# ayushpradhan-dev/robust-speech-analysis-framework

Measured on AMD Instinct MI355X. Metric: audio-seconds processed/sec (extract+CNN-LSTM fwd), higher is better.
Workload: dtype f32

## Files before the change

robust_speech_analysis_framework_amd/csrc/mshds_pitch.hip:

```cpp
#include <algorithm>
#include <map>
#include <mutex>
#include <vector>

#include "mshds_common.h"
#include "mshds_pitch_layout.h"

namespace rsaf {
namespace mshds {

struct PitchParams {
    double dt, min_pitch, ceiling, voicing_thr, octave_cost, dt_window;
    int cheb_all_full;
    int cheb_clipped;
    int nsamp_window, half_window, nsamp_period, half_period, min_lag, max_lag, brent_ixmax, max_cand;
    int refine_depth, is_cc;
    int nfft;
    double voicing_thr2;
    int debug_stop;
};

struct FrameOut {
    double intensity;
    double ncand;
    double freq[MAXC];
    double strength[MAXC];
};

typedef double double4_t __attribute__((ext_vector_type(4)));
__device__ __forceinline__ double cheb_eval(const double* __restrict__ c, double frac) {
    const double t = 2.0 * frac - 1.0, t2 = 2.0 * t;
    double b1 = 0.0, b2 = 0.0;
#pragma unroll
    for (int j = NCH - 1; j >= 1; --j) { const double b0 = fma(t2, b1, c[j] - b2); b2 = b1; b1 = b0; }
    return fma(t, b1, c[0] - b2);
}

__device__ void improve_max_cheb(const double* __restrict__ Pc, int x0, bool live, double& xm, double& ym) {
    const double ix1 = (double)x0 + 1.0;
    double c0[NCH], c1[NCH];
#pragma unroll
    for (int j = 0; j < NCH; ++j) { c0[j] = Pc[j]; c1[j] = Pc[NCH + j]; }
    auto f = [&](double v1) {
        double fl = floor(v1);
        double cell = fl - (ix1 - 1.0);
        cell = cell < 0.0 ? 0.0 : (cell > 1.0 ? 1.0 : cell);
        const double frac = v1 - (ix1 - 1.0 + cell);
        const bool hi = cell > 0.5;
        const double t = 2.0 * frac - 1.0, t2 = 2.0 * t;
        double b1 = 0.0, b2 = 0.0;
#pragma unroll
        for (int j = NCH - 1; j >= 1; --j) { const double b0 = fma(t2, b1, (hi ? c1[j] : c0[j]) - b2); b2 = b1; b1 = b0; }
        return -fma(t, b1, (hi ? c1[0] : c0[0]) - b2);
    };
    brent_maximise(f, ix1, live, xm, ym);
}

struct RefineArgs {
    const double* r; int RN, RC, depth, nz_lo, nz_hi, ncand;
    const int* place; double* cf; double* cs;
};
template <int G, bool RECUR>
__device__ void refine_candidates(const RefineArgs& A, int tid, int nthreads) {
    const int lane = tid & 63, lg = lane & (G - 1), gidx = (tid >> 6) * (64 / G) + lane / G;
    __syncthreads();
    for (int kb = 1; kb < A.ncand; kb += nthreads / G) {
        const int k = kb + gidx;
        const bool live = k < A.ncand;
        double xm, ym;
        improve_max_group<G, RECUR>(A.r, A.RN, (double)(A.place[live ? k : 1] + A.RC), A.depth, A.nz_lo, A.nz_hi, lg,
                                    live, xm, ym);
        if (ym > 1.0) ym = 1.0 / ym;
        if (live && lg == 0) { A.cf[k] = 1.0 / DXS / (xm - A.RC); A.cs[k] = ym; }
    }
}


__device__ __forceinline__ double2_t cmul(double2_t a, double2_t b) {
    return double2_t{a.x * b.x - a.y * b.y, a.x * b.y + a.y * b.x};
}
__device__ __forceinline__ double2_t tw_at(const double2_t* __restrict__ tw, int t, int M) {
    const bool neg = t >= M;
    const double2_t w = tw[neg ? t - M : t];
    return neg ? double2_t{-w.x, -w.y} : w;
}

template <int LOG2M>
struct FftPlan {
    static constexpr int M = 1 << LOG2M, N = 2 * M;
    static constexpr int N4 = LOG2M / 2;
    static constexpr bool HAS2 = (LOG2M & 1) != 0;
    static constexpr int T4 = M / 4, T2 = M / 2;
    static constexpr int BPT4 = T4 > 256 ? T4 / 256 : 1, BPT2 = T2 > 256 ? T2 / 256 : 1;
    static constexpr bool PRE = LOG2M <= 11;
    static constexpr int NTW4 = PRE && N4 > 1 ? (N4 - 1) * BPT4 * 3 : 1, NTW2 = PRE && HAS2 ? BPT2 : 1;
};

template <int LOG2M>
struct FftTw {
    double2_t w4[FftPlan<LOG2M>::NTW4];
    double2_t w2[FftPlan<LOG2M>::NTW2];
};

template <int LOG2M>
__device__ __forceinline__ void fft_load_twiddles(FftTw<LOG2M>& R, const double2_t* __restrict__ tw, int tid) {
    using PL = FftPlan<LOG2M>;
    if (!PL::PRE) return;
#pragma unroll
    for (int st = 1; st < PL::N4; ++st) {
        const int Ns = 1 << (2 * st), step = PL::N / (Ns * 4);
#pragma unroll
        for (int bq = 0; bq < PL::BPT4; ++bq) {
            const int j = tid + 256 * bq, t1 = (j & (Ns - 1)) * step;
#pragma unroll
            for (int r = 1; r <= 3; ++r) R.w4[((st - 1) * PL::BPT4 + bq) * 3 + r - 1] = tw_at(tw, (r * t1) & (PL::N - 1), PL::M);
        }
    }
    if (PL::HAS2) {
        const int Ns = 1 << (2 * PL::N4), step = PL::N / (Ns * 2);
#pragma unroll
        for (int bq = 0; bq < PL::BPT2; ++bq) R.w2[bq] = tw_at(tw, ((tid + 256 * bq) & (Ns - 1)) * step, PL::M);
    }
}

__device__ __forceinline__ int fsw(int e) { return e ^ ((e >> 3) & 3); }

template <int LOG2M>
__device__ __forceinline__ double2_t* fft_stockham(double2_t* a, double2_t* b, const FftTw<LOG2M>& R,
                                                   const double2_t* __restrict__ tw, int tid) {
    using PL = FftPlan<LOG2M>;
    constexpr int M = PL::M, N = PL::N, T4 = PL::T4, T2 = PL::T2;
    double2_t* src = a;
    double2_t* dst = b;
#pragma unroll
    for (int st = 0; st < PL::N4; ++st) {
        const int Ns = 1 << (2 * st), step = N / (Ns * 4);
#pragma unroll
        for (int bq = 0; bq < PL::BPT4; ++bq) {
            const int j = tid + 256 * bq;
            if (T4 >= 256 || j < T4) {
                const int k = j & (Ns - 1);
                const bool rs = st == 1;
                double2_t v0 = src[rs ? fsw(j) : j], v1 = src[rs ? fsw(j + T4) : j + T4], v2 = src[rs ? fsw(j + 2 * T4) : j + 2 * T4],
                          v3 = src[rs ? fsw(j + 3 * T4) : j + 3 * T4];
                if (st > 0) {
                    if (PL::PRE) {
                        const int o = ((st - 1) * PL::BPT4 + bq) * 3;
                        v1 = cmul(v1, R.w4[o]);
                        v2 = cmul(v2, R.w4[o + 1]);
                        v3 = cmul(v3, R.w4[o + 2]);
                    } else {
                        const int t1 = k * step;
                        v1 = cmul(v1, tw_at(tw, t1, M));
                        v2 = cmul(v2, tw_at(tw, 2 * t1, M));
                        v3 = cmul(v3, tw_at(tw, 3 * t1, M));
                    }
                }
                const double2_t a0 = v0 + v2, a1 = v0 - v2, a2 = v1 + v3;
                const double2_t d = v1 - v3;
                const double2_t a3 = double2_t{d.y, -d.x};
                const int j0 = ((j - k) << 2) + k;
                const bool ws = st == 0 && PL::N4 >= 2;
                dst[ws ? fsw(j0) : j0] = a0 + a2;
                dst[ws ? fsw(j0 + Ns) : j0 + Ns] = a1 + a3;
                dst[ws ? fsw(j0 + 2 * Ns) : j0 + 2 * Ns] = a0 - a2;
                dst[ws ? fsw(j0 + 3 * Ns) : j0 + 3 * Ns] = a1 - a3;
            }
        }
        __syncthreads();
        double2_t* t_ = src; src = dst; dst = t_;
    }
    if (PL::HAS2) {
        const int Ns = 1 << (2 * PL::N4), step = N / (Ns * 2);
#pragma unroll
        for (int bq = 0; bq < PL::BPT2; ++bq) {
            const int j = tid + 256 * bq;
            if (T2 >= 256 || j < T2) {
                const int k = j & (Ns - 1);
                const double2_t v0 = src[j];
                const double2_t v1 = cmul(src[j + T2], PL::PRE ? R.w2[bq] : tw_at(tw, k * step, M));
                const int j0 = ((j - k) << 1) + k;
                dst[j0] = v0 + v1;
                dst[j0 + Ns] = v0 - v1;
            }
        }
        __syncthreads();
        double2_t* t_ = src; src = dst; dst = t_;
    }
    return src;
}


template <int LOG2N>
__global__ __launch_bounds__(256) void pitch_cc_kernel(const float* __restrict__ wav, const ClipInfo* __restrict__ ci,
                                                       const double* __restrict__ gpeak, const PitchParams P,
                                                       const double2_t* __restrict__ tw1, const double2_t* __restrict__ tw2,
                                                       double* __restrict__ rbuf, int rstride, int max_frames) {
    extern __shared__ __attribute__((aligned(16))) char smem_raw[];
    const ClipInfo c = ci[blockIdx.y];
    if ((int)blockIdx.x * CC_FRAMES_PER_WG >= c.n_frames) return;
    const int tid = threadIdx.x, lane = tid & 63, wv = tid >> 6;
    constexpr int N = 1 << LOG2N, M = N >> 1;
    const int nw = P.nsamp_window, L = P.max_lag;
    const int seg_len = nw + L + 1;
    FftTw<LOG2N> twa;
    FftTw<LOG2N - 1> twb;
    fft_load_twiddles<LOG2N>(twa, tw1, tid);
    fft_load_twiddles<LOG2N - 1>(twb, tw2, tid);
    constexpr int NPK = (M / 2) / 256 + 1;
    double2_t twp[NPK];
#pragma unroll
    for (int i = 0; i < NPK; ++i) twp[i] = tw2[tid + 256 * i <= M / 2 ? tid + 256 * i : 0];
    const CcLds lds(N, L);
    double2_t* za = lds.za<double2_t>(smem_raw);
    double2_t* zb = lds.zb<double2_t, N>(smem_raw);
    double* s_sy = lds.sy(smem_raw);
    double* s_red = lds.scratch(smem_raw) + CcLds::RED;
    double* s_val = lds.scratch(smem_raw) + CcLds::VAL;
    double* s_scan = lds.scratch(smem_raw) + CcLds::SCAN;
    const float* x = wav + c.sample_off;
    const int n = c.n_samples;
    const double gp = gpeak[blockIdx.y];
    for (int f = blockIdx.x * CC_FRAMES_PER_WG; f < (int)(blockIdx.x + 1) * CC_FRAMES_PER_WG && f < c.n_frames; ++f) {
    double* rb = rbuf + ((int64_t)blockIdx.y * max_frames + f) * rstride;
    const double t = c.t1 + f * P.dt;
    const int64_t left = low_index(t, c.x1), right = left + 1;
    {
        int64_t s0 = right - P.nsamp_period, s1 = left + P.nsamp_period;
        s0 = s0 < 0 ? 0 : (s0 > n - 1 ? n - 1 : s0);
        s1 = s1 < 0 ? 0 : (s1 > n - 1 ? n - 1 : s1);
        double s = 0.0;
        for (int64_t i = s0 + tid; i <= s1; i += 256) s += (double)x[i];
        s = group_sum<64>(s);
        if (lane == 0) s_red[wv] = s;
    }
    __syncthreads();
    const double local_mean = (s_red[0] + s_red[1] + s_red[2] + s_red[3]) / (2.0 * P.nsamp_period);
    int loc_max_lag;
    {
        const double start_time = t - 0.5 * (1.0 / P.min_pitch + P.dt_window);
        int64_t start = low_index(start_time, c.x1);
        if (start < 0) start = 0;
        int64_t span = L + nw;
        if (span > n - start) span = n - start;
        loc_max_lag = (int)(span - nw);
        int pa = P.half_window - P.half_period, pb = P.half_window + P.half_period;
        pa = pa < 0 ? 0 : pa;
        pb = pb > nw ? nw : pb;
        double m = 0.0, sx = 0.0;
        const float* xs = x + start;
        const int avail = (int)((n - start) < (int64_t)seg_len ? (n - start) : (int64_t)seg_len);
#pragma unroll 4
        for (int j = tid; j < N; j += 256) {
            const double v = j < avail ? ((double)xs[j] - local_mean) : 0.0;
            za[j] = double2_t{j < nw ? v : 0.0, v};
            if (j >= pa && j < pb) m = fmax(m, fabs(v));
            if (j < nw) sx += v * v;
        }
        m = wave_max_dpp(m);
        sx = group_sum<64>(sx);
        if (lane == 0) { s_val[wv] = m; s_red[4 + wv] = sx; }
    }
    __syncthreads();
    const double local_peak = fmax(fmax(s_val[0], s_val[1]), fmax(s_val[2], s_val[3]));
    const double intensity = gp > 0.0 ? (local_peak > gp ? 1.0 : local_peak / gp) : 0.0;
    const double sumx2 = (s_red[4] + s_red[5]) + (s_red[6] + s_red[7]);
    {
        constexpr int NQ = 4;
        double inc[NQ];
#pragma unroll
        for (int q = 0; q < NQ; ++q) {
            const int i = tid + 256 * q;
            double d = 0.0;
            if (i < L) { const double u = za[i + nw].y, w0 = za[i].y; d = u * u - w0 * w0; }
            double sc = d;
#pragma unroll
            for (int o = 1; o < 64; o <<= 1) { const double t2 = __shfl_up(sc, o, 64); if (lane >= o) sc += t2; }
            inc[q] = sc;
            if (lane == 63) s_scan[4 * q + wv] = sc;
        }
        __syncthreads();
        if (tid == 0) s_sy[0] = sumx2;
#pragma unroll
        for (int q = 0; q < NQ; ++q) {
            const int i = tid + 256 * q;
            if (i < L) {
                double off = 0.0;
                for (int z = 0; z < 4 * q + wv; ++z) off += s_scan[z];
                s_sy[i + 1] = sumx2 + (off + inc[q]);
            }
        }
    }
    if (P.debug_stop == 1) continue;

    double2_t* Z = fft_stockham<LOG2N>(za, zb, twa, tw1, tid);
    double2_t* Y = Z == za ? zb : za;
    auto spec = [&](int k) {
        const double2_t zk = Z[k], zn = Z[(N - k) & (N - 1)];
        const double2_t A = double2_t{0.5 * (zk.x + zn.x), 0.5 * (zk.y - zn.y)};
        const double2_t Bm = double2_t{0.5 * (zk.y + zn.y), -0.5 * (zk.x - zn.x)};
        return double2_t{A.x * Bm.x + A.y * Bm.y, A.x * Bm.y - A.y * Bm.x};
    };
#pragma unroll
    for (int i = 0; i < NPK; ++i) {
        const int k = tid + 256 * i;
        if (k > M / 2) continue;
        const double2_t ck = spec(k), cm = spec(M - k);
        const double2_t w = twp[i];
        {
            const double2_t su = double2_t{ck.x + cm.x, ck.y - cm.y}, di = double2_t{ck.x - cm.x, ck.y + cm.y};
            const double2_t yy = double2_t{su.x - (w.x * di.y - w.y * di.x), su.y + (w.x * di.x + w.y * di.y)};
            Y[k] = double2_t{yy.x, -yy.y};
        }
        if (k != 0 && k != M - k) {
            const double2_t su = double2_t{cm.x + ck.x, cm.y - ck.y}, di = double2_t{cm.x - ck.x, cm.y + ck.y};
            const double2_t yy = double2_t{su.x + (w.x * di.y + w.y * di.x), su.y - (w.x * di.x - w.y * di.y)};
            Y[M - k] = double2_t{yy.x, -yy.y};
        }
    }
    __syncthreads();
    const double* r = reinterpret_cast<const double*>(fft_stockham<LOG2N - 1>(Y, Y == za ? zb : za, twb, tw2, tid));
    if (P.debug_stop == 2) continue;
    if (tid == 0) { rb[0] = 1.0; rb[L + 1] = intensity; }
    const double inv_n = 1.0 / (double)N;
    for (int l = 1 + tid; l <= L; l += 256) {
        const double v = ((l & 1) ? -r[l] : r[l]) * inv_n;
        const double den = sumx2 * s_sy[l];
        rb[l] = (l <= loc_max_lag && den > 0.0) ? v / sqrt(den) : 0.0;
    }
    __syncthreads();
    }
}


__device__ __forceinline__ wfft::cplx ld_tw(const double2_t* __restrict__ tw, int i) {
    const double2_t w = tw[i];
    return wfft::cplx{w.x, w.y};
}
__device__ __forceinline__ double fast_rsqrt(double d) {
    double y = __builtin_amdgcn_rsq(d);
    y = y * (1.5 - 0.5 * d * y * y);
    y = y * (1.5 - 0.5 * d * y * y);
    return y;
}
__device__ __forceinline__ double wave_scan_incl(double v, int lane) {
    v += dpp_f64<0x111>(v);
    v += dpp_f64<0x112>(v);
    v += dpp_f64<0x114>(v);
    v += dpp_f64<0x118>(v);
    const double t0 = readlane_f64(v, 15), t1 = readlane_f64(v, 31), t2 = readlane_f64(v, 47);
    const int row = lane >> 4;
    return v + (row == 0 ? 0.0 : (row == 1 ? t0 : (row == 2 ? t0 + t1 : (t0 + t1) + t2)));
}

template <int R>
__global__ __launch_bounds__(64, R == 32 ? 2 : (R == 16 ? 3 : 4)) void pitch_ac_wave_kernel(const float* __restrict__ wav, const ClipInfo* __restrict__ ci,
                                                           const double* __restrict__ gpeak, const double* __restrict__ win,
                                                           const double* __restrict__ wr, const PitchParams P,
                                                           const double2_t* __restrict__ tw, double* __restrict__ rbuf,
                                                           int rstride, int max_frames) {
    using namespace wfft;
    extern __shared__ __attribute__((aligned(16))) char smem_raw[];
    double* lds = reinterpret_cast<double*>(smem_raw);
    const ClipInfo c = ci[blockIdx.y];
    const int f0 = blockIdx.x * WF_FRAMES;
    if (f0 >= c.n_frames) return;
    const int lane_ = threadIdx.x;
    constexpr int S = 64 * R, N = 2 * S, L2 = 64 / R;
    const int nw = P.nsamp_window, L = P.brent_ixmax;
    const float* x = wav + c.sample_off;
    const int n = c.n_samples;
    const double gp = gpeak[blockIdx.y];
    LdsMem mem{lds};
    const int f1 = f0 + WF_FRAMES < c.n_frames ? f0 + WF_FRAMES : c.n_frames;
    int pa = P.half_window - P.half_period, pb = P.half_window + P.half_period;
    pa = pa < 0 ? 0 : pa;
    pb = pb > nw ? nw : pb;
#pragma unroll 1
    for (int f = f0; f < f1; ++f) {
        int lane = lane_;
        asm volatile("" : "+v"(lane));
        cplx w_s = ld_tw(tw, 2 * lane), w_b = ld_tw(tw, (lane % L2) * (N / 64));
        double* rb = rbuf + ((int64_t)blockIdx.y * max_frames + f) * rstride;
        const double t = c.t1 + f * P.dt;
        const int left = (int)low_index(t, c.x1), right = left + 1;
        const int start = right - P.half_window;
        const bool inside = start >= 0 && start + nw <= n;
        cplx v[R];
#pragma unroll
        for (int m = 0; m < R; ++m) {
            const int j = 128 * m + 2 * lane;
            int i0 = start + j, i1 = i0 + 1;
            i0 = i0 < 0 ? 0 : (i0 > n - 1 ? n - 1 : i0);
            i1 = i1 < 0 ? 0 : (i1 > n - 1 ? n - 1 : i1);
            v[m] = cplx{(double)x[i0], (double)x[i1]};
        }
        double local_mean;
        {
            int s0 = right - P.nsamp_period, s1 = left + P.nsamp_period;
            s0 = s0 < 0 ? 0 : (s0 > n - 1 ? n - 1 : s0);
            s1 = s1 < 0 ? 0 : (s1 > n - 1 ? n - 1 : s1);
            double sm = 0.0;
            if (inside && s0 >= start && s1 < start + nw) {
                const int a0 = s0 - start, a1 = s1 - start;
#pragma unroll
                for (int m = 0; m < R; ++m) {
                    const int jb = 128 * m, j = jb + 2 * lane;
                    if (jb + 127 >= a0 && jb <= a1) {
                        if (j >= a0 && j <= a1) sm += v[m].x;
                        if (j + 1 >= a0 && j + 1 <= a1) sm += v[m].y;
                    }
                }
            } else {
                for (int i = s0 + lane; i <= s1; i += 256) {
                    const float q0 = x[i], q1 = i + 64 <= s1 ? x[i + 64] : 0.f, q2 = i + 128 <= s1 ? x[i + 128] : 0.f,
                                q3 = i + 192 <= s1 ? x[i + 192] : 0.f;
                    sm += ((double)q0 + (double)q1) + ((double)q2 + (double)q3);
                }
            }
            local_mean = group_sum<64>(sm) / (2.0 * P.nsamp_period);
        }
        constexpr int WCH = R == 32 ? 8 : 4;
        double pk = 0.0;
#pragma unroll
        for (int mc = 0; mc < R; mc += WCH) {
            double2_t w2[WCH];
#pragma unroll
            for (int u = 0; u < WCH; ++u) {
                const int j = 128 * (mc + u) + 2 * lane;
                w2[u] = *reinterpret_cast<const double2_t*>(win + (j < nw ? j : nw - 2));
            }
#pragma unroll
            for (int u = 0; u < WCH; ++u) {
                const int m = mc + u, jb = 128 * m, j = jb + 2 * lane;
                const bool on = j < nw;
                const double e0 = on ? (v[m].x - local_mean) * w2[u].x : 0.0, e1 = on ? (v[m].y - local_mean) * w2[u].y : 0.0;
                if (jb + 127 >= pa && jb < pb) {
                    if (j >= pa && j < pb) pk = fmax(pk, fabs(e0));
                    if (j + 1 >= pa && j + 1 < pb) pk = fmax(pk, fabs(e1));
                }
                v[m] = cplx{e0, e1};
            }
            asm volatile("" ::: "memory");
        }
        const double local_peak = wave_max_dpp(pk);
        const double intensity = gp > 0.0 ? (local_peak > gp ? 1.0 : local_peak / gp) : 0.0;
        if (P.debug_stop == 1) continue;
        wave_fft<R>(v, lds, lane, w_s, w_b);
        {
            ac_spec_store<R>(v, mem, lane);
            wave_sync();
            const cplx y_half = ac_spec_pairs<R>(v, mem, lane, ld_tw(tw, lane));
            wave_sync();
            ac_spec_load<R>(v, mem, lane, y_half);
            wave_sync();
        }
        asm volatile("" : "+v"(lane));
        w_s = ld_tw(tw, 2 * lane);
        w_b = ld_tw(tw, (lane % L2) * (N / 64));
        wave_fft<R>(v, lds, lane, w_s, w_b);
        if (P.debug_stop == 2) continue;
        const double r0 = readlane_f64(v[0].x, 0);
        if (lane == 0) { rb[0] = 1.0; rb[L + 1] = intensity; }
        double wa[8], wb[8];
#pragma unroll
        for (int m = 0; m < 8; ++m) {
            const int l0 = 2 * (lane + 64 * m);
            wa[m] = wr[l0 < L ? l0 : L];
            wb[m] = wr[l0 + 1 < L ? l0 + 1 : L];
        }
#pragma unroll
        for (int m = 0; m < 8; ++m) {
            const int l0 = 2 * (lane + 64 * m);
            if (128 * m > L) break;
            if (l0 >= 1 && l0 <= L) rb[l0] = r0 > 0.0 ? v[m].x * fast_rcp(r0 * wa[m]) : 0.0;
            if (l0 + 1 <= L) rb[l0 + 1] = r0 > 0.0 ? -v[m].y * fast_rcp(r0 * wb[m]) : 0.0;
        }
    }
}

template <int R>
__global__ __launch_bounds__(64, R == 32 ? 2 : 3) void pitch_cc_wave_kernel(const float* __restrict__ wav, const ClipInfo* __restrict__ ci,
                                                           const double* __restrict__ gpeak, const PitchParams P,
                                                           const double2_t* __restrict__ tw, double* __restrict__ rbuf,
                                                           int rstride, int max_frames) {
    using namespace wfft;
    extern __shared__ __attribute__((aligned(16))) char smem_raw[];
    const int nw = P.nsamp_window, L = P.max_lag;
    const CcWaveLds lay(Plan<R>::LDS_DOUBLES, L);
    double* lds = lay.fft(smem_raw);
    double* s_sy = lay.sy(smem_raw);
    const ClipInfo c = ci[blockIdx.y];
    const int f0 = blockIdx.x * WF_FRAMES;
    if (f0 >= c.n_frames) return;
    const int lane_ = threadIdx.x;
    constexpr int S = 64 * R, H = R / 2, L2 = 64 / R, L2H = 64 / H;
    const int seg_len = nw + L + 1;
    const float* x = wav + c.sample_off;
    const int n = c.n_samples;
    const double gp = gpeak[blockIdx.y];
    LdsMem mem{lds};
    const int f1 = f0 + WF_FRAMES < c.n_frames ? f0 + WF_FRAMES : c.n_frames;
    int pa = P.half_window - P.half_period, pb = P.half_window + P.half_period;
    pa = pa < 0 ? 0 : pa;
    pb = pb > nw ? nw : pb;
#pragma unroll 1
    for (int f = f0; f < f1; ++f) {
        int lane = lane_;
        asm volatile("" : "+v"(lane));
        double* rb = rbuf + ((int64_t)blockIdx.y * max_frames + f) * rstride;
        const double t = c.t1 + f * P.dt;
        const int left = (int)low_index(t, c.x1), right = left + 1;
        const double start_time = t - 0.5 * (1.0 / P.min_pitch + P.dt_window);
        int64_t start64 = low_index(start_time, c.x1);
        if (start64 < 0) start64 = 0;
        const int start = (int)start64;
        int span = L + nw;
        if (span > n - start) span = n - start;
        const int loc_max_lag = span - nw;
        const int avail = n - start < seg_len ? n - start : seg_len;
        cplx v[R];
#pragma unroll
        for (int m = 0; m < R; ++m) {
            int gi = start + lane + 64 * m;
            gi = gi > n - 1 ? n - 1 : gi;
            v[m] = cplx{0.0, (double)x[gi]};
        }
        float tail[16];
#pragma unroll
        for (int q = 0; q < 16; ++q) {
            int gi = start + lane + 64 * q + nw;
            gi = gi > n - 1 ? n - 1 : gi;
            tail[q] = x[gi];
        }
        double local_mean;
        {
            int s0 = right - P.nsamp_period, s1 = left + P.nsamp_period;
            s0 = s0 < 0 ? 0 : (s0 > n - 1 ? n - 1 : s0);
            s1 = s1 < 0 ? 0 : (s1 > n - 1 ? n - 1 : s1);
            double sm = 0.0;
            if (s0 >= start && s1 < start + avail) {
                const int a0 = s0 - start, a1 = s1 - start;
#pragma unroll
                for (int m = 0; m < R; ++m) {
                    const int jb = 64 * m, j = jb + lane;
                    if (jb + 63 >= a0 && jb <= a1 && j >= a0 && j <= a1) sm += v[m].y;
                }
            } else {
                for (int i = s0 + lane; i <= s1; i += 256) {
                    const float q0 = x[i], q1 = i + 64 <= s1 ? x[i + 64] : 0.f, q2 = i + 128 <= s1 ? x[i + 128] : 0.f,
                                q3 = i + 192 <= s1 ? x[i + 192] : 0.f;
                    sm += ((double)q0 + (double)q1) + ((double)q2 + (double)q3);
                }
            }
            local_mean = group_sum<64>(sm) / (2.0 * P.nsamp_period);
        }
        double pk = 0.0, sx = 0.0;
#pragma unroll
        for (int m = 0; m < R; ++m) {
            const int jb = 64 * m, j = jb + lane;
            double e = 0.0, a = 0.0;
            if (j < avail) e = v[m].y - local_mean;
            if (j < nw) a = e;
            if (jb + 63 >= pa && jb < pb && j >= pa && j < pb) pk = fmax(pk, fabs(e));
            sx = fma(a, a, sx);
            v[m] = cplx{a, e};
        }
        const double local_peak = wave_max_dpp(pk);
        const double intensity = gp > 0.0 ? (local_peak > gp ? 1.0 : local_peak / gp) : 0.0;
        const double sumx2 = group_sum<64>(sx);
        {
            double carry = 0.0;
            if (lane == 0) s_sy[0] = sumx2;
#pragma unroll
            for (int q = 0; q < 16; ++q) {
                if (64 * q >= L) break;
                const int i = lane + 64 * q;
                double d = 0.0;
                if (i < L) {
                    const double u = i + nw < avail ? (double)tail[q] - local_mean : 0.0, w0 = v[q].y;
                    d = u * u - w0 * w0;
                }
                const double sc = wave_scan_incl(d, lane);
                if (i < L) s_sy[i + 1] = sumx2 + (carry + sc);
                carry += readlane_f64(sc, 63);
            }
        }
        if (P.debug_stop == 1) continue;
        const cplx w_s1 = ld_tw(tw, lane);
        wave_fft<R>(v, lds, lane, w_s1, ld_tw(tw, (lane % L2) * R));
        cplx y[H];
        cc_spec_store<R>(v, mem, lane);
        wave_sync();
        const cplx y_half = cc_spec_pairs<R>(v, y, mem, lane, w_s1);
        wave_sync();
        cc_spec_load<R>(y, mem, lane, y_half);
        wave_sync();
        wave_fft<H>(y, lds, lane, ld_tw(tw, 2 * lane), ld_tw(tw, (lane % L2H) * R));
        if (P.debug_stop == 2) continue;
        if (lane == 0) { rb[0] = 1.0; rb[L + 1] = intensity; }
        const double inv_n = 1.0 / (double)S;
        constexpr int MO = H < 8 ? H : 8;
        double ya[MO], yb[MO];
#pragma unroll
        for (int m = 0; m < MO; ++m) {
            const int l0 = 2 * (lane + 64 * m);
            ya[m] = s_sy[l0 < L ? l0 : L];
            yb[m] = s_sy[l0 + 1 < L ? l0 + 1 : L];
        }
#pragma unroll
        for (int m = 0; m < MO; ++m) {
            const int l0 = 2 * (lane + 64 * m);
            if (128 * m > L) break;
            if (l0 >= 1 && l0 <= L) {
                const double den = sumx2 * ya[m];
                rb[l0] = (l0 <= loc_max_lag && den > 0.0) ? (y[m].x * inv_n) * fast_rsqrt(den) : 0.0;
            }
            if (l0 + 1 <= L) {
                const double den = sumx2 * yb[m];
                rb[l0 + 1] = (l0 + 1 <= loc_max_lag && den > 0.0) ? (-y[m].y * inv_n) * fast_rsqrt(den) : 0.0;
            }
        }
        wave_sync();
    }
}

constexpr int CT = 64;
struct DeferArgs {
    FrameHdr* hdr;
    double* pc_a;
    double* pc_b;
    int grouped;
};
struct CandCtx {
    const PitchParams& P;
    const DeferArgs& DA;
    const double* cheb;
    int lane;
    int L, RC, RN;
    int nz_lo, nz_hi;
    double* r;
    double *s_mfreq, *s_mstr, *s_mloc;
    int* s_maxlag;
    int* s_cnt;
    double* s_part;
};

__device__ __forceinline__ void cand_load_row(const CandCtx& X, const double* __restrict__ rb, int r_lo, int r_hi) {
    const int tid = X.lane, RC = X.RC, L = X.L;
    double* r = X.r;
    for (int j0 = RC + r_lo + tid; j0 <= RC + r_hi; j0 += 10 * CT) {
        double v[10];
#pragma unroll
        for (int u = 0; u < 10; ++u) {
            const int j = j0 + u * CT;
            const int l = j >= RC ? j - RC : RC - j;
            v[u] = rb[l <= L ? l : L];
        }
#pragma unroll
        for (int u = 0; u < 10; ++u) {
            const int j = j0 + u * CT;
            const int l = j >= RC ? j - RC : RC - j;
            if (j <= RC + r_hi) r[j] = l <= L ? v[u] : 0.0;
        }
    }
}

__device__ __forceinline__ void cand_collect_maxima(const CandCtx& X, double thr_low) {
    const PitchParams& P = X.P;
    const int lane = X.lane, RC = X.RC;
    const double* r = X.r;
    int* s_maxlag = X.s_maxlag;
    int* s_cnt = X.s_cnt;
    const int lag_lo = P.min_lag > 2 ? P.min_lag : 2;
    int lag_hi = P.max_lag - 1;
    if (lag_hi > P.brent_ixmax - 1) lag_hi = P.brent_ixmax - 1;
    int count = 0;
    for (int base = lag_lo; base <= lag_hi; base += 64) {
        const int l = base + lane;
        bool ok = false;
        if (l <= lag_hi) {
            const double v = r[RC + l];
            ok = (v > 0.5 * thr_low) && (v > r[RC + l - 1]) && (v >= r[RC + l + 1]);
        }
        const unsigned long long m = __ballot(ok);
        const int pos = count + __popcll(m & ((1ull << lane) - 1ull));
        if (ok && pos < MAX_MAXIMA) s_maxlag[pos] = l;
        count += __popcll(m);
    }
    if (lane == 0) s_cnt[CandLds::CNT_NMAX] = count < MAX_MAXIMA ? count : MAX_MAXIMA;
}

__device__ __forceinline__ void cand_first_estimates(const CandCtx& X, int nmax) {
    const PitchParams& P = X.P;
    const int lane = X.lane, RC = X.RC, RN = X.RN, nz_lo = X.nz_lo, nz_hi = X.nz_hi;
    const double* r = X.r;
    const int* s_maxlag = X.s_maxlag;
    double *s_mfreq = X.s_mfreq, *s_mstr = X.s_mstr, *s_mloc = X.s_mloc;
    const int l16 = lane & 15, gidx = lane >> 4;
    for (int mb = 0; mb < nmax; mb += CT / 16) {
        const int m = mb + gidx;
        const bool live = m < nmax;
        const int l = s_maxlag[live ? m : 0];
        const double y0 = r[RC + l - 1], y1 = r[RC + l], y2 = r[RC + l + 1];
        const double dr = 0.5 * (y2 - y0), d2r = 2.0 * y1 - y0 - y2;
        const double fm = 1.0 / DXS / (l + dr / d2r);
        double st = sinc_group<16, false>(r, RN, RC + 1.0 / DXS / fm, 30, nz_lo, nz_hi, l16);
        if (st > 1.0) st = 1.0 / st;
        if (live && l16 == 0) { s_mfreq[m] = fm; s_mstr[m] = st; s_mloc[m] = st - P.octave_cost * log2(P.min_pitch / fm); }
    }
}

struct CandMaxima { double mloc0, mloc1, mr0, mr1; };
__device__ __forceinline__ void cand_build_list(const CandCtx& X, const CandMaxima& M, double vthr, double* cf, double* cs,
                                                double* cloc, int* place_lag, int* ncand_out) {
    const PitchParams& P = X.P;
    const int lane = X.lane;
    const double mloc0 = M.mloc0, mloc1 = M.mloc1, mr0 = M.mr0, mr1 = M.mr1;
    const double *s_mfreq = X.s_mfreq, *s_mstr = X.s_mstr;
    const int* s_maxlag = X.s_maxlag;
    unsigned long long todo0 = __ballot(mr0 > 0.5 * vthr), todo1 = __ballot(mr1 > 0.5 * vthr);
    double my_loc = 0.0;
    int my_m = -1, nc = 1;
    double weakest = 2.0;
    int wplace = 0;
    bool known = false;
    for (int half = 0; half < 2; ++half) {
        unsigned long long todo = half ? todo1 : todo0;
        while (todo) {
            const int bit = __ffsll((long long)todo) - 1;
            todo &= todo - 1;
            const int m = 64 * half + bit;
            const double loc_m = readlane_f64(half ? mloc1 : mloc0, bit);
            int place;
            if (nc < P.max_cand) {
                place = nc++;
            } else {
                if (!known) {
                    const double v = (lane >= 1 && lane < P.max_cand) ? my_loc : INFINITY;
                    double mn = v;
#pragma unroll
                    for (int o = 32; o >= 1; o >>= 1) mn = fmin(mn, __shfl_xor(mn, o, 64));
                    if (mn < 2.0) { weakest = mn; wplace = __ffsll((long long)__ballot(v == mn)) - 1; }
                    else { weakest = 2.0; wplace = 0; }
                    known = true;
                }
                place = loc_m <= weakest ? 0 : wplace;
            }
            if (place) {
                if (lane == place) { my_loc = loc_m; my_m = m; }
                known = false;
            }
        }
    }
    if (lane < MAXC) {
        const bool on = lane >= 1 && lane < nc && my_m >= 0;
        cf[lane] = on ? s_mfreq[my_m] : 0.0;
        cs[lane] = on ? s_mstr[my_m] : 0.0;
        cloc[lane] = on ? my_loc : 0.0;
        place_lag[lane] = on ? s_maxlag[my_m] : 0;
    }
    if (lane == 0) *ncand_out = nc;
}

__device__ __forceinline__ int cand_row_min(int v) {
    v = min(v, __builtin_amdgcn_update_dpp(0, v, 0xB1, 0xf, 0xf, false));
    v = min(v, __builtin_amdgcn_update_dpp(0, v, 0x4E, 0xf, 0xf, false));
    v = min(v, __builtin_amdgcn_update_dpp(0, v, 0x141, 0xf, 0xf, false));
    v = min(v, __builtin_amdgcn_update_dpp(0, v, 0x140, 0xf, 0xf, false));
    return __builtin_amdgcn_readlane(v, 0);
}

struct CandClip {
    bool use_cheb;
    int n_clip_cols;
    bool cand_lane;
    int my_b0;
};
__device__ __forceinline__ CandClip cand_clip_analysis(const CandCtx& X, int nc, const int* place_lag) {
    const PitchParams& P = X.P;
    const double* cheb = X.cheb;
    const int lane = X.lane, RC = X.RC, RN = X.RN;
    bool use_cheb = cheb != nullptr;
    int n_clip_cols = 0;
    const bool cand_lane = lane >= 1 && lane < nc;
    const int my_b0 = (cand_lane ? place_lag[lane] : 0) + RC - 1;
    if (use_cheb && !P.cheb_all_full) {
        int dc0 = P.refine_depth, dc1 = P.refine_depth;
        dc0 = dc0 < my_b0 + 1 ? dc0 : my_b0 + 1;
        dc0 = dc0 < RN - my_b0 - 1 ? dc0 : RN - my_b0 - 1;
        dc1 = dc1 < my_b0 + 2 ? dc1 : my_b0 + 2;
        dc1 = dc1 < RN - my_b0 - 2 ? dc1 : RN - my_b0 - 2;
        n_clip_cols = __popcll(__ballot(cand_lane && dc0 < P.refine_depth)) + __popcll(__ballot(cand_lane && dc1 < P.refine_depth));
        const int dmin = cand_row_min(cand_lane ? min(dc0, dc1) : P.refine_depth);
        if (n_clip_cols > 0 && (!P.cheb_clipped || dmin < 3)) use_cheb = false;
    }
    return CandClip{use_cheb, n_clip_cols, cand_lane, my_b0};
}

__device__ __forceinline__ void cand_coef_4x4x4(const CandCtx& X, int nc, const int* place_lag, const CandClip& C) {
    const double* cheb = X.cheb;
    const int lane = X.lane, RC = X.RC, nz_lo = X.nz_lo, nz_hi = X.nz_hi;
    const double* r = X.r;
    const bool cand_lane = C.cand_lane;
    const int my_b0 = C.my_b0;
    double* s_P = X.s_part;
    const int d = X.P.refine_depth;
    const int kq = lane >> 4, nn = lane & 15;
    const int ncol = 2 * (nc - 1);
    const int bmin = cand_row_min(cand_lane ? my_b0 : 0x7fffffff), bmax = -cand_row_min(cand_lane ? -my_b0 : 0x7fffffff);
    const int groups = (ncol + 3) >> 2;
    int rb4[3];
    bool cf4[3];
#pragma unroll
    for (int g = 0; g < 3; ++g) {
        const int n = 4 * g + (lane & 3), k = 1 + (n >> 1);
        rb4[g] = place_lag[k < nc ? k : 1] + RC - 1 + (n & 1);
        cf4[g] = n < ncol;
    }
    int o_lo = nz_lo - (bmax + 1), o_hi = nz_hi - bmin;
    o_lo = o_lo < -(d - 1) ? -(d - 1) : o_lo;
    o_hi = o_hi > d ? d : o_hi;
    double a4[3] = {0.0, 0.0, 0.0};
    const double* ctab = cheb + (int64_t)(d - 1) * NCH + nn;
    int o = o_lo;
    for (; o + 31 <= o_hi; o += 32) {
        double cw[8];
#pragma unroll
        for (int u = 0; u < 8; ++u) cw[u] = ctab[(int64_t)(o + 4 * u + kq) * NCH];
#pragma unroll
        for (int u = 0; u < 8; ++u) {
            const int oo = o + 4 * u + kq;
            a4[0] = __builtin_amdgcn_mfma_f64_4x4x4f64(cw[u], cf4[0] ? r[rb4[0] + oo] : 0.0, a4[0], 0, 0, 0);
            if (groups > 1) a4[1] = __builtin_amdgcn_mfma_f64_4x4x4f64(cw[u], cf4[1] ? r[rb4[1] + oo] : 0.0, a4[1], 0, 0, 0);
            if (groups > 2) a4[2] = __builtin_amdgcn_mfma_f64_4x4x4f64(cw[u], cf4[2] ? r[rb4[2] + oo] : 0.0, a4[2], 0, 0, 0);
        }
    }
    for (; o <= o_hi; o += 4) {
        const int oo = o + kq, oc = oo <= o_hi ? oo : o_hi;
        const double cw = oo <= o_hi ? ctab[(int64_t)oc * NCH] : 0.0;
        a4[0] = __builtin_amdgcn_mfma_f64_4x4x4f64(cw, cf4[0] ? r[rb4[0] + oc] : 0.0, a4[0], 0, 0, 0);
        if (groups > 1) a4[1] = __builtin_amdgcn_mfma_f64_4x4x4f64(cw, cf4[1] ? r[rb4[1] + oc] : 0.0, a4[1], 0, 0, 0);
        if (groups > 2) a4[2] = __builtin_amdgcn_mfma_f64_4x4x4f64(cw, cf4[2] ? r[rb4[2] + oc] : 0.0, a4[2], 0, 0, 0);
    }
    const int coef = (nn & 12) + kq;
#pragma unroll
    for (int g = 0; g < 3; ++g) {
        const int n = 4 * g + (lane & 3), k = 1 + (n >> 1);
        if (g < groups && n < ncol) s_P[(k * 2 + (n & 1)) * NCH + coef] = a4[g];
    }
}

__device__ __forceinline__ void cand_coef_16x16x4(const CandCtx& X, int nc, const int* place_lag, const CandClip& C) {
    const double* cheb = X.cheb;
    const int lane = X.lane, RC = X.RC, RN = X.RN, nz_lo = X.nz_lo, nz_hi = X.nz_hi;
    const double* r = X.r;
    const bool cand_lane = C.cand_lane;
    const int my_b0 = C.my_b0, n_clip_cols = C.n_clip_cols;
    double* s_P = X.s_part;
    const int d = X.P.refine_depth;
    const int kq = lane >> 4, nn = lane & 15;
    const int ncol = 2 * (nc - 1), tiles = (ncol + 15) >> 4;
    const int bmin = cand_row_min(cand_lane ? my_b0 : 0x7fffffff), bmax = -cand_row_min(cand_lane ? -my_b0 : 0x7fffffff);
    int rbase[2];
    bool colfull[2];
#pragma unroll
    for (int T = 0; T < 2; ++T) {
        const int n = 16 * T + nn, k = 1 + (n >> 1);
        rbase[T] = place_lag[k < nc ? k : 1] + RC - 1 + (n & 1);
        colfull[T] = n_clip_cols == 0 || (rbase[T] + 1 >= d && RN - rbase[T] - 1 >= d);
    }
    int o_lo = nz_lo - (bmax + 1), o_hi = nz_hi - bmin;
    o_lo = o_lo < -(d - 1) ? -(d - 1) : o_lo;
    o_hi = o_hi > d ? d : o_hi;
    double4_t acc0 = {0.0, 0.0, 0.0, 0.0}, acc1 = acc0;
    const double* ctab = cheb + (int64_t)(d - 1) * NCH + nn;
    int o = o_lo;
    for (; o + 31 <= o_hi; o += 32) {
        double cw[8];
#pragma unroll
        for (int u = 0; u < 8; ++u) cw[u] = ctab[(int64_t)(o + 4 * u + kq) * NCH];
#pragma unroll
        for (int u = 0; u < 8; ++u) {
            const int oo = o + 4 * u + kq;
            acc0 = __builtin_amdgcn_mfma_f64_16x16x4f64(cw[u], colfull[0] ? r[rbase[0] + oo] : 0.0, acc0, 0, 0, 0);
            if (tiles > 1) acc1 = __builtin_amdgcn_mfma_f64_16x16x4f64(cw[u], colfull[1] ? r[rbase[1] + oo] : 0.0, acc1, 0, 0, 0);
        }
    }
    for (; o <= o_hi; o += 4) {
        const int oo = o + kq, oc = oo <= o_hi ? oo : o_hi;
        const double cw = oo <= o_hi ? ctab[(int64_t)oc * NCH] : 0.0;
        acc0 = __builtin_amdgcn_mfma_f64_16x16x4f64(cw, colfull[0] ? r[rbase[0] + oc] : 0.0, acc0, 0, 0, 0);
        if (tiles > 1) acc1 = __builtin_amdgcn_mfma_f64_16x16x4f64(cw, colfull[1] ? r[rbase[1] + oc] : 0.0, acc1, 0, 0, 0);
    }
#pragma unroll
    for (int T = 0; T < 2; ++T) {
        const int n = 16 * T + nn, k = 1 + (n >> 1);
        if (T < tiles && k < nc) {
#pragma unroll
            for (int v = 0; v < 4; ++v) s_P[(k * 2 + (n & 1)) * NCH + kq + 4 * v] = T == 0 ? acc0[v] : acc1[v];
        }
    }
}

__device__ __forceinline__ void cand_coef_clipped_cells(const CandCtx& X, int nc, const int* place_lag) {
    const double* cheb = X.cheb;
    const int lane = X.lane, RC = X.RC, RN = X.RN;
    const double* r = X.r;
    double* s_P = X.s_part;
    const int d = X.P.refine_depth;
    const int ncol = 2 * (nc - 1);
    __builtin_amdgcn_fence(__ATOMIC_RELEASE, "workgroup");
    __builtin_amdgcn_wave_barrier();
    __builtin_amdgcn_fence(__ATOMIC_ACQUIRE, "workgroup");
    const double* clip_tabs = cheb + (int64_t)2 * d * NCH;
    const int jj = lane & 15, ph = lane >> 4;
    for (int col = 0; col < ncol; ++col) {
        const int k = 1 + (col >> 1), b = place_lag[k] + RC - 1 + (col & 1);
        int dc = d;
        dc = dc < b + 1 ? dc : b + 1;
        dc = dc < RN - b - 1 ? dc : RN - b - 1;
        if (dc >= d) continue;
        const double* tab = clip_tabs + (int64_t)NCH * dc * (dc - 1) + jj;
        double acc = 0.0;
        int o = -(dc - 1) + ph;
        for (; o + 12 <= dc; o += 16) {
            double tw4[4];
#pragma unroll
            for (int u = 0; u < 4; ++u) tw4[u] = tab[(int64_t)(o + 4 * u + dc - 1) * NCH];
#pragma unroll
            for (int u = 0; u < 4; ++u) acc = fma(tw4[u], r[b + o + 4 * u], acc);
        }
        for (; o <= dc; o += 4) acc = fma(tab[(int64_t)(o + dc - 1) * NCH], r[b + o], acc);
        acc += __shfl_xor(acc, 16, 64);
        acc += __shfl_xor(acc, 32, 64);
        if (ph == 0) s_P[(k * 2 + (col & 1)) * NCH + jj] = acc;
    }
}

__device__ __forceinline__ bool cand_hand_over_or_brent(const CandCtx& X, int nc, const int* place_lag, double* cf, double* cs,
                                                        double* pc_out) {
    const DeferArgs& DA = X.DA;
    const int tid = X.lane, RC = X.RC;
    const double* s_P = X.s_part;
    if (DA.hdr) {
        for (int i = 2 * NCH + tid; i < nc * 2 * NCH; i += CT) pc_out[i] = s_P[i];
        __syncthreads();
        return true;
    }
    if (tid < 64) {
        const int k = 1 + tid;
        const bool live = k < nc;
        double xm, ym;
        improve_max_cheb(s_P + (live ? k : 1) * 2 * NCH, place_lag[live ? k : 1] + RC, live, xm, ym);
        if (ym > 1.0) ym = 1.0 / ym;
        if (live) { cf[k] = 1.0 / DXS / (xm - RC); cs[k] = ym; }
    }
    __syncthreads();
    return false;
}

__device__ __forceinline__ void cand_refine_direct(const CandCtx& X, int nc, const int* place_lag, double* cf, double* cs) {
const PitchParams& P = X.P;
const int tid = X.lane, L = X.L, RC = X.RC, RN = X.RN, nz_lo = X.nz_lo, nz_hi = X.nz_hi;
const double* r = X.r;
    const int nref = nc - 1;
    const int span = P.refine_depth < 2 * L ? P.refine_depth : 2 * L;
    RefineArgs A{r, RN, RC, P.refine_depth, nz_lo, nz_hi, nc, place_lag, cf, cs};
    if (nref <= 4) { if (span >= 6 * 64) refine_candidates<64, true>(A, tid, CT); else refine_candidates<64, false>(A, tid, CT); }
    else if (nref <= 8) { if (span >= 6 * 32) refine_candidates<32, true>(A, tid, CT); else refine_candidates<32, false>(A, tid, CT); }
    else { if (span >= 6 * 16) refine_candidates<16, true>(A, tid, CT); else refine_candidates<16, false>(A, tid, CT); }
    __syncthreads();
}

__device__ __forceinline__ bool cand_refine_list(const CandCtx& X, int nc, const int* place_lag, double* cf, double* cs,
                                                 double* pc_out) {
    if (X.DA.hdr && X.DA.grouped) return true;
    const CandClip C = cand_clip_analysis(X, nc, place_lag);
    if (C.use_cheb) {
        const int ncol = 2 * (nc - 1);
        if (nc > 1 && ncol <= 12 && C.n_clip_cols == 0) {
            cand_coef_4x4x4(X, nc, place_lag, C);
        } else if (nc > 1) {
            cand_coef_16x16x4(X, nc, place_lag, C);
            if (C.n_clip_cols > 0) cand_coef_clipped_cells(X, nc, place_lag);
        }
        __syncthreads();
        if (X.P.debug_stop == 6) return true;
        return cand_hand_over_or_brent(X, nc, place_lag, cf, cs, pc_out);
    }
    cand_refine_direct(X, nc, place_lag, cf, cs);
    return false;
}

__device__ __forceinline__ void cand_write_hdr(FrameHdr* hdr, int tid, int flags, int n_a, const int* pl_a, int n_b,
                                               const int* pl_b, int hit) {
    if (tid < MAXC) {
        hdr->lag_a[tid] = (uint16_t)pl_a[tid];
        if (pl_b) {
            hdr->lag_b[tid] = (uint16_t)pl_b[tid];
            hdr->a_slot_of_b[tid] = (uint8_t)hit;
        }
    }
    if (tid == 0) { hdr->flags = flags; hdr->n_a = n_a; hdr->n_b = n_b; }
}

__device__ __forceinline__ void cand_write_frame_out(FrameOut* o, int tid, double intensity, double gp, int ncand,
                                                     const double* cf, const double* cs) {
    if (tid == 0) {
        o->intensity = intensity;
        o->ncand = gp > 0.0 ? (double)ncand : 1.0;
    }
    if (tid < MAXC) {
        const bool on = tid < ncand && gp > 0.0;
        o->freq[tid] = on ? cf[tid] : 0.0;
        o->strength[tid] = on ? cs[tid] : 0.0;
    }
}

__global__ __launch_bounds__(64) void pitch_cand_kernel(const ClipInfo* __restrict__ ci, const double* __restrict__ gpeak,
                                                        const PitchParams P, const double* __restrict__ rbuf, int rstride,
                                                        int max_frames, FrameOut* __restrict__ out,
                                                        FrameOut* __restrict__ out2, const double* __restrict__ cheb,
                                                        const DeferArgs DA) {
    extern __shared__ __attribute__((aligned(16))) char smem_raw[];
    const ClipInfo c = ci[blockIdx.y];
    const int f = blockIdx.x;
    if (f >= c.n_frames) return;
    const int tid = threadIdx.x, lane = tid & 63;
    const int L = P.is_cc ? P.max_lag : P.brent_ixmax;
    const int RC = P.brent_ixmax;
    const int RN = 2 * P.brent_ixmax + 1;
    int r_lo, r_hi;
    pitch_r_range(RC, L, P.min_lag, P.max_lag, (DA.hdr && DA.grouped) ? 30 : P.refine_depth, &r_lo, &r_hi);
    const CandLds lds(r_lo, r_hi);
    double* r_store = lds.r_store(smem_raw);
    double* r = r_store - (RC + r_lo);
    double* lists = lds.lists(smem_raw);
    int* ilists = reinterpret_cast<int*>(lists);
    double* s_mfreq = lists + CandLds::MFREQ;
    double* s_mstr = lists + CandLds::MSTR;
    double* s_mloc = lists + CandLds::MLOC;
    double* s_cf = lists + CandLds::CF;
    double* s_cs = lists + CandLds::CS;
    double* s_cloc = lists + CandLds::CLOC;
    int* s_maxlag = ilists + CandLds::MAXLAG;
    int* s_place = ilists + CandLds::PLACE;
    int* s_place2 = ilists + CandLds::PLACE2;
    int* s_cnt = ilists + CandLds::CNT;
    double* s_cf2 = lists + CandLds::CF2;
    double* s_cs2 = lists + CandLds::CS2;
    double* s_cloc2 = lists + CandLds::CLOC2;
    double* s_part = lists + CandLds::PART;
    const CandCtx X{P, DA, cheb, lane, L, RC, RN, RC - L, RC + L, r, s_mfreq, s_mstr, s_mloc, s_maxlag, s_cnt, s_part};

    FrameOut* o = out + c.frame_off + f;
#define RSAF_PITCH_DBG_STOP(k)                                                                       \
    if (P.debug_stop == (k)) {                                                                       \
        if (tid == 0) { o->intensity = 0.0; o->ncand = 1.0; }                                        \
        if (tid < MAXC) { o->freq[tid] = 0.0; o->strength[tid] = 0.0; }                              \
        return;                                                                                      \
    }
    RSAF_PITCH_DBG_STOP(1)
    RSAF_PITCH_DBG_STOP(2)
    const double* rb = rbuf + ((int64_t)blockIdx.y * max_frames + f) * rstride;
    const double intensity = rb[L + 1];
    const double gp = gpeak[blockIdx.y];
    cand_load_row(X, rb, r_lo, r_hi);
    if (tid == 0) s_cnt[CandLds::CNT_NMAX] = 0;
    __syncthreads();
    const bool dual = out2 != nullptr && P.voicing_thr2 >= 0.0;
    const double thr_low = dual && P.voicing_thr2 < P.voicing_thr ? P.voicing_thr2 : P.voicing_thr;
    cand_collect_maxima(X, thr_low);
    __syncthreads();
    RSAF_PITCH_DBG_STOP(3)
    const int nmax = s_cnt[CandLds::CNT_NMAX];
    cand_first_estimates(X, nmax);
    __syncthreads();
    RSAF_PITCH_DBG_STOP(4)
    const CandMaxima M{lane < nmax ? s_mloc[lane] : 0.0, lane + 64 < nmax ? s_mloc[lane + 64] : 0.0,
                       lane < nmax ? r[RC + s_maxlag[lane]] : -1.0, lane + 64 < nmax ? r[RC + s_maxlag[lane + 64]] : -1.0};
    cand_build_list(X, M, P.voicing_thr, s_cf, s_cs, s_cloc, s_place, &s_cnt[CandLds::CNT_NCAND]);
    if (dual) cand_build_list(X, M, P.voicing_thr2, s_cf2, s_cs2, s_cloc2, s_place2, &s_cnt[CandLds::CNT_NCAND2]);
    __syncthreads();
    const int ncand = s_cnt[CandLds::CNT_NCAND];
    RSAF_PITCH_DBG_STOP(5)
    const int64_t wframe = (int64_t)blockIdx.y * max_frames + f;
    FrameHdr* hdr = DA.hdr ? DA.hdr + wframe : nullptr;
    int flags = 0;
    if (!dual) {
        if (cand_refine_list(X, ncand, s_place, s_cf, s_cs, DA.pc_a ? DA.pc_a + wframe * PC_DOUBLES : nullptr)) flags = HDR_A_DEFER;
        if (hdr) cand_write_hdr(hdr, tid, gp > 0.0 ? flags : 0, ncand, s_place, 0, nullptr, 0);
    } else {
        const int ncand2 = s_cnt[CandLds::CNT_NCAND2];
        const bool low_is_second = P.voicing_thr2 < P.voicing_thr;
        int* pl_a = low_is_second ? s_place2 : s_place;   double* cf_a = low_is_second ? s_cf2 : s_cf;   double* cs_a = low_is_second ? s_cs2 : s_cs;
        int* pl_b = low_is_second ? s_place : s_place2;   double* cf_b = low_is_second ? s_cf : s_cf2;   double* cs_b = low_is_second ? s_cs : s_cs2;
        const int nc_a = low_is_second ? ncand2 : ncand, nc_b = low_is_second ? ncand : ncand2;
        const bool def_a = cand_refine_list(X, nc_a, pl_a, cf_a, cs_a, DA.pc_a ? DA.pc_a + wframe * PC_DOUBLES : nullptr);
        if (def_a) flags |= HDR_A_DEFER;
        if (tid == 0) s_cnt[CandLds::CNT_MISSING] = 0;
        __syncthreads();
        int hit = 0;
        {
            const int pa_reg = tid < MAXC ? pl_a[tid] : 0;
            const int mine = (tid >= 1 && tid < nc_b) ? pl_b[tid] : -1;
            for (int z = 1; z < nc_a; ++z) if (__builtin_amdgcn_readlane(pa_reg, z) == mine) hit = z;
            if (tid >= 1 && tid < nc_b) {
                if (hit) { if (!def_a) { cf_b[tid] = cf_a[hit]; cs_b[tid] = cs_a[hit]; } } else atomicAdd(&s_cnt[CandLds::CNT_MISSING], 1);
            }
        }
        __syncthreads();
        if (s_cnt[CandLds::CNT_MISSING] > 0) {
            if (tid >= 1 && tid < nc_b) {
                for (int m = 0; m < nmax; ++m) if (s_maxlag[m] == pl_b[tid]) { cf_b[tid] = s_mfreq[m]; cs_b[tid] = s_mstr[m]; }
            }
            __syncthreads();
            if (cand_refine_list(X, nc_b, pl_b, cf_b, cs_b, DA.pc_b ? DA.pc_b + wframe * PC_DOUBLES : nullptr)) flags |= HDR_B_DEFER;
        } else if (def_a) {
            flags |= HDR_B_COPY;
        }
        if (hdr) cand_write_hdr(hdr, tid, gp > 0.0 ? flags : 0, nc_a, pl_a, nc_b, pl_b, hit);
        cand_write_frame_out(out2 + c.frame_off + f, tid, intensity, gp, ncand2, s_cf2, s_cs2);
    }
    cand_write_frame_out(o, tid, intensity, gp, ncand, s_cf, s_cs);
}
#undef RSAF_PITCH_DBG_STOP

__global__ __launch_bounds__(256) void pitch_cell_coef_kernel(const ClipInfo* __restrict__ ci, int n_clips, int max_frames,
                                                              const int* __restrict__ hdr, const double* __restrict__ rbuf,
                                                              int rstride, int L, int RC, const double* __restrict__ tabs,
                                                              int b_lo, int n_b, int ntap_pad, int chunk_frames, int n_chunks,
                                                              double* __restrict__ pc) {
    using namespace wfft;
    extern __shared__ __attribute__((aligned(16))) char smem_raw[];
    const CellLds lds(ntap_pad);
    double* tab = lds.tab(smem_raw);
    unsigned* qall = lds.queues(smem_raw);
    const int64_t wid = blockIdx.x;
    const int64_t q = wid >> 3;
    const int bi = (int)(q % n_b);
    const int64_t chunk = (q / n_b) * 8 + (wid & 7);
    if (chunk >= n_chunks) return;
    const int tid = threadIdx.x, lane = tid & 63, wv = tid >> 6;
    unsigned* qb = qall + wv * CELL_Q;
    const int b = b_lo + bi;
    const int lag0 = b - RC + 1, lag1 = b - RC;
    const int64_t total = (int64_t)n_clips * max_frames;
    const int per_wave = chunk_frames / 4;
    const int64_t g_begin = chunk * chunk_frames + (int64_t)wv * per_wave;
    const int64_t g_end = g_begin + per_wave < total ? g_begin + per_wave : total;
    const int nn = lane & 15, kq = lane >> 4;
    struct Rec { int nc; int lw[8]; };
    auto load_rec = [&](int64_t g) {
        Rec r;
        r.nc = 0;
#pragma unroll
        for (int i = 0; i < 8; ++i) r.lw[i] = 0;
        if (g < g_end) {
            const int clip = (int)(g / max_frames), fr = (int)(g - (int64_t)clip * max_frames);
            if (fr < ci[clip].n_frames) {
                const FrameHdr* h = FrameHdr::at(hdr, g);
                const int flags = h->flags, nc = h->n_a;
#pragma unroll
                for (int i = 0; i < 8; ++i) r.lw[i] = (int)h->lag_a_pair(i);
                r.nc = (flags & HDR_A_DEFER) ? nc : 0;
            }
        }
        return r;
    };
    Rec rec = load_rec(g_begin + lane);
    {
        const double2_t* src = reinterpret_cast<const double2_t*>(tabs + (int64_t)bi * ntap_pad * NCH);
        double2_t* dst = reinterpret_cast<double2_t*>(tab);
        const int n2 = ntap_pad * NCH / 2;
        for (int i0 = tid; i0 < n2; i0 += 8 * 256) {
            double2_t v[8];
#pragma unroll
            for (int u = 0; u < 8; ++u) v[u] = src[i0 + 256 * u < n2 ? i0 + 256 * u : n2 - 1];
#pragma unroll
            for (int u = 0; u < 8; ++u) if (i0 + 256 * u < n2) dst[i0 + 256 * u] = v[u];
        }
    }
    __syncthreads();
    int count = 0;
    auto run_tile = [&](int off, int n) {
        const unsigned e = qb[off + (nn < n ? nn : 0)];
        const int64_t g = e >> 5;
        const int k = (e >> 1) & 15, c = e & 1;
        const double* rb = rbuf + g * rstride;
        double4_t acc = {0.0, 0.0, 0.0, 0.0};
        double av[2][8], bv[2][8];
        auto fetch = [&](int t0, double (&a8)[8], double (&b8)[8]) {
#pragma unroll
            for (int u = 0; u < 8; ++u) {
                const int t = t0 + 4 * u + kq;
                const int tc = t < ntap_pad ? t : ntap_pad - 1;
                b8[u] = rb[tc <= L ? tc : L];
                a8[u] = t < ntap_pad ? tab[tc * NCH + nn] : 0.0;
            }
        };
        fetch(0, av[0], bv[0]);
        for (int t0 = 0; t0 < ntap_pad; t0 += 64) {
            if (t0 + 32 < ntap_pad) fetch(t0 + 32, av[1], bv[1]);
#pragma unroll
            for (int u = 0; u < 8; ++u) acc = __builtin_amdgcn_mfma_f64_16x16x4f64(av[0][u], bv[0][u], acc, 0, 0, 0);
            if (t0 + 32 >= ntap_pad) break;
            if (t0 + 64 < ntap_pad) fetch(t0 + 64, av[0], bv[0]);
#pragma unroll
            for (int u = 0; u < 8; ++u) acc = __builtin_amdgcn_mfma_f64_16x16x4f64(av[1][u], bv[1][u], acc, 0, 0, 0);
        }
        if (nn < n) {
            double* dst = pc + (g * MAXC + k) * (2 * NCH) + c * NCH;
#pragma unroll
            for (int v = 0; v < 4; ++v) dst[kq + 4 * v] = acc[v];
        }
    };
    for (int64_t g0 = g_begin; g0 < g_end; g0 += 64) {
        const int64_t g = g0 + lane;
        int m0 = 0, m1 = 0;
#pragma unroll
        for (int k = 1; k < MAXC; ++k) {
            const int lg = (rec.lw[k >> 1] >> (16 * (k & 1))) & 0xffff;
            if (k < rec.nc && lg == lag0) m0 = k;
            if (k < rec.nc && lg == lag1) m1 = k;
        }
        rec = load_rec(g + 64);
        const unsigned long long b0 = __ballot(m0 != 0), b1 = __ballot(m1 != 0);
        const unsigned long long below = (1ull << lane) - 1ull;
        if (m0) qb[count + __popcll(b0 & below)] = ((unsigned)g << 5) | ((unsigned)m0 << 1);
        count += __popcll(b0);
        if (m1) qb[count + __popcll(b1 & below)] = ((unsigned)g << 5) | ((unsigned)m1 << 1) | 1u;
        count += __popcll(b1);
        wave_sync();
        int done = 0;
        for (; count - done >= 16; done += 16) run_tile(done, 16);
        const int left = count - done;
        const unsigned rest = lane < left ? qb[done + lane] : 0u;
        wave_sync();
        if (lane < left) qb[lane] = rest;
        count = left;
        wave_sync();
    }
    if (count > 0) run_tile(0, count);
}

__global__ __launch_bounds__(64) void pitch_brent_kernel(const ClipInfo* __restrict__ ci, const int* __restrict__ hdr,
                                                         const double* __restrict__ pc_a, const double* __restrict__ pc_b,
                                                         int max_frames, int RC, FrameOut* __restrict__ out_a,
                                                         FrameOut* __restrict__ out_b) {
    const ClipInfo c = ci[blockIdx.y];
    const int f0 = blockIdx.x * BR_FRAMES;
    if (f0 >= c.n_frames) return;
    const int lane = threadIdx.x;
    const int64_t g0 = (int64_t)blockIdx.y * max_frames + f0;
    int cnt_a = 0, cnt_b = 0;
    if (lane < BR_FRAMES && f0 + lane < c.n_frames) {
        const FrameHdr* h = FrameHdr::at(hdr, g0 + lane);
        const int flags = h->flags;
        if (flags & HDR_A_DEFER) cnt_a = h->n_a > 1 ? h->n_a - 1 : 0;
        if (flags & HDR_B_DEFER) cnt_b = h->n_b > 1 ? h->n_b - 1 : 0;
    }
    const int tot = cnt_a + cnt_b;
    int incl = tot;
#pragma unroll
    for (int o = 1; o < BR_FRAMES; o <<= 1) { const int up = __shfl_up(incl, o, 64); if (lane >= o) incl += up; }
    const int excl = incl - tot;
    const int T = __builtin_amdgcn_readlane(incl, BR_FRAMES - 1);
    for (int q0 = 0; q0 < T; q0 += 64) {
        const int q = q0 + lane;
        const bool live = q < T;
        int j = 0;
#pragma unroll
        for (int jj = 1; jj < BR_FRAMES; ++jj) if (__builtin_amdgcn_readlane(excl, jj) <= q) j = jj;
        if (!live) j = 0;
        const int r = q - __shfl(excl, j, 64), na = __shfl(cnt_a, j, 64);
        const bool is_b = live && r >= na;
        const int slot = live ? (is_b ? r - na : r) + 1 : 1;
        const int64_t g = g0 + j;
        const FrameHdr* h = FrameHdr::at(hdr, g);
        const int lag = (is_b ? h->lag_b : h->lag_a)[slot];
        const double* Pc = (is_b ? pc_b : pc_a) + (g * MAXC + slot) * (2 * NCH);
        double xm, ym;
        improve_max_cheb(Pc, lag + RC, live, xm, ym);
        if (ym > 1.0) ym = 1.0 / ym;
        const double fq = 1.0 / DXS / (xm - RC);
        if (live) {
            FrameOut* o = (is_b ? out_b : out_a) + c.frame_off + f0 + j;
            o->freq[slot] = fq;
            o->strength[slot] = ym;
            if (!is_b && out_b != nullptr && (h->flags & HDR_B_COPY)) {
                const int nc_b = h->n_b;
                FrameOut* o2 = out_b + c.frame_off + f0 + j;
#pragma unroll
                for (int w = 0; w < 4; ++w) {
                    const unsigned hw = h->a_slot_of_b_quad(w);
#pragma unroll
                    for (int u = 0; u < 4; ++u) {
                        const int t = 4 * w + u;
                        if (t >= 1 && t < nc_b && (int)((hw >> (8 * u)) & 0xff) == slot) { o2->freq[t] = fq; o2->strength[t] = ym; }
                    }
                }
            }
        }
    }
}

constexpr int PATH_CH = 32;
constexpr int PATH_RING = 4 * PATH_CH;

__global__ __launch_bounds__(64) void path_kernel(const FrameOut* __restrict__ fr, const ClipInfo* __restrict__ ci,
                                                  double dt, double silence_thr, double voicing_thr, double octave_cost,
                                                  double octave_jump_cost, double vuv_cost, double ceiling,
                                                  unsigned char* __restrict__ psi, int* __restrict__ end_state) {
    __shared__ double s_delta[PATH_RING * MAXC], s_logf[PATH_RING * MAXC];
    __shared__ unsigned char s_flag[PATH_RING * MAXC];
    __shared__ double s_cur[2][MAXC];
    __shared__ __attribute__((aligned(16))) unsigned char s_psi[PATH_CH * MAXC];
    const ClipInfo c = ci[blockIdx.x];
    const int lane = threadIdx.x;
    const int nF = c.n_frames;
    if (nF <= 0) return;
    const FrameOut* F = fr + c.frame_off;
    unsigned char* P = psi + c.frame_off * MAXC;
    const double corr = 0.01 / dt;
    const double ojc = octave_jump_cost * corr, vuc = vuv_cost * corr;
    auto clampn = [](double nc) { const int v = (int)nc; return v < 0 ? 0 : (v > MAXC ? MAXC : v); };
    constexpr int PPLN = PATH_CH * MAXC / 64;
    constexpr int RING = PATH_RING;
    double lfq[PPLN], lst[PPLN], lnc[PPLN], lin[PPLN];
    auto fetch = [&](int f0) {
#pragma unroll
        for (int u = 0; u < PPLN; ++u) {
            const int pr = lane + 64 * u, fi = f0 + (pr >> 4), cd = pr & (MAXC - 1);
            const int f = fi < nF ? fi : nF - 1;
            lfq[u] = F[f].freq[cd]; lst[u] = F[f].strength[cd]; lnc[u] = F[f].ncand; lin[u] = F[f].intensity;
        }
    };
    auto derive_to = [&](int f0) {
        const int base = (f0 % RING) * MAXC;
#pragma unroll
        for (int u = 0; u < PPLN; ++u) {
            const int pr = lane + 64 * u, cd = pr & (MAXC - 1);
            const bool valid = cd < clampn(lnc[u]);
            const bool vl = !(lfq[u] > 0.0 && lfq[u] < ceiling);
            double unv = silence_thr <= 0.0 ? 0.0 : 2.0 - lin[u] / (silence_thr / (1.0 + voicing_thr));
            unv = voicing_thr + fmax(0.0, unv);
            s_delta[base + pr] = valid ? (vl ? unv : lst[u] - octave_cost * log2(ceiling / lfq[u])) : -1e300;
            s_logf[base + pr] = vl ? 0.0 : log2(lfq[u]);
            s_flag[base + pr] = (unsigned char)((vl ? 1 : 0) | (valid ? 2 : 0));
        }
    };
    auto lds_sync = [] {
        __builtin_amdgcn_fence(__ATOMIC_RELEASE, "wavefront");
        __builtin_amdgcn_wave_barrier();
        __builtin_amdgcn_fence(__ATOMIC_ACQUIRE, "wavefront");
    };
    const int j = lane >> 2, q = lane & 3;
    fetch(0);
    derive_to(0);
    fetch(PATH_CH);
    lds_sync();
    if (q == 0) { s_cur[0][j] = s_delta[j]; s_psi[j] = 0; }
    double cur = s_delta[j];
    for (int f0 = 0; f0 < nF; f0 += PATH_CH) {
        if (f0 + PATH_CH < nF) {
            derive_to(f0 + PATH_CH);
            fetch(f0 + 2 * PATH_CH);
        }
        lds_sync();
        const int fend = f0 + PATH_CH < nF ? f0 + PATH_CH : nF;
#pragma unroll 1
        for (int f = f0 > 0 ? f0 : 1; f < fend; ++f) {
            const int me = (f % RING) * MAXC + j, pb = ((f - 1) % RING) * MAXC;
            const double delta = s_delta[me], logf = s_logf[me];
            const int fl = s_flag[me], vl = fl & 1, valid = (fl >> 1) & 1;
            const double* pcur = s_cur[(f - 1) & 1];
            double best = -INFINITY;
            int place = 0;
#pragma unroll
            for (int u = 0; u < 4; ++u) {
                const int c1 = q + 4 * u;
                const double pc = pcur[c1], pl = s_logf[pb + c1];
                const int pf = s_flag[pb + c1], pv = pf & 1, pval = (pf >> 1) & 1;
                const double tc = (pv && vl) ? 0.0 : ((pv || vl) ? vuc : ojc * fabs(pl - logf));
                const double v = pval ? pc - tc + delta : -INFINITY;
                if (v > best) { best = v; place = c1; }
            }
            {
                double ov = dpp_f64<0xB1>(best);
                int op = __builtin_amdgcn_update_dpp(0, place, 0xB1, 0xf, 0xf, false);
                if (ov > best || (ov == best && op < place)) { best = ov; place = op; }
                ov = dpp_f64<0x4E>(best);
                op = __builtin_amdgcn_update_dpp(0, place, 0x4E, 0xf, 0xf, false);
                if (ov > best || (ov == best && op < place)) { best = ov; place = op; }
            }
            if (best == -INFINITY) place = 0;
            if (!valid) best = -1e300;
            cur = best;
            if (q == 0) { s_cur[f & 1][j] = best; s_psi[(f - f0) * MAXC + j] = (unsigned char)place; }
            lds_sync();
        }
        if (lane < fend - f0)
            reinterpret_cast<uint4*>(P + (int64_t)f0 * MAXC)[lane] = reinterpret_cast<const uint4*>(s_psi)[lane];
        lds_sync();
    }
    double bv = q == 0 ? cur : -INFINITY;
    int bi = j;
#pragma unroll
    for (int o = 32; o >= 1; o >>= 1) {
        const double ov = __shfl_xor(bv, o, 64);
        const int oi = __shfl_xor(bi, o, 64);
        if (ov > bv || (ov == bv && oi < bi)) { bv = ov; bi = oi; }
    }
    if (lane == 0) end_state[blockIdx.x] = bi;
}

constexpr int BT_CHUNK = 3072;
__global__ __launch_bounds__(256) void backtrack_kernel(const FrameOut* __restrict__ fr, const ClipInfo* __restrict__ ci,
                                                        const unsigned char* __restrict__ psi,
                                                        const int* __restrict__ end_state, double* __restrict__ sel_freq,
                                                        double* __restrict__ sel_strength) {
    __shared__ __attribute__((aligned(16))) unsigned char s_psi[BT_CHUNK * MAXC];
    __shared__ unsigned char s_state[BT_CHUNK];
    __shared__ unsigned char s_map[256 * MAXC];
    __shared__ unsigned char s_entry[256];
    __shared__ int s_carry;
    const ClipInfo c = ci[blockIdx.x];
    if (c.n_frames <= 0) return;
    const int tid = threadIdx.x;
    const FrameOut* F = fr + c.frame_off;
    const unsigned char* P = psi + c.frame_off * MAXC;
    if (tid == 0) s_carry = end_state[blockIdx.x];
    for (int hi = c.n_frames; hi > 0; hi -= BT_CHUNK) {
        const int lo = hi > BT_CHUNK ? hi - BT_CHUNK : 0, cnt = hi - lo;
        const uint4* src = reinterpret_cast<const uint4*>(P + (int64_t)lo * MAXC);
        uint4* dst = reinterpret_cast<uint4*>(s_psi);
        for (int i = tid; i < cnt; i += 256) dst[i] = src[i];
        __syncthreads();
        const int SL = (cnt + 255) / 256, nseg = (cnt + SL - 1) / SL;
        const int fb = tid * SL, ft = min(fb + SL, cnt) - 1;
        if (tid < nseg) {
            unsigned char x[MAXC];
#pragma unroll
            for (int e = 0; e < MAXC; ++e) x[e] = (unsigned char)e;
            for (int f = ft; f >= fb; --f) {
                if (lo + f > 0) {
#pragma unroll
                    for (int e = 0; e < MAXC; ++e) x[e] = s_psi[f * MAXC + x[e]];
                }
            }
#pragma unroll
            for (int e = 0; e < MAXC; ++e) s_map[tid * MAXC + e] = x[e];
        }
        __syncthreads();
        if (tid == 0) {
            int st = s_carry;
            for (int t = nseg - 1; t >= 0; --t) { s_entry[t] = (unsigned char)st; st = s_map[t * MAXC + st]; }
            s_carry = st;
        }
        __syncthreads();
        if (tid < nseg) {
            int st = s_entry[tid];
            for (int f = ft; f >= fb; --f) {
                s_state[f] = (unsigned char)st;
                if (lo + f > 0) st = s_psi[f * MAXC + st];
            }
        }
        __syncthreads();
        for (int i = tid; i < cnt; i += 256) {
            const int st = s_state[i];
            sel_freq[c.frame_off + lo + i] = F[lo + i].freq[st];
            sel_strength[c.frame_off + lo + i] = F[lo + i].strength[st];
        }
        __syncthreads();
    }
}

__global__ __launch_bounds__(64) void pitch_stats_kernel(const double* __restrict__ sel_freq, const ClipInfo* __restrict__ ci,
                                                         double ceiling, double* __restrict__ out) {
    const ClipInfo c = ci[blockIdx.x];
    const int lane = threadIdx.x;
    const double* f = sel_freq + c.frame_off;
    double n0 = 0, s0 = 0, nv = 0, sv = 0, sst = 0;
    for (int i = lane; i < c.n_frames; i += 64) {
        const double v = f[i];
        if (v != 0.0) { n0 += 1; s0 += v; }
        if (v > 0.0 && v < ceiling) { nv += 1; sv += v; sst += 12.0 * log2(v / 100.0); }
    }
    n0 = wave_sum_f64(n0); s0 = wave_sum_f64(s0); nv = wave_sum_f64(nv); sv = wave_sum_f64(sv); sst = wave_sum_f64(sst);
    const double m0 = n0 > 0 ? s0 / n0 : 0.0, mst = nv > 0 ? sst / nv : 0.0;
    double q0 = 0, qst = 0;
    for (int i = lane; i < c.n_frames; i += 64) {
        const double v = f[i];
        if (v != 0.0) q0 += (v - m0) * (v - m0);
        if (v > 0.0 && v < ceiling) { const double d = 12.0 * log2(v / 100.0) - mst; qst += d * d; }
    }
    q0 = wave_sum_f64(q0); qst = wave_sum_f64(qst);
    const double sd0 = n0 > 0 ? sqrt(q0 / n0) : 0.0;
    double nf = 0, sf = 0;
    for (int i = lane; i < c.n_frames; i += 64) {
        const double v = f[i];
        if (v != 0.0 && fabs((v - m0) / sd0) <= 2.0) { nf += 1; sf += v; }
    }
    nf = wave_sum_f64(nf); sf = wave_sum_f64(sf);
    if (lane == 0) {
        double* o = out + (int64_t)blockIdx.x * 8;
        const double qn = __longlong_as_double(0x7ff8000000000000LL);
        o[0] = n0; o[1] = m0; o[2] = sd0; o[3] = nf > 0 ? sf / nf : qn;
        o[4] = nv; o[5] = nv > 0 ? sv / nv : qn; o[6] = nv > 1 ? sqrt(qst / (nv - 1)) : qn; o[7] = nf;
    }
}

}
}

using namespace rsaf;
using namespace rsaf::mshds;


static int fft_twiddles(int N, const double** out) {
    static std::mutex mu;
    static std::map<std::pair<int, int>, double*> cache;
    int dev = 0;
    RSAF_CHECK_HIP(hipGetDevice(&dev));
    std::lock_guard<std::mutex> lock(mu);
    auto it = cache.find({dev, N});
    if (it == cache.end()) {
        std::vector<double> h((size_t)N);
        for (int k = 0; k < N / 2; ++k) {
            const double a = 2.0 * M_PI * (double)k / (double)N;
            h[2 * k] = cos(a);
            h[2 * k + 1] = -sin(a);
        }
        if (N >= 4) { h[2 * (N / 4)] = 0.0; h[2 * (N / 4) + 1] = -1.0; }
        double* d = nullptr;
        RSAF_CHECK_HIP(hipMalloc(&d, (size_t)N * sizeof(double)));
        RSAF_CHECK_HIP(hipMemcpy(d, h.data(), (size_t)N * sizeof(double), hipMemcpyHostToDevice));
        it = cache.emplace(std::make_pair(dev, N), d).first;
    }
    *out = it->second;
    return RSAF_OK;
}


enum PitchSlot {
    PS_DT, PS_MIN_PITCH, PS_CEILING, PS_VOICING_THR, PS_OCTAVE_COST, PS_SILENCE_THR, PS_OCTAVE_JUMP, PS_VUV,
    PS_NSAMP_WINDOW, PS_NSAMP_PERIOD, PS_MIN_LAG, PS_MAX_LAG, PS_BRENT_IXMAX, PS_MAX_CAND, PS_REFINE_DEPTH, PS_IS_CC,
    PS_DT_WINDOW,
    PS_TABLE_MODE,
};

static int pitch_row_lags(const double* h) { return (int)h[PS_IS_CC] ? (int)h[PS_MAX_LAG] : (int)h[PS_BRENT_IXMAX]; }

struct PitchCall {
    const float* wav;
    const ClipInfo* ci;
    int n_clips, max_frames;
    const double* gpeak;
    const double *window, *window_r, *sinc_cheb;
    double* workspace;
    int64_t workspace_bytes;
    hipStream_t stream;
};

struct PitchOutputs {
    FrameOut* frame_out;
    unsigned char* psi;
    int* end_state;
    double *sel_freq, *sel_strength, *stats;
    bool complete() const { return frame_out && psi && end_state && sel_freq && sel_strength && stats; }
};

struct PitchPlan {
    PitchParams P;
    double silence_thr, octave_jump, vuv;
    bool dual;
    int seg_len, Lr, rstride;
    int ncc, log2m, log2n;
    int wave_r;
    size_t lds_corr, lds_cand, lds_cell;
    int cell_b_lo, cell_n_b, cell_ntap_pad;
    bool defer;
    bool grouped;
    const double* cheb;
    int group;
    double corr_flops, corr_lds;
};

static int64_t cell_workgroups(const PitchPlan& pl, int64_t gframes, int* n_chunks_out) {
    const int64_t n_chunks = (gframes + CELL_CHUNK_FRAMES - 1) / CELL_CHUNK_FRAMES;
    if (n_chunks_out) *n_chunks_out = (int)n_chunks;
    return 8 * (int64_t)pl.cell_n_b * ((n_chunks + 7) / 8);
}

static int pitch_plan(const PitchCall& c, const double* h, const PitchOutputs& o1, const PitchOutputs& o2,
                      double voicing_thr2, PitchPlan* plan) {
    PitchPlan& pl = *plan;
    PitchParams& P = pl.P;
    const int n_clips = c.n_clips, max_frames = c.max_frames;
    RSAF_CHECK_ARG(n_clips >= 0 && n_clips <= 65535 && max_frames >= 0, "bad clip/frame count");
    if (n_clips == 0) return RSAF_OK;
    RSAF_CHECK_ARG(c.wav && c.ci && c.gpeak && h && o1.complete(), "NULL pointer");
    const bool dual = pl.dual = voicing_thr2 >= 0.0;
    RSAF_CHECK_ARG(!dual || o2.complete(), "NULL pointer (second threshold outputs)");
    P.dt = h[PS_DT]; P.min_pitch = h[PS_MIN_PITCH]; P.ceiling = h[PS_CEILING]; P.voicing_thr = h[PS_VOICING_THR];
    P.octave_cost = h[PS_OCTAVE_COST];
    pl.silence_thr = h[PS_SILENCE_THR]; pl.octave_jump = h[PS_OCTAVE_JUMP]; pl.vuv = h[PS_VUV];
    P.nsamp_window = (int)h[PS_NSAMP_WINDOW]; P.nsamp_period = (int)h[PS_NSAMP_PERIOD];
    P.min_lag = (int)h[PS_MIN_LAG]; P.max_lag = (int)h[PS_MAX_LAG]; P.brent_ixmax = (int)h[PS_BRENT_IXMAX];
    P.max_cand = (int)h[PS_MAX_CAND]; P.refine_depth = (int)h[PS_REFINE_DEPTH]; P.is_cc = (int)h[PS_IS_CC];
    P.dt_window = h[PS_DT_WINDOW];
    const int table_mode = (int)h[PS_TABLE_MODE];
    P.cheb_clipped = table_mode == 1 ? 1 : 0;
    P.voicing_thr2 = dual ? voicing_thr2 : -1.0;
    { const char* e = getenv("RSAF_PITCH_STOP"); P.debug_stop = e ? atoi(e) : 0; }
    P.half_window = P.nsamp_window / 2;
    P.half_period = P.nsamp_period / 2 + 1;
    RSAF_CHECK_ARG(P.max_cand >= 2 && P.max_cand <= MAXC - 1, "max_candidates must be in [2, 15]");
    RSAF_CHECK_ARG(P.nsamp_window >= 4 && P.brent_ixmax >= 2 && P.max_lag >= 2, "window too short");
    RSAF_CHECK_ARG(P.is_cc || (c.window && c.window_r), "AC needs the window tables");
    RSAF_CHECK_ARG((P.is_cc ? P.max_lag : P.brent_ixmax) <= 1023, "more than 1023 lags (pitch floor below ~16 Hz) is not supported");
    P.nfft = 1;
    while ((double)P.nfft < (double)P.nsamp_window * 1.5) P.nfft *= 2;
    if (P.nfft < 16) P.nfft = 16;
    RSAF_CHECK_ARG(P.is_cc || P.nsamp_window + P.brent_ixmax <= P.nfft, "brent_ixmax must not exceed half the analysis window");
    const int seg_len = pl.seg_len = P.is_cc ? P.nsamp_window + P.max_lag + 1 : P.nsamp_window;
    const int Lr = pl.Lr = pitch_row_lags(h);
    pl.rstride = Lr + 2;
    int ncc = 64;
    while (ncc < seg_len) ncc *= 2;
    RSAF_CHECK_ARG(!P.is_cc || ncc <= 4096, "cross-correlation window + lag range longer than 4 095 samples is not supported");
    RSAF_CHECK_ARG(P.is_cc || P.nfft <= 4096, "autocorrelation window longer than 2 730 samples is not supported");
    pl.lds_corr = P.is_cc ? CcLds(ncc, Lr).bytes() : 0;
    pl.defer = getenv("RSAF_PITCH_INKERNEL") == nullptr;
    pl.grouped = pl.defer && table_mode == 2 && !dual && P.is_cc && c.sinc_cheb != nullptr;
    int r_lo_h, r_hi_h;
    pitch_r_range(P.brent_ixmax, Lr, P.min_lag, P.max_lag, pl.grouped ? 30 : P.refine_depth, &r_lo_h, &r_hi_h);
    pl.lds_cand = CandLds(r_lo_h, r_hi_h).bytes();
    RSAF_CHECK_ARG(pl.lds_corr <= 150 * 1024 && pl.lds_cand <= 150 * 1024, "analysis window too long for LDS");
    const int64_t row_bytes_per_clip = (int64_t)max_frames * PitchWs::bytes_per_frame(pl.rstride);
    RSAF_CHECK_ARG(max_frames == 0 || (c.workspace && c.workspace_bytes >= row_bytes_per_clip),
                   "workspace too small (rsaf_mshds_pitch_workspace_bytes)");
    int group = max_frames == 0 ? n_clips : (int)std::min<int64_t>(n_clips, c.workspace_bytes / std::max<int64_t>(row_bytes_per_clip, 1));
    if (max_frames > 0) group = (int)std::min<int64_t>(group, ((int64_t)1 << 26) / max_frames > 0 ? ((int64_t)1 << 26) / max_frames : 1);
    pl.group = group;
    RSAF_CHECK_ARG(table_mode != 2 || (!dual && P.is_cc), "per-cell tables serve single-threshold cross-correlation analyses only");
    pl.log2m = 0;
    while ((2 << pl.log2m) < P.nfft) ++pl.log2m;
    pl.log2n = 0;
    while ((1 << pl.log2n) < ncc) ++pl.log2n;
    int wave_r = 0;
    if (!P.is_cc) wave_r = pl.log2m <= 9 ? 8 : 1 << (pl.log2m - 6);
    else if (pl.log2n <= 11) wave_r = pl.log2n <= 10 ? 16 : 32;
    if (wave_r && !P.is_cc) P.nfft = 128 * wave_r;
    if (wave_r && P.is_cc) ncc = 64 * wave_r;
    pl.wave_r = wave_r;
    pl.ncc = ncc;
    pl.cheb = table_mode == 2 ? nullptr : c.sinc_cheb;
    const int cell_lag_lo = P.min_lag > 2 ? P.min_lag : 2;
    const int cell_lag_hi = std::min(P.max_lag - 1, P.brent_ixmax - 1);
    const bool unclipped = P.brent_ixmax + cell_lag_lo - 1 >= P.refine_depth && cell_lag_hi + 2 + P.refine_depth <= P.brent_ixmax;
    P.cheb_all_full = unclipped ? 1 : 0;
    if (pl.cheb == nullptr) P.cheb_clipped = 0;
    if (!unclipped && !P.cheb_clipped) pl.cheb = nullptr;
    pl.cell_b_lo = P.brent_ixmax + cell_lag_lo - 1;
    pl.cell_n_b = cell_lag_hi - cell_lag_lo + 2;
    pl.cell_ntap_pad = (Lr + 1 + 3) & ~3;
    pl.lds_cell = CellLds(pl.cell_ntap_pad).bytes();
    if (pl.grouped) {
        RSAF_CHECK_ARG(pl.cell_n_b >= 1 && pl.lds_cell <= 150 * 1024, "per-cell tables: lag range too long for LDS");
        if (max_frames > 0 && P.debug_stop == 0)
            RSAF_CHECK_ARG(cell_workgroups(pl, (int64_t)group * max_frames, nullptr) <= 0x7fffffffLL,
                           "per-cell tables: too many workgroups");
    }
    const double Mfft = 0.5 * (double)P.nfft;
    const double ac_flops = 2.0 * 5.0 * Mfft * log2(Mfft) + 30.0 * Mfft;
    const double cc_flops = 5.0 * ncc * log2((double)ncc) + 2.5 * ncc * log2(0.5 * ncc) + 40.0 * 0.5 * ncc + 4.0 * seg_len;
    const double ac_lds = 160.0 * Mfft;
    const double cc_lds = wave_r ? 120.0 * ncc + 16.0 * Lr
                                 : 16.0 * ncc * (ceil(log2((double)ncc) / 2.0) + 2.0) * 2.0 + 16.0 * 0.5 * ncc * (ceil(log2(0.5 * ncc) / 2.0) + 1.0) * 2.0;
    pl.corr_flops = P.is_cc ? cc_flops : ac_flops;
    pl.corr_lds = P.is_cc ? cc_lds : ac_lds;
    return RSAF_OK;
}

static int pitch_prepare(const PitchPlan& pl, const double2_t** tw_out, const double2_t** tw2_out) {
    if (!pl.wave_r)
        RSAF_CHECK_HIP(hipFuncSetAttribute((const void*)pitch_cc_kernel<12>, hipFuncAttributeMaxDynamicSharedMemorySize, (int)pl.lds_corr));
    const double *tw = nullptr, *tw2 = nullptr;
    int rc = fft_twiddles(pl.P.is_cc ? 2 * pl.ncc : pl.P.nfft, &tw);
    if (rc == RSAF_OK && pl.P.is_cc) rc = fft_twiddles(pl.ncc, &tw2);
    if (rc != RSAF_OK) return rc;
    *tw_out = reinterpret_cast<const double2_t*>(tw);
    *tw2_out = reinterpret_cast<const double2_t*>(tw2);
    if (pl.lds_cand > 48 * 1024)
        RSAF_CHECK_HIP(hipFuncSetAttribute((const void*)pitch_cand_kernel, hipFuncAttributeMaxDynamicSharedMemorySize,
                                           (int)pl.lds_cand));
    if (pl.grouped && pl.lds_cell > 48 * 1024)
        RSAF_CHECK_HIP(hipFuncSetAttribute((const void*)pitch_cell_coef_kernel, hipFuncAttributeMaxDynamicSharedMemorySize,
                                           (int)pl.lds_cell));
    return RSAF_OK;
}

struct PitchGroup {
    const ClipInfo* ci;
    const double* gpeak;
    int nc;
    PitchWs ws;
};

static PitchGroup pitch_group(const PitchCall& c, const PitchPlan& pl, int c0) {
    const int nc = std::min(pl.group, c.n_clips - c0);
    return PitchGroup{c.ci + c0, c.gpeak + c0, nc, PitchWs(c.workspace, (int64_t)nc * c.max_frames, pl.rstride)};
}

template <int R>
static void launch_ac_wave(const PitchCall& c, const PitchPlan& pl, const PitchGroup& g, dim3 grid, const double2_t* tw) {
    hipLaunchKernelGGL(pitch_ac_wave_kernel<R>, grid, dim3(64), (size_t)wfft::Plan<R>::LDS_DOUBLES * sizeof(double), c.stream,
                       c.wav, g.ci, g.gpeak, c.window, c.window_r, pl.P, tw, g.ws.rows, pl.rstride, c.max_frames);
}

template <int R>
static void launch_cc_wave(const PitchCall& c, const PitchPlan& pl, const PitchGroup& g, dim3 grid, const double2_t* tw2) {
    hipLaunchKernelGGL(pitch_cc_wave_kernel<R>, grid, dim3(64), CcWaveLds(wfft::Plan<R>::LDS_DOUBLES, pl.Lr).bytes(), c.stream, c.wav, g.ci, g.gpeak, pl.P, tw2,
                       g.ws.rows, pl.rstride, c.max_frames);
}

static int launch_correlation(const PitchCall& c, const PitchPlan& pl, const PitchGroup& g, const double2_t* tw, const double2_t* tw2) {
    ProfScope prof(pl.P.is_cc ? "mshds_pitch_cc_fft" : "mshds_pitch_ac_fft", c.stream,
                   pl.corr_flops * (double)c.max_frames * (double)g.nc, pl.corr_lds * (double)c.max_frames * (double)g.nc);
    const dim3 wave_grid((c.max_frames + WF_FRAMES - 1) / WF_FRAMES, g.nc);
    if (!pl.wave_r)
        hipLaunchKernelGGL(pitch_cc_kernel<12>, dim3((c.max_frames + CC_FRAMES_PER_WG - 1) / CC_FRAMES_PER_WG, g.nc), dim3(256),
                           pl.lds_corr, c.stream, c.wav, g.ci, g.gpeak, pl.P, tw, tw2, g.ws.rows, pl.rstride, c.max_frames);
    else if (pl.P.is_cc)
        switch (pl.wave_r) {
            case 16: launch_cc_wave<16>(c, pl, g, wave_grid, tw2); break;
            case 32: launch_cc_wave<32>(c, pl, g, wave_grid, tw2); break;
        }
    else
        switch (pl.wave_r) {
            case 8: launch_ac_wave<8>(c, pl, g, wave_grid, tw); break;
            case 16: launch_ac_wave<16>(c, pl, g, wave_grid, tw); break;
            case 32: launch_ac_wave<32>(c, pl, g, wave_grid, tw); break;
        }
    RSAF_CHECK_HIP(hipGetLastError());
    return RSAF_OK;
}

static int launch_candidates(const PitchCall& c, const PitchPlan& pl, const PitchGroup& g, FrameOut* out, FrameOut* out2) {
    const double rows = (double)c.max_frames * (double)g.nc;
    const DeferArgs DA{pl.defer ? g.ws.hdr : nullptr, pl.defer ? g.ws.pc_a : nullptr, pl.defer ? g.ws.pc_b : nullptr, pl.grouped ? 1 : 0};
    ProfScope prof(pl.grouped ? "mshds_pitch_cand_lists" : pl.cheb ? "mshds_pitch_cand_cheb" : "mshds_pitch_cand_direct", c.stream,
                   pl.cheb ? rows * 2048.0 * 2.0 * ceil(2.0 * pl.P.refine_depth / 4.0) : 0.0,
                   rows * (double)(pl.Lr + 2) * 8.0);
    hipLaunchKernelGGL(pitch_cand_kernel, dim3(c.max_frames, g.nc), dim3(CT), pl.lds_cand, c.stream, g.ci, g.gpeak, pl.P,
                       (const double*)g.ws.rows, pl.rstride, c.max_frames, out, out2, pl.cheb, DA);
    RSAF_CHECK_HIP(hipGetLastError());
    return RSAF_OK;
}

static int launch_refinement(const PitchCall& c, const PitchPlan& pl, const PitchGroup& g, FrameOut* out, FrameOut* out2) {
    const double rows = (double)c.max_frames * (double)g.nc;
    if (pl.grouped) {
        int n_chunks;
        const int64_t n_wg = cell_workgroups(pl, (int64_t)g.nc * c.max_frames, &n_chunks);
        ProfScope prof("mshds_pitch_cand_cells", c.stream, rows * 28.0 * 2.0 * pl.cell_ntap_pad * NCH,
                       rows * 28.0 * (double)(pl.Lr + 1) * 8.0);
        hipLaunchKernelGGL(pitch_cell_coef_kernel, dim3((unsigned)n_wg), dim3(256), pl.lds_cell, c.stream, g.ci, g.nc, c.max_frames,
                           (const int*)g.ws.hdr, (const double*)g.ws.rows, pl.rstride, pl.Lr, pl.P.brent_ixmax, c.sinc_cheb,
                           pl.cell_b_lo, pl.cell_n_b, pl.cell_ntap_pad, CELL_CHUNK_FRAMES, n_chunks, g.ws.pc_a);
        RSAF_CHECK_HIP(hipGetLastError());
    }
    const bool low_is_second = pl.dual && pl.P.voicing_thr2 < pl.P.voicing_thr;
    FrameOut* oa = low_is_second ? out2 : out;
    FrameOut* ob = low_is_second ? out : out2;
    ProfScope prof("mshds_pitch_cand_brent", c.stream, 0.0, rows * 15.0 * 2.0 * NCH * 8.0);
    hipLaunchKernelGGL(pitch_brent_kernel, dim3((c.max_frames + BR_FRAMES - 1) / BR_FRAMES, g.nc), dim3(64), 0, c.stream, g.ci,
                       (const int*)g.ws.hdr, (const double*)g.ws.pc_a, (const double*)g.ws.pc_b, c.max_frames, pl.P.brent_ixmax, oa, ob);
    RSAF_CHECK_HIP(hipGetLastError());
    return RSAF_OK;
}

static int launch_paths(const PitchCall& c, const PitchPlan& pl, const PitchOutputs& o, double voicing_thr) {
    const PitchParams& P = pl.P;
    {
        ProfScope prof("mshds_pitch_path", c.stream, 0.0, 0.0);
        hipLaunchKernelGGL(path_kernel, dim3(c.n_clips), dim3(64), 0, c.stream, (const FrameOut*)o.frame_out, c.ci, P.dt,
                           pl.silence_thr, voicing_thr, P.octave_cost, pl.octave_jump, pl.vuv, P.ceiling, o.psi, o.end_state);
        RSAF_CHECK_HIP(hipGetLastError());
        hipLaunchKernelGGL(backtrack_kernel, dim3(c.n_clips), dim3(256), 0, c.stream, (const FrameOut*)o.frame_out, c.ci, o.psi,
                           o.end_state, o.sel_freq, o.sel_strength);
        RSAF_CHECK_HIP(hipGetLastError());
    }
    hipLaunchKernelGGL(pitch_stats_kernel, dim3(c.n_clips), dim3(64), 0, c.stream, o.sel_freq, c.ci, P.ceiling, o.stats);
    RSAF_CHECK_HIP(hipGetLastError());
    return RSAF_OK;
}

static int pitch_run(const PitchCall& c, const double* params_host, const PitchOutputs& o1, const PitchOutputs& o2,
                     double voicing_thr2) {
    PitchPlan pl;
    int rc = pitch_plan(c, params_host, o1, o2, voicing_thr2, &pl);
    if (rc != RSAF_OK || c.n_clips == 0) return rc;
    const double2_t *tw, *tw2;
    if ((rc = pitch_prepare(pl, &tw, &tw2)) != RSAF_OK) return rc;
    FrameOut* out2 = pl.dual ? o2.frame_out : nullptr;
    for (int c0 = 0; c.max_frames > 0 && c0 < c.n_clips; c0 += pl.group) {
        const PitchGroup g = pitch_group(c, pl, c0);
        if ((rc = launch_correlation(c, pl, g, tw, tw2)) != RSAF_OK) return rc;
        if ((rc = launch_candidates(c, pl, g, o1.frame_out, out2)) != RSAF_OK) return rc;
        if (pl.defer && pl.P.debug_stop == 0 && (rc = launch_refinement(c, pl, g, o1.frame_out, out2)) != RSAF_OK) return rc;
    }
    if ((rc = launch_paths(c, pl, o1, pl.P.voicing_thr)) != RSAF_OK) return rc;
    return pl.dual ? launch_paths(c, pl, o2, voicing_thr2) : RSAF_OK;
}

extern "C" {

int rsaf_mshds_frameout_doubles(void) { return (int)(sizeof(FrameOut) / sizeof(double)); }

int64_t rsaf_mshds_pitch_workspace_bytes_per_clip(int max_frames, const double* params_host ) {
    if (!params_host || max_frames < 0) return -1;
    return (int64_t)max_frames * PitchWs::bytes_per_frame(pitch_row_lags(params_host) + 2);
}

int rsaf_mshds_pitch(const float* wav, const void* clip_info, int n_clips, int max_frames, const double* gpeak,
                     const double* window, const double* window_r, const double* params_host ,
                     void* frame_out, unsigned char* psi, int* end_state, double* sel_freq, double* sel_strength, double* stats_out,
                     const double* sinc_cheb, void* workspace, int64_t workspace_bytes, rsaf_stream_t stream) {
    const PitchCall call{wav, (const ClipInfo*)clip_info, n_clips, max_frames, gpeak, window, window_r, sinc_cheb,
                         (double*)workspace, workspace_bytes, (hipStream_t)stream};
    return pitch_run(call, params_host, PitchOutputs{(FrameOut*)frame_out, psi, end_state, sel_freq, sel_strength, stats_out},
                     PitchOutputs{}, -1.0);
}

int rsaf_mshds_pitch_dual(const float* wav, const void* clip_info, int n_clips, int max_frames, const double* gpeak,
                          const double* window, const double* window_r, const double* params_host ,
                          void* frame_out, unsigned char* psi, int* end_state, double* sel_freq, double* sel_strength,
                          double* stats_out, double voicing_threshold2, void* frame_out2, unsigned char* psi2, int* end_state2,
                          double* sel_freq2, double* sel_strength2, double* stats_out2, const double* sinc_cheb,
                          void* workspace, int64_t workspace_bytes, rsaf_stream_t stream) {
    RSAF_CHECK_ARG(voicing_threshold2 >= 0.0, "second voicing threshold must be >= 0");
    const PitchCall call{wav, (const ClipInfo*)clip_info, n_clips, max_frames, gpeak, window, window_r, sinc_cheb,
                         (double*)workspace, workspace_bytes, (hipStream_t)stream};
    return pitch_run(call, params_host, PitchOutputs{(FrameOut*)frame_out, psi, end_state, sel_freq, sel_strength, stats_out},
                     PitchOutputs{(FrameOut*)frame_out2, psi2, end_state2, sel_freq2, sel_strength2, stats_out2},
                     voicing_threshold2);
}

}
```

robust_speech_analysis_framework_amd/csrc/mshds_pitch_layout.h:

```cpp
#pragma once
#include <cstddef>
#include <cstdint>

#if defined(__HIPCC__)
#define PL_HD __host__ __device__ __forceinline__
#else
#define PL_HD inline
#endif

namespace rsaf {
namespace mshds {

constexpr int MAXC = 16;
constexpr int MAX_MAXIMA = 96;
constexpr int NCH = 16;
constexpr int PC_DOUBLES = MAXC * 2 * NCH;
constexpr int CELL_Q = 192;
constexpr int WF_FRAMES = 8;
constexpr int CC_FRAMES_PER_WG = 16;
constexpr int BR_FRAMES = 16;
constexpr int CELL_CHUNK_FRAMES = 4096;

PL_HD void pitch_r_range(int rc, int L, int min_lag, int max_lag, int depth, int* lo, int* hi) {
    const int w = 2 * L + 2, span = w < rc ? w : rc;
    const int lag_lo = min_lag > 2 ? min_lag : 2;
    int lag_hi = max_lag - 1;
    if (lag_hi > rc - 1) lag_hi = rc - 1;
    const int d = depth > 30 ? depth : 30;
    int a = lag_lo - d - 3, b = lag_hi + d + 3;
    *lo = a < -span ? -span : a;
    *hi = b > span ? span : b;
}

constexpr int HDR_A_DEFER = 1, HDR_B_DEFER = 2, HDR_B_COPY = 4;
struct FrameHdr {
    int flags;
    int n_a, n_b;
    int unused0;
    uint16_t lag_a[MAXC];
    uint16_t lag_b[MAXC];
    uint8_t a_slot_of_b[MAXC];
    uint8_t unused1[32];
    PL_HD uint32_t lag_a_pair(int i) const { return reinterpret_cast<const uint32_t*>(lag_a)[i]; }
    PL_HD uint32_t a_slot_of_b_quad(int i) const { return reinterpret_cast<const uint32_t*>(a_slot_of_b)[i]; }
    static PL_HD const FrameHdr* at(const int* records, int64_t frame);
};
static_assert(sizeof(FrameHdr) == 128, "one 128-byte record per frame");
static_assert(offsetof(FrameHdr, flags) == 0 && offsetof(FrameHdr, n_a) == 4 && offsetof(FrameHdr, n_b) == 8, "FrameHdr");
static_assert(offsetof(FrameHdr, lag_a) == 16 && offsetof(FrameHdr, lag_b) == 48 && offsetof(FrameHdr, a_slot_of_b) == 80,
              "FrameHdr");
PL_HD const FrameHdr* FrameHdr::at(const int* records, int64_t frame) {
    return reinterpret_cast<const FrameHdr*>(records + frame * (int64_t)(sizeof(FrameHdr) / sizeof(int)));
}

struct CandLds {
    int r_doubles;
    static constexpr int MFREQ = 0, MSTR = MFREQ + MAX_MAXIMA, MLOC = MSTR + MAX_MAXIMA;
    static constexpr int CF = MLOC + MAX_MAXIMA, CS = CF + MAXC, CLOC = CS + MAXC;
    static constexpr int MAXLAG = 2 * (CLOC + MAXC);
    static constexpr int PLACE = MAXLAG + MAX_MAXIMA, PLACE2 = PLACE + MAXC;
    static constexpr int CNT = PLACE2 + MAXC;
    static constexpr int CNT_NMAX = 0, CNT_NCAND = 1, CNT_NCAND2 = 2, CNT_MISSING = 3, CNT_INTS = 4;
    static_assert((CNT + CNT_INTS) % 2 == 0, "the doubles behind the int arrays stay 8-byte aligned");
    static constexpr int CF2 = (CNT + CNT_INTS) / 2, CS2 = CF2 + MAXC, CLOC2 = CS2 + MAXC;
    static constexpr int PART = CLOC2 + MAXC;
    static constexpr int LIST_DOUBLES = PART + PC_DOUBLES;
    PL_HD CandLds(int r_lo, int r_hi) : r_doubles((r_hi - r_lo + 2) & ~1) {}
    PL_HD double* r_store(char* lds) const { return reinterpret_cast<double*>(lds); }
    PL_HD double* lists(char* lds) const { return r_store(lds) + r_doubles; }
    PL_HD size_t bytes() const { return (size_t)(r_doubles + LIST_DOUBLES) * sizeof(double); }
};

struct CcLds {
    int n_complex, sy_doubles;
    static constexpr int RED = 0;
    static constexpr int VAL = RED + 8;
    static constexpr int SCAN = VAL + 4;
    static constexpr int UNUSED = SCAN + 16;
    static constexpr int SCRATCH_DOUBLES = UNUSED + 4;
    PL_HD CcLds(int N, int L) : n_complex(N), sy_doubles((L + 2) & ~1) {}
    template <class C> PL_HD C* za(char* lds) const {
        static_assert(sizeof(C) == 2 * sizeof(double), "a complex double");
        return reinterpret_cast<C*>(lds);
    }
    template <class C> PL_HD C* zb(char* lds) const { return za<C>(lds) + n_complex; }
    template <class C, int N> PL_HD C* zb(char* lds) const { return za<C>(lds) + N; }
    PL_HD double* sy(char* lds) const { return reinterpret_cast<double*>(lds) + 4 * n_complex; }
    PL_HD double* scratch(char* lds) const { return sy(lds) + sy_doubles; }
    PL_HD size_t bytes() const { return (size_t)(4 * n_complex + sy_doubles + SCRATCH_DOUBLES) * sizeof(double); }
};

struct CcWaveLds {
    int fft_doubles, sy_doubles;
    PL_HD CcWaveLds(int plan_doubles, int L) : fft_doubles(plan_doubles), sy_doubles((L + 3) & ~1) {}
    PL_HD double* fft(char* lds) const { return reinterpret_cast<double*>(lds); }
    PL_HD double* sy(char* lds) const { return fft(lds) + fft_doubles; }
    PL_HD size_t bytes() const { return (size_t)(fft_doubles + sy_doubles) * sizeof(double); }
};

struct CellLds {
    int tab_doubles;
    PL_HD explicit CellLds(int ntap_pad) : tab_doubles(ntap_pad * NCH) {}
    PL_HD double* tab(char* lds) const { return reinterpret_cast<double*>(lds); }
    PL_HD unsigned* queues(char* lds) const { return reinterpret_cast<unsigned*>(tab(lds) + tab_doubles); }
    PL_HD size_t bytes() const { return (size_t)tab_doubles * sizeof(double) + 4 * CELL_Q * sizeof(unsigned); }
};

struct PitchWs {
    double* rows;
    double *pc_a, *pc_b;
    FrameHdr* hdr;
    static PL_HD int64_t bytes_per_frame(int rstride) {
        return (int64_t)rstride * (int64_t)sizeof(double) + 2 * (int64_t)PC_DOUBLES * (int64_t)sizeof(double) + (int64_t)sizeof(FrameHdr);
    }
    PL_HD PitchWs(double* workspace, int64_t frames, int rstride) {
        rows = workspace;
        pc_a = rows + frames * rstride;
        pc_b = pc_a + frames * PC_DOUBLES;
        hdr = reinterpret_cast<FrameHdr*>(pc_b + frames * PC_DOUBLES);
    }
};

}
}
```

robust_speech_analysis_framework_amd/mshds.py:

```python
from __future__ import annotations

import collections
import ctypes as C
import math
import os

import numpy as np

from . import _lib
from .wavio import read_wav_mono_device

FS = 16000.0
DX = 1.0 / FS
SAMPLE_RATE = 16000

FEATURE_NAMES = [
    "Speaking_Rate", "Articulation_Rate", "Phonation_Ratio", "Pause_Rate", "Mean_Pause_Duration",
    "mean_F0", "stdev_F0_Semitone", "mean_dB", "range_ratio_dB", "HNR_dB",
    "Spectral_Slope", "Spectral_Tilt", "Cepstral_Peak_Prominence",
    "mean_F1_Loc", "std_F1_Loc", "mean_B1_Loc", "std_B1_Loc",
    "mean_F2_Loc", "std_F2_Loc", "mean_B2_Loc", "std_B2_Loc",
    "Spectral_Gravity", "Spectral_Std_Dev", "Spectral_Skewness", "Spectral_Kurtosis",
]
BUILT_COLUMNS = [0, 1, 2, 3, 4, 5, 6, 7, 8, 9, 10, 11, 12, 13, 14, 15, 16, 17, 18, 19, 20, 21, 22, 23, 24]

CLIP_INFO = np.dtype([("sample_off", "<i8"), ("frame_off", "<i8"), ("t1", "<f8"),
                      ("n_samples", "<i4"), ("n_frames", "<i4"), ("x1", "<f8"), ("xmax", "<f8")])
assert CLIP_INFO.itemsize == 48
CPP_SEG_FIELDS = ("ix1", "m_in", "m_out", "res_off", "frame_off", "nf", "x1_seg", "x1o", "window", "t1", "nx", "nfft",
                  "work_off", "item_off", "lg")
CPP_SEG = {name: i for i, name in enumerate(CPP_SEG_FIELDS)}
CPP_HDR_FIELDS = ("n_seg", "fail", "total_frames", "total_resampled")
CPP_HDR = {name: i for i, name in enumerate(CPP_HDR_FIELDS)}
CPP_HDR_INTS = len(CPP_HDR_FIELDS)
CPP_NQ_MAX = 513
RESAMPLE_INFO = np.dtype([("sample_off", "<i8"), ("out_off", "<i8"), ("pos0", "<f8"), ("x1o", "<f8"),
                          ("n_in", "<i4"), ("n_out", "<i4"), ("table", "<i4"), ("pad", "<i4")])
assert RESAMPLE_INFO.itemsize == 48
LP_SIG = np.dtype([("in_off", "<i8"), ("out_off", "<i8"), ("work_off", "<i8"), ("n", "<i4"), ("lg", "<i4")])
assert LP_SIG.itemsize == 32
RS_DEPTH = 500
RS_RATE = 10000.0


def resample10k_tables(pos0: float, depth: int = RS_DEPTH):
    k = np.arange(depth)
    sgn = np.where(k % 2 == 0, 1.0, -1.0)
    rows, bs = [], []
    for r in range(5):
        pr = pos0 + 1.6 * r
        b = int(math.floor(pr))
        f = pr - b
        w = np.zeros(2 * depth + 1)
        if f == 0.0:
            w[depth] = 1.0
        else:
            for a0, span, first, step in ((math.pi * f, f + depth, depth, -1), (math.pi * (1.0 - f), depth + 1.0 - f, depth + 1, 1)):
                a = a0 + math.pi * k
                w[first + step * k] = 0.5 * math.sin(a0) * sgn / a * (1.0 + np.cos(a / span))
        rows.append(w)
        bs.append(b)
    return np.stack(rows), bs


def short_term_frames(n_samples: int, window_duration: float, time_step: float, x1: float = 0.5 * DX):
    duration = n_samples * DX
    if window_duration > duration:
        return 0, 0.0
    nf = int(math.floor((duration - window_duration) / time_step)) + 1
    mid = x1 - 0.5 * DX + 0.5 * duration
    t1 = mid - 0.5 * nf * time_step + 0.5 * time_step
    return nf, t1


class SoundDomain:

    def __init__(self, lengths, x1=None, xmax=None):
        self.x1 = [0.5 * DX] * len(lengths) if x1 is None else [float(v) for v in x1]
        self.xmax = [int(n) / FS for n in lengths] if xmax is None else [float(v) for v in xmax]
        assert len(self.x1) == len(lengths) and len(self.xmax) == len(lengths)

    def sub(self, ids):
        return SoundDomain(ids, [self.x1[i] for i in ids], [self.xmax[i] for i in ids])


def _clip_info(sample_offs, lengths, grid, dom=None):
    dom = dom if dom is not None else SoundDomain(lengths)
    ci = np.zeros(len(lengths), dtype=CLIP_INFO)
    off = 0
    for i, (so, n) in enumerate(zip(sample_offs, lengths)):
        nf, t1 = grid(int(n), dom.x1[i])
        ci[i] = (int(so), off, t1, int(n), nf, dom.x1[i], dom.xmax[i])
        off += nf
    return ci, off, int(ci["n_frames"].max()) if len(ci) else 0


def _dev(arr, device, blocking=False):
    import torch
    a = np.ascontiguousarray(arr)
    t = torch.from_numpy(a.view(np.uint8).reshape(-1)) if a.dtype.fields is not None else torch.from_numpy(a)
    if blocking or torch.device(device).type != "cuda" or t.numel() == 0:
        return t.to(device)
    return t.pin_memory().to(device, non_blocking=True)


def sinc_cheb_table(depth: int, ncoef: int = 16):
    d = int(depth)
    n = np.arange(ncoef)
    nodes = np.cos(np.pi * (n + 0.5) / ncoef)
    frac = ((nodes + 1.0) / 2.0)[:, None]
    hs = 0.5 * np.sin(np.pi * frac)
    kk = np.arange(d)[None, :]
    sign = np.where(kk % 2 == 0, 1.0, -1.0)
    a_l = np.pi * (frac + kk)
    w_l = hs * sign / a_l * (1.0 + np.cos(a_l / (d + frac)))
    a_r = np.pi * (1.0 - frac + kk)
    w_r = hs * sign / a_r * (1.0 + np.cos(a_r / (d + 1.0 - frac)))
    w = np.concatenate([w_l[:, ::-1], w_r], axis=1)
    j = np.arange(ncoef)[:, None]
    t = np.cos(np.pi * j * (n[None, :] + 0.5) / ncoef)
    c = (2.0 / ncoef) * (t @ w)
    c[0] *= 0.5
    return np.ascontiguousarray(c.T)


CHEB_CLIP_MAX_DEPTH = 128


def sinc_cheb_tables(depth: int, with_clipped: bool):
    parts = [sinc_cheb_table(depth).reshape(-1)]
    if with_clipped:
        parts += [sinc_cheb_table(e).reshape(-1) for e in range(1, depth)]
    return np.concatenate(parts)


CELL_TABLES_MAX_LDS = 96 * 1024


def sinc_cell_tables(max_lag: int, brent_ixmax: int, min_lag: int, depth: int):
    L, RC = int(max_lag), int(brent_ixmax)
    RN = 2 * RC + 1
    lag_lo, lag_hi = max(int(min_lag), 2), min(L - 1, RC - 1)
    if lag_hi < lag_lo:
        return None
    b_lo, b_hi = RC + lag_lo - 1, RC + lag_hi
    ntap_pad = (L + 1 + 3) & ~3
    if ntap_pad * 16 * 8 + 4 * 192 * 4 > CELL_TABLES_MAX_LDS:
        return None
    out = np.zeros((b_hi - b_lo + 1, ntap_pad, 16))
    m = np.arange(L + 1)
    by_depth = {}
    for b in range(b_lo, b_hi + 1):
        dc = min(int(depth), b + 1, RN - b - 1)
        if dc < 3:
            return None
        if dc not in by_depth:
            by_depth[dc] = sinc_cheb_table(dc)
        tab = by_depth[dc]
        for sign in (1, -1):
            o = RC - b + sign * m
            ok = (o >= -(dc - 1)) & (o <= dc)
            if sign < 0:
                ok &= m > 0
            out[b - b_lo, m[ok]] += tab[o[ok] + dc - 1]
    return out


class _PitchGeom:

    def __init__(self, time_step, floor, ceiling, periods, is_cc):
        self.periods, self.is_cc, self.floor = periods, is_cc, float(floor)
        self.dt = time_step if time_step > 0 else periods / floor / 4.0
        self.ceiling = min(float(ceiling), 0.5 / DX)
        self.dt_window = periods / floor
        self.nsamp_period = int(math.floor(1.0 / DX / floor))
        nsw = int(math.floor(self.dt_window / DX))
        self.half_window = nsw // 2 - 1
        self.nsamp_window = self.half_window * 2
        self.min_lag = max(2, int(math.floor(1.0 / DX / self.ceiling)))
        self.max_lag = min(int(math.floor(self.nsamp_window / periods)) + 2, self.nsamp_window)
        self.brent_ixmax = int(math.floor(self.nsamp_window * (1.0 if is_cc else 0.5)))
        self.frame_window = (1.0 / floor + self.dt_window) if is_cc else self.dt_window

    def grid(self, n, x1=0.5 * DX):
        if self.half_window < 2:
            return 0, 0.0
        return short_term_frames(n, self.frame_window, self.dt, x1)

    def tables(self):
        if self.is_cc:
            return None, None
        n = self.nsamp_window
        i = np.arange(1, n + 1)
        win = 0.5 - 0.5 * np.cos(i * 2.0 * np.pi / (n + 1))
        nfft = 1
        while nfft < n * 1.5:
            nfft *= 2
        sp = np.fft.rfft(win, n=nfft)
        wr = np.fft.irfft(sp.real ** 2 + sp.imag ** 2, n=nfft)
        wr = wr / wr[0]
        return win, wr[:self.brent_ixmax + 1].copy()


def _gaussian_window(n: int):
    i = np.arange(1, n + 1)
    imid, edge = 0.5 * (n + 1), math.exp(-12.0)
    return (np.exp(-48.0 * (i - imid) ** 2 / (n + 1) ** 2) - edge) / (1.0 - edge)


_CppCaps = collections.namedtuple("_CppCaps", "max_seg cap_res cap_frames cap_work lg_max chunk")


def _cpp_caps(max_len: int, chunk_limit: int) -> _CppCaps:
    dur = max_len * DX
    max_seg = int(dur / 0.02) + 2
    cap_res = int(dur * 10000.0) + max_seg + 16
    cap_frames = int(dur / 0.002) + max_seg
    cap_work = int(max_len) + 2000 * max_seg
    lg_max = min(26, max(11, int(max_len + 2000 - 1).bit_length()))
    chunk = max(1, min(chunk_limit, int(3.0e9 // (cap_frames * CPP_NQ_MAX * 8))))
    return _CppCaps(max_seg, cap_res, cap_frames, cap_work, lg_max, chunk)


def lowpass_eligible(lengths):
    cap = int(_lib.load().rsaf_praat_lowpass_max_samples())
    return [int(n) <= cap for n in lengths]


class MshdsEngine:
    def __init__(self, device="cuda"):
        import torch
        _lib.load()
        _lib.require_gpu()
        self.device = torch.device(device)
        self._tables = {}
        self.fo_doubles = _lib.load().rsaf_mshds_frameout_doubles()
        self.n_streams = 3
        self._aux = None

    def _table(self, key, builder):
        if key not in self._tables:
            self._tables[key] = tuple(None if a is None else _dev(np.asarray(a, dtype=np.float64), self.device, blocking=True)
                                      for a in builder())
        return self._tables[key]

    def _pitch_outputs(self, tf, n):
        import torch
        dev = self.device
        return {"frame_out": torch.empty(tf * self.fo_doubles, dtype=torch.float64, device=dev),
                "psi": torch.empty(tf * 16, dtype=torch.uint8, device=dev),
                "end_state": torch.empty(max(n, 1), dtype=torch.int32, device=dev),
                "sel_freq": torch.zeros(tf, dtype=torch.float64, device=dev),
                "sel_strength": torch.zeros(tf, dtype=torch.float64, device=dev),
                "stats": torch.empty((max(n, 1), 8), dtype=torch.float64, device=dev)}

    def pitch(self, wav, sample_offs, lengths, gpeak, *, time_step, floor, ceiling, max_candidates=15,
              silence_threshold=0.03, voicing_threshold=0.45, octave_cost=0.01, octave_jump_cost=0.35,
              voiced_unvoiced_cost=0.14, periods=3.0, is_cc=False, refine_depth=70, voicing_threshold2=None,
              stream=None, dom=None):
        import torch
        lib = _lib.load()
        g = _PitchGeom(time_step, floor, ceiling, periods, is_cc)
        ci, total, mx = _clip_info(sample_offs, lengths, g.grid, dom)
        n = len(lengths)
        dev = self.device
        ci_d = _dev(ci, dev)
        win, wr = self._table(("pitch", g.nsamp_window, is_cc), g.tables)
        tf = max(total, 1)
        first = self._pitch_outputs(tf, n)
        clipped_tables = bool(is_cc) and int(refine_depth) <= CHEB_CLIP_MAX_DEPTH
        table_mode = 1 if clipped_tables else 0
        cheb = None
        if is_cc and not clipped_tables and voicing_threshold2 is None and g.half_window >= 2:
            (cell,) = self._table(("sinc_cell", g.max_lag, g.brent_ixmax, g.min_lag, int(refine_depth)),
                                  lambda: (sinc_cell_tables(g.max_lag, g.brent_ixmax, g.min_lag, int(refine_depth)),))
            if cell is not None:
                table_mode, cheb = 2, cell
        params = (C.c_double * 18)(g.dt, g.floor, g.ceiling, voicing_threshold, octave_cost, silence_threshold,
                                   octave_jump_cost, voiced_unvoiced_cost, g.nsamp_window, g.nsamp_period, g.min_lag,
                                   g.max_lag, g.brent_ixmax, max_candidates, refine_depth, 1 if is_cc else 0,
                                   g.dt_window, table_mode)
        second = None
        if voicing_threshold2 is not None:
            second = {"geom": g, "ci": ci, "ci_dev": ci_d, "total_frames": total, "max_frames": mx, **self._pitch_outputs(tf, n)}
        wp = _lib.ptr(win) if win is not None else None
        wrp = _lib.ptr(wr) if wr is not None else None
        if cheb is None:
            (cheb,) = self._table(("sinc_cheb", int(refine_depth), clipped_tables),
                                  lambda: (sinc_cheb_tables(int(refine_depth), clipped_tables),))
        chp = _lib.ptr(cheb)
        per_clip = int(lib.rsaf_mshds_pitch_workspace_bytes_per_clip(mx, params)) if n else 0
        ws_bytes = max(per_clip * max(1, min(n, int(self.pitch_ws_cap_bytes // max(per_clip, 1)))), 8)
        ws = torch.empty(ws_bytes // 8, dtype=torch.float64, device=dev)
        def ptrs(o):
            return [_lib.ptr(o[k]) for k in first]
        if n and g.half_window >= 2:
            if second is None:
                _lib.check(lib.rsaf_mshds_pitch(
                    _lib.ptr(wav), _lib.ptr(ci_d), n, mx, _lib.ptr(gpeak), wp, wrp, params, *ptrs(first),
                    chp, _lib.ptr(ws), ws_bytes, _lib.stream_ptr(stream)), "rsaf_mshds_pitch")
            else:
                _lib.check(lib.rsaf_mshds_pitch_dual(
                    _lib.ptr(wav), _lib.ptr(ci_d), n, mx, _lib.ptr(gpeak), wp, wrp, params, *ptrs(first),
                    float(voicing_threshold2), *ptrs(second), chp, _lib.ptr(ws), ws_bytes, _lib.stream_ptr(stream)),
                    "rsaf_mshds_pitch_dual")
        else:
            for o in (first, second) if second is not None else (first,):
                o["stats"].fill_(float("nan"))
                o["stats"][:, 0] = 0
        if second is not None:
            second["stats"] = second["stats"][:n]
        return {"geom": g, "ci": ci, "ci_dev": ci_d, "sel_freq": first["sel_freq"], "sel_strength": first["sel_strength"],
                "stats": first["stats"][:n], "frame_out": first["frame_out"], "total_frames": total, "max_frames": mx,
                "second": second}

    def intensity(self, wav, sample_offs, lengths, minimum_pitch, time_step, subtract_mean=True, stream=None, dom=None):
        import torch
        lib = _lib.load()
        phys = 6.4 / minimum_pitch
        dt = time_step if time_step > 0 else 0.8 / minimum_pitch
        half_dur = 0.5 * phys
        half = int(math.floor(half_dur / DX))

        def build():
            i = np.arange(-half, half + 1)
            xx = i * DX / half_dur
            return (np.i0((2.0 * np.pi * np.pi + 0.5) * np.sqrt(np.maximum(0.0, 1.0 - xx * xx))),)
        (win,) = self._table(("intensity", half, minimum_pitch), build)
        ci, total, mx = _clip_info(sample_offs, lengths, lambda n, x1: short_term_frames(n, phys, dt, x1), dom)
        n = len(lengths)
        db = torch.empty(max(total, 1), dtype=torch.float64, device=self.device)
        stats = torch.empty((max(n, 1), 2), dtype=torch.float64, device=self.device)
        if n:
            _lib.check(lib.rsaf_mshds_intensity(_lib.ptr(wav), _lib.ptr(_dev(ci, self.device)), n, mx, _lib.ptr(win),
                                                half, dt, 1 if subtract_mean else 0, _lib.ptr(db), _lib.ptr(stats),
                                                _lib.stream_ptr(stream)), "rsaf_mshds_intensity")
        return {"db": db, "ci": ci, "ci_dev": _dev(ci, self.device), "stats": stats[:n], "dt": dt, "max_frames": mx}

    def speechrate(self, wav, sample_offs, lengths, gpeak, stream=None, dom=None):
        import torch
        lib = _lib.load()
        n = len(lengths)
        inten = self.intensity(wav, sample_offs, lengths, 50.0, 0.016, True, stream, dom)
        p = self.pitch(wav, sample_offs, lengths, gpeak, time_step=0.02, floor=30.0, ceiling=450.0,
                       max_candidates=4, silence_threshold=0.03, voicing_threshold=0.25, octave_cost=0.01,
                       octave_jump_cost=0.35, voiced_unvoiced_cost=0.25, stream=stream, dom=dom)
        out = torch.empty((max(n, 1), 5), dtype=torch.float64, device=self.device)
        if n:
            wsd = int(lib.rsaf_mshds_speechrate_workspace_doubles(inten["max_frames"]))
            ws = torch.empty(n * wsd, dtype=torch.float64, device=self.device)
            _lib.check(lib.rsaf_mshds_speechrate(_lib.ptr(inten["db"]), _lib.ptr(inten["ci_dev"]), n, inten["max_frames"],
                                                 inten["dt"], _lib.ptr(p["sel_freq"]), _lib.ptr(p["ci_dev"]),
                                                 p["geom"].dt, p["geom"].ceiling, _lib.ptr(ws), _lib.ptr(out),
                                                 _lib.stream_ptr(stream)), "rsaf_mshds_speechrate")
        return out[:n]

    def spectral_moments(self, wav, sample_offs, lengths, pitch, window_length=0.025, time_step=0.005,
                         maximum_frequency=5000.0, frequency_step=20.0, stream=None, dom=None):
        import torch
        lib = _lib.load()
        nyq = 0.5 / DX
        phys = 2.0 * window_length
        eff_t = window_length / math.sqrt(math.pi)
        tstep = max(time_step, eff_t / 8.0)
        fstep = max(frequency_step, (1.0 / eff_t) / 8.0)
        nsamp = int(math.floor(phys / DX))
        half = nsamp // 2 - 1
        nsamp = half * 2
        fmax = maximum_frequency if 0 < maximum_frequency <= nyq else nyq
        nfreq = int(math.floor(fmax / fstep))
        nfft = 1
        while nfft < nsamp or nfft < 2 * nfreq * (nyq / fmax):
            nfft *= 2
        bw_samples = max(1, int(math.floor(fstep * DX * nfft)))
        if bw_samples != 1:
            raise _lib.RsafError("spectrogram: only one FFT bin per frequency band is implemented")
        fstep = 1.0 / (DX * nfft)
        nfreq = int(math.floor(fmax / fstep))

        def build():
            i = np.arange(1, nsamp + 1)
            phase = (i - 0.5 * (nsamp + 1)) / nsamp
            edge = math.exp(-12.0)
            win = (np.exp(-48.0 * phase * phase) - edge) / (1.0 - edge)
            k = np.arange(nfft)
            tw = np.stack([np.cos(2.0 * np.pi * k / nfft), -np.sin(2.0 * np.pi * k / nfft)], axis=1)
            return win, tw.reshape(-1)
        win, tw = self._table(("spec", nsamp, nfft), build)

        def grid(n, x1):
            duration = n * DX
            if phys > duration or half < 1:
                return 0, 0.0
            nt = 1 + int(math.floor((duration - phys) / tstep))
            return nt, x1 + 0.5 * ((n - 1) * DX - (nt - 1) * tstep)
        ci, total, mx = _clip_info(sample_offs, lengths, grid, dom)
        n = len(lengths)
        mom = torch.empty(max(total, 1) * 5, dtype=torch.float64, device=self.device)
        stats = torch.empty((max(n, 1), 4), dtype=torch.float64, device=self.device)
        if n:
            _lib.check(lib.rsaf_mshds_spectral_moments(
                _lib.ptr(wav), _lib.ptr(_dev(ci, self.device)), _lib.ptr(pitch["ci_dev"]), n, mx,
                _lib.ptr(pitch["sel_freq"]), pitch["geom"].dt, pitch["geom"].ceiling, _lib.ptr(win), _lib.ptr(tw),
                nsamp, nfft, nfreq, tstep, fstep, _lib.ptr(mom), _lib.ptr(stats), _lib.stream_ptr(stream)),
                "rsaf_mshds_spectral_moments")
        return {"stats": stats[:n], "moments": mom, "ci": ci, "fstep": fstep, "tstep": tstep}

    def formants(self, wav, sample_offs, lengths, gpeak, floor, ceiling, frame_shift=0.005, stream=None, dom=None):
        import torch
        lib = _lib.load()
        n = len(lengths)
        dev = self.device
        dom = dom if dom is not None else SoundDomain(lengths)
        ok = lowpass_eligible(lengths)
        if not all(ok):
            out = torch.full((n, 8), float("nan"), dtype=torch.float64, device=dev)
            ids = [i for i in range(n) if ok[i]]
            if ids:
                sub = self.formants(wav, [sample_offs[i] for i in ids], [lengths[i] for i in ids],
                                    gpeak[_dev(np.asarray(ids, dtype=np.int64), dev)].contiguous(), floor, ceiling, frame_shift,
                                    stream, dom.sub(ids))
                out[_dev(np.asarray(ids, dtype=np.int64), dev)] = sub
            return out
        dxo = 1.0 / RS_RATE
        ratio = RS_RATE / FS
        ri = np.zeros(n, dtype=RESAMPLE_INFO)
        lps = np.zeros(n, dtype=LP_SIG)
        tabs, bases, key_to_table = [], [], {}
        out_off = work_off = 0
        for i, (so, nn) in enumerate(zip(sample_offs, lengths)):
            m = int(math.floor(dom.xmax[i] * RS_RATE + 0.5))
            x1o = 0.5 * (dom.xmax[i] - (m - 1) / RS_RATE)
            pos0 = (x1o - dom.x1[i]) / DX
            if pos0 not in key_to_table:
                key_to_table[pos0] = len(tabs)
                rows, bs = resample10k_tables(pos0)
                tabs.append(rows)
                bases.append(bs)
            ri[i] = (int(so), out_off, pos0, x1o, int(nn), m, key_to_table[pos0], 0)
            lg = max(11, int(nn + 2000 - 1).bit_length())
            lps[i] = (int(so), int(so), work_off, int(nn), lg)
            out_off += m
            work_off += 1 << (lg - 1)
        max_out = int(ri["n_out"].max()) if n else 0
        y10 = torch.empty(max(out_off, 1), dtype=torch.float64, device=dev)
        out = torch.full((max(n, 1), 8), float("nan"), dtype=torch.float64, device=dev)
        if n == 0:
            return out[:0]
        ri_d = _dev(ri, dev)
        wstride = int(lib.rsaf_mshds_resample10k_table_stride(RS_DEPTH))
        tab = np.zeros((len(tabs), 5, wstride))
        tab[:, :, :2 * RS_DEPTH + 1] = np.stack(tabs)
        tab_d = _dev(tab.reshape(-1), dev)
        base_d = _dev(np.asarray(bases, dtype=np.int32).reshape(-1), dev)
        lp = torch.empty(int(wav.numel()), dtype=torch.float64, device=dev)
        work = torch.empty(2 * work_off, dtype=torch.float64, device=dev)
        _lib.check(lib.rsaf_praat_lowpass_batch(_lib.ptr(wav), _lib.ptr(_dev(lps, dev)), n, int(lps["lg"].max()), RS_RATE * DX,
                                                _lib.ptr(work), work_off, _lib.ptr(lp), _lib.stream_ptr(stream)),
                   "rsaf_praat_lowpass_batch")
        _lib.check(lib.rsaf_mshds_resample10k(_lib.ptr(lp), _lib.ptr(ri_d), n, max_out, _lib.ptr(tab_d), wstride, _lib.ptr(base_d),
                                              RS_DEPTH, _lib.ptr(y10), _lib.stream_ptr(stream)), "rsaf_mshds_resample10k")
        del work
        dt_window = 0.05
        nsw = int(math.floor(dt_window / dxo))

        (win,) = self._table(("formant", nsw), lambda: (_gaussian_window(nsw),))
        ci = np.zeros(n, dtype=CLIP_INFO)
        foff = 0
        for i in range(n):
            m, x1o = int(ri[i]["n_out"]), float(ri[i]["x1o"])
            duration = m * dxo
            if dt_window > duration:
                nf, t1 = 0, 0.0
            else:
                nf = int(math.floor((duration - dt_window) / frame_shift)) + 1
                t1 = x1o - 0.5 * dxo + 0.5 * duration - 0.5 * nf * frame_shift + 0.5 * frame_shift
            ci[i] = (int(ri[i]["out_off"]), foff, t1, m, nf, x1o, dom.xmax[i])
            foff += nf
        mxf = int(ci["n_frames"].max())
        frames = torch.empty(max(foff, 1) * 10, dtype=torch.float64, device=dev)
        ci_d = _dev(ci, dev)
        _lib.check(lib.rsaf_mshds_formants(_lib.ptr(y10), _lib.ptr(ri_d), _lib.ptr(ci_d), n, mxf, _lib.ptr(win), nsw,
                                           frame_shift, dxo, math.exp(-2.0 * math.pi * 50.0 * dxo), _lib.ptr(frames),
                                           _lib.stream_ptr(stream)), "rsaf_mshds_formants")
        p = self.pitch(wav, sample_offs, lengths, gpeak, time_step=frame_shift, floor=floor, ceiling=ceiling,
                       periods=1.0, is_cc=True, refine_depth=70, stream=stream, dom=dom)
        pulses, npul, max_pulses = self.pulses(wav, lengths, p, stream)
        _lib.check(lib.rsaf_mshds_formant_stats(_lib.ptr(frames), _lib.ptr(ci_d), n, frame_shift, _lib.ptr(pulses),
                                                max_pulses, _lib.ptr(npul), _lib.ptr(out), _lib.stream_ptr(stream)),
                   "rsaf_mshds_formant_stats")
        self._last_formants = {"frames": frames, "ci": ci, "pulses": pulses, "n_pulses": npul, "max_pulses": max_pulses,
                               "y10": y10, "ri": ri, "pitch": p}
        return out[:n]

    def pulses(self, wav, lengths, pitch, stream=None):
        import torch
        n = len(lengths)
        ceiling = pitch["geom"].ceiling
        max_pulses = int(max(lengths) * DX * ceiling * 1.5) + 16
        pulses = torch.empty(max(n, 1) * max_pulses, dtype=torch.float64, device=self.device)
        npul = torch.zeros(max(n, 1), dtype=torch.int32, device=self.device)
        if n:
            lib = _lib.load()
            mx = int(pitch["max_frames"])
            need = int(lib.rsaf_mshds_pulses_workspace_bytes(n, mx, pitch["geom"].dt, ceiling))
            ws = torch.empty((need + 7) // 8, dtype=torch.float64, device=self.device)
            _lib.check(lib.rsaf_mshds_pulses(_lib.ptr(wav), _lib.ptr(pitch["ci_dev"]), n, mx, _lib.ptr(pitch["sel_freq"]),
                                             pitch["geom"].dt, ceiling, _lib.ptr(ws), need, _lib.ptr(pulses), max_pulses,
                                             _lib.ptr(npul), _lib.stream_ptr(stream)), "rsaf_mshds_pulses")
        return pulses, npul, max_pulses

    def slope_tilt(self, wav, sample_offs, lengths, gpeak, floor, ceiling, stream=None, dom=None):
        import torch
        n = len(lengths)
        out = torch.full((max(n, 1), 2), float("nan"), dtype=torch.float64, device=self.device)
        if n == 0:
            return out[:0]
        p = self.pitch(wav, sample_offs, lengths, gpeak, time_step=0.0, floor=floor, ceiling=ceiling, stream=stream, dom=dom)
        pulses, npul, max_pulses = self.pulses(wav, lengths, p, stream)
        _lib.check(_lib.load().rsaf_mshds_ltas_slope_tilt(_lib.ptr(wav), _lib.ptr(p["ci_dev"]), n, _lib.ptr(pulses),
                                                          max_pulses, _lib.ptr(npul), 0.0001, 0.02, 1.3, _lib.ptr(out),
                                                          _lib.stream_ptr(stream)), "rsaf_mshds_ltas_slope_tilt")
        self._last_ltas = {"pitch": p, "pulses": pulses, "n_pulses": npul, "max_pulses": max_pulses}
        return out[:n]

    pitch_ws_cap_bytes = 16.0e9
    CPP_CHUNK = 48

    def cpp(self, wav, sample_offs, lengths, gpeak, floor, ceiling, frame_shift=0.005, stream=None, pitch=None, dom=None):
        import torch
        lib = _lib.load()
        n = len(lengths)
        dev = self.device
        out = torch.full((max(n, 1),), float("nan"), dtype=torch.float64, device=dev)
        if n == 0:
            return out[:0]
        p = pitch if pitch is not None else self.pitch(wav, sample_offs, lengths, gpeak, time_step=frame_shift, floor=floor,
                                                       ceiling=ceiling, voicing_threshold=0.3, stream=stream, dom=dom)
        pulses, npul, max_pulses = self.pulses(wav, lengths, p, stream)

        def build_tw():
            k = np.arange(512)
            return (np.stack([np.cos(2.0 * np.pi * k / 1024.0), -np.sin(2.0 * np.pi * k / 1024.0)], axis=1).reshape(-1),)
        (win,) = self._table(("cpp_window", 1000), lambda: (_gaussian_window(1000),))
        (tw,) = self._table(("cpp_twiddle", 1024), build_tw)
        max_seg, cap_res, cap_frames, cap_work, lg_max, chunk = _cpp_caps(max(lengths), self.CPP_CHUNK)
        segd = int(lib.rsaf_mshds_cpp_seg_doubles())
        ci_all = p["ci"]
        for c0 in range(0, n, chunk):
            c1 = min(n, c0 + chunk)
            m = c1 - c0
            ci_d = _dev(ci_all[c0:c1], dev)
            segs = torch.empty(m * max_seg * segd, dtype=torch.float64, device=dev)
            hdr = torch.zeros(m * CPP_HDR_INTS, dtype=torch.int32, device=dev)
            res = torch.empty(m * cap_res, dtype=torch.float64, device=dev)
            ceps = torch.empty(m * cap_frames * CPP_NQ_MAX, dtype=torch.float64, device=dev)
            cppf = torch.empty(m * cap_frames, dtype=torch.float64, device=dev)
            lp_origin = int(min(int(r["sample_off"]) for r in ci_all[c0:c1]))
            lp_end = int(max(int(r["sample_off"]) + int(r["n_samples"]) for r in ci_all[c0:c1]))
            lp = torch.empty(max(lp_end - lp_origin, 1), dtype=torch.float64, device=dev)
            lpw = torch.empty(m * cap_work * 2, dtype=torch.float64, device=dev)
            _lib.check(lib.rsaf_mshds_cpp(_lib.ptr(wav), _lib.ptr(ci_d), m, _lib.c_void_p_off(pulses, c0 * max_pulses),
                                          max_pulses, _lib.c_void_p_off(npul, c0), _lib.ptr(win), _lib.ptr(tw), max_seg,
                                          cap_res, cap_frames, _lib.ptr(segs), _lib.ptr(hdr), _lib.ptr(res), _lib.ptr(ceps),
                                          _lib.ptr(cppf), _lib.ptr(lp), lp_origin, _lib.ptr(lpw), cap_work, lg_max,
                                          _lib.c_void_p_off(out, c0), _lib.stream_ptr(stream)),
                       "rsaf_mshds_cpp")
            self._last_cpp = {"segs": segs, "hdr": hdr, "res": res, "ceps": ceps, "cpp_frames": cppf, "max_seg": max_seg,
                              "cap_res": cap_res, "cap_frames": cap_frames, "seg_doubles": segd, "pulses": pulses,
                              "n_pulses": npul, "max_pulses": max_pulses, "chunk": (c0, c1)}
        return out[:n]

    def hnr_mean(self, pitch_cc, stream=None):
        import torch
        n = len(pitch_cc["ci"])
        out = torch.empty(max(n, 1), dtype=torch.float64, device=self.device)
        if n:
            _lib.check(_lib.load().rsaf_mshds_hnr_mean(_lib.ptr(pitch_cc["sel_freq"]), _lib.ptr(pitch_cc["sel_strength"]),
                                                       _lib.ptr(pitch_cc["ci_dev"]), n, _lib.ptr(out),
                                                       _lib.stream_ptr(stream)), "rsaf_mshds_hnr_mean")
        return out[:n]

    def clip_peaks(self, wav, sample_offs, lengths, stream=None):
        import torch
        n = len(lengths)
        ci, _, _ = _clip_info(sample_offs, lengths, lambda k, x1: (0, 0.0))
        gp = torch.zeros(max(n, 1), dtype=torch.float64, device=self.device)
        if n:
            _lib.check(_lib.load().rsaf_mshds_clip_peak(_lib.ptr(wav), _lib.ptr(_dev(ci, self.device)), n, _lib.ptr(gp),
                                                        _lib.stream_ptr(stream)), "rsaf_mshds_clip_peak")
        return gp

    def extract_packed(self, wav, sample_offs, lengths, stream=None, x1=None, xmax=None, before_host_sync=None):
        import torch
        n = len(lengths)
        out = torch.full((n, 25), float("nan"), dtype=torch.float64, device=self.device)
        if n == 0:
            return out, []
        sample_offs = [int(v) for v in sample_offs]
        lengths = [int(v) for v in lengths]
        dom = SoundDomain(lengths, x1, xmax)
        gpeak = self.clip_peaks(wav, sample_offs, lengths, stream)
        two = stream is None and self.n_streams > 1
        main = torch.cuda.current_stream(self.device) if two else None
        if two and self._aux is None:
            self._aux = [torch.cuda.Stream(device=self.device) for _ in range(2)]
        three = two and self.n_streams > 2

        def side(fn, which=0):
            if not two:
                return fn()
            aux = self._aux[which if three else 0]
            aux.wait_stream(main)
            with torch.cuda.stream(aux):
                return fn()

        def join(*tensors):
            if two:
                for aux in self._aux[:2 if three else 1]:
                    main.wait_stream(aux)
                for t in tensors:
                    t.record_stream(main)

        sr = side(lambda: self.speechrate(wav, sample_offs, lengths, gpeak, stream, dom))
        wide = self.pitch(wav, sample_offs, lengths, gpeak, time_step=0.005, floor=50.0, ceiling=600.0, stream=stream, dom=dom)
        if before_host_sync is not None:
            before_host_sync()
        st = wide["stats"].cpu().numpy()
        join(sr)
        out[:, 0:5] = sr
        ranges = []
        for i in range(n):
            if st[i, 0] == 0 or not st[i, 7] > 0:
                ranges.append((75, 500))
            else:
                ranges.append((60, 250) if st[i, 3] < 170 else (100, 500))
        for rng in sorted(set(ranges)):
            ids = [i for i in range(n) if ranges[i] == rng]
            so = [sample_offs[i] for i in ids]
            ln = [lengths[i] for i in ids]
            dm = dom.sub(ids)
            idx = _dev(np.asarray(ids, dtype=np.int64), self.device)
            gp = gpeak[idx].contiguous()
            floor, ceiling = float(rng[0]), float(rng[1])

            def branch_hnr():
                inten = self.intensity(wav, so, ln, floor, 0.005, True, stream, dm)
                cc = self.pitch(wav, so, ln, gp, time_step=0.005, floor=floor, ceiling=0.5 / DX, max_candidates=15,
                                silence_threshold=0.1, voicing_threshold=0.0, octave_cost=0.0, octave_jump_cost=0.0,
                                voiced_unvoiced_cost=0.0, periods=4.5, is_cc=True, refine_depth=700, stream=stream, dom=dm)
                return inten["stats"], self.hnr_mean(cc, stream)

            def branch_pulses():
                fm = self.formants(wav, so, ln, gp, floor, ceiling, 0.005, stream, dm)
                return fm, self.slope_tilt(wav, so, ln, gp, floor, ceiling, stream, dm)

            i_stats, hnr = side(branch_hnr, 0)
            fm, sl = side(branch_pulses, 1)
            p = self.pitch(wav, so, ln, gp, time_step=0.005, floor=floor, ceiling=ceiling, voicing_threshold2=0.3,
                           stream=stream, dom=dm)
            sm = self.spectral_moments(wav, so, ln, p, 0.025, 0.005, stream=stream, dom=dm)
            cppv = self.cpp(wav, so, ln, gp, floor, ceiling, 0.005, stream, pitch=p["second"], dom=dm)
            join(i_stats, hnr, fm, sl)
            out[idx, 5] = p["stats"][:, 5]
            out[idx, 6] = p["stats"][:, 6]
            out[idx, 7] = i_stats[:, 0]
            out[idx, 8] = i_stats[:, 1]
            out[idx, 9] = hnr
            out[idx, 10:12] = sl
            out[idx, 12] = cppv
            out[idx, 13:21] = fm
            out[idx, 21:25] = sm["stats"]
        return out, ranges


_ENGINE = None


def get_engine(device="cuda"):
    global _ENGINE
    if _ENGINE is None:
        _ENGINE = MshdsEngine(device)
    return _ENGINE


def extract_mshds_features(input_df, audio_file_column="filepath", verbose=True, batch_files=64):
    import pandas as pd
    import torch
    eng = get_engine()
    rows = []
    paths = list(input_df[audio_file_column])
    for b0 in range(0, len(paths), batch_files):
        batch = paths[b0:b0 + batch_files]
        clips, ok_idx, x1s, xmaxs = [], [], [], []
        for j, pth in enumerate(batch):
            filename = os.path.basename(pth)
            try:
                x, fs, n_in = read_wav_mono_device(pth, device=eng.device)
                x1, xmax = 0.5 / fs, int(x.numel()) / fs
                if fs != SAMPLE_RATE:
                    from .resample import resample_praat_sound
                    x, x1, xmax = resample_praat_sound(x, fs, SAMPLE_RATE, 50, device=eng.device)
                if int(x.numel()) == 0:
                    raise ValueError("empty file")
                clips.append(x)
                ok_idx.append(j)
                x1s.append(x1)
                xmaxs.append(xmax)
            except Exception as e:
                if verbose:
                    print(f"ERROR processing file '{filename}': {e}. Appending NaNs.")
        feats = np.full((len(batch), 25), np.nan)
        if clips:
            lengths = [int(c.numel()) for c in clips]
            offs = np.zeros(len(clips) + 1, dtype=np.int64)
            offs[1:] = np.cumsum(lengths)
            wav = torch.cat(clips) if len(clips) > 1 else clips[0].contiguous()
            try:
                vals, _ = eng.extract_packed(wav, offs[:-1], lengths, x1=x1s, xmax=xmaxs)
                torch.cuda.synchronize()
                feats[ok_idx] = vals.cpu().numpy()
            except _lib.RsafError as e:
                if verbose:
                    print(f"WARNING: batch of {len(clips)} files failed ({e}); retrying file by file.")
                for k, (j, c) in enumerate(zip(ok_idx, clips)):
                    try:
                        v1, _ = eng.extract_packed(c.contiguous(), [0], [int(c.numel())], x1=x1s[k:k + 1], xmax=xmaxs[k:k + 1])
                        torch.cuda.synchronize()
                        feats[j] = v1.cpu().numpy()[0]
                    except _lib.RsafError as e1:
                        if verbose:
                            print(f"ERROR processing file '{os.path.basename(batch[j])}': {e1}. Appending NaNs.")
        for j, pth in enumerate(batch):
            d = {"filename": os.path.basename(pth)}
            d.update({nme: feats[j, k] for k, nme in enumerate(FEATURE_NAMES)})
            rows.append(d)
    return pd.DataFrame(rows)
```

robust_speech_analysis_framework_amd/pipeline.py:

```python
from __future__ import annotations

import numpy as np

from . import _lib, smile

BUILT_STAGES = ["mshds", "smile", "w2v2", "cnnlstm"]

SMILE_LLD_BYTES_PER_AUDIO_S = 16000 * 4 + 38 * 8 * 100
LDS_PEAK_GBS = 256 * 128 * 2.4
LATENCY_FAMILIES = {
    "mshds_pitch_path": "Viterbi over <= 15 candidates, one wave per clip",
    "smile_viterbi": "Viterbi over 7 states, one wave per clip",
    "lstm_recurrent": "persistent bi-LSTM recurrence",
}
F16_MFMA_PEAK_TFLOPS = 2500.0
SPLIT_PRODUCTS = 3


def resolve_stages(spec: str):
    if spec in ("all", ""):
        return list(BUILT_STAGES)
    st = [s.strip() for s in spec.split(",") if s.strip()]
    for s in st:
        if s not in BUILT_STAGES:
            raise ValueError(f"stage '{s}' is not built (built: {BUILT_STAGES})")
    if "cnnlstm" in st and "w2v2" not in st:
        raise ValueError("stage 'cnnlstm' consumes the output of stage 'w2v2'")
    return st


class Pipeline:
    def __init__(self, stages, device, seconds: float, w2v2_seed: int = 0, cnnlstm_seed: int = 0,
                 w2v2_chunks_per_call: int = 256, overlap: bool = True):
        import torch
        _lib.load()
        self.stages = list(stages)
        self.device = device
        self.seconds = seconds
        self._packed = None
        self._packed_key = None
        self.finite_cols = None
        self.last_frames = None
        self.w2v2 = None
        self.model = None
        self.mshds = None
        self.overlap = overlap and "mshds" in self.stages and "w2v2" in self.stages
        self._aux = torch.cuda.Stream(device=device) if self.overlap else None
        self._pool = None
        if self.overlap:
            from concurrent.futures import ThreadPoolExecutor
            self._pool = ThreadPoolExecutor(max_workers=1, thread_name_prefix="rsaf-mshds")
        if "mshds" in self.stages:
            from .mshds import MshdsEngine
            self.mshds = MshdsEngine(device)
        if "w2v2" in self.stages:
            from .w2v2 import W2V2Engine
            from .w2v2_config import W2V2Config, random_state_dict
            cfg = W2V2Config()
            self.w2v2 = W2V2Engine(cfg, random_state_dict(cfg, w2v2_seed), device,
                                   max_chunks_per_call=w2v2_chunks_per_call)
        if "cnnlstm" in self.stages:
            from .cnnlstm import CNNLSTM
            torch.manual_seed(cnnlstm_seed)
            self.model = CNNLSTM().to(device).eval()

    def _pack(self, wav):
        key = (wav.data_ptr(), tuple(wav.shape))
        if self._packed_key != key:
            self._packed = smile.pack_clips(wav, device=self.device)
            self._packed_key = key
        return self._packed

    def run(self, wav, only=None):
        import torch
        if only is not None:
            keep = (self.stages, self.mshds, self.w2v2, self.model, self.overlap)
            self.stages = [s for s in self.stages if s in only]
            self.mshds = self.mshds if "mshds" in only else None
            self.w2v2 = self.w2v2 if "w2v2" in only else None
            self.model = self.model if "cnnlstm" in only else None
            self.overlap = False
            try:
                return self.run(wav)
            finally:
                self.stages, self.mshds, self.w2v2, self.model, self.overlap = keep
        cols = []
        p = self._pack(wav)
        n_clips, n_samp = int(wav.shape[0]), int(wav.shape[1])
        main = torch.cuda.current_stream()
        mshds_cols = None
        smile_cols = None
        if self.mshds is not None and not self.overlap:
            offs = np.arange(n_clips, dtype=np.int64) * n_samp
            hold = {}

            def _smile_now():
                if "smile" in self.stages:
                    hold["cols"] = smile.smile_features(p).to(torch.float32)
            feats, _ = self.mshds.extract_packed(p.wav, offs, [n_samp] * n_clips, before_host_sync=_smile_now)
            mshds_cols = feats.to(torch.float32)
            smile_cols = hold.get("cols")
        fut = None
        if self.overlap:
            self._aux.wait_stream(main)

            def _mshds_job():
                torch.cuda.set_device(self.device)
                with torch.cuda.stream(self._aux):
                    offs_ = np.arange(n_clips, dtype=np.int64) * n_samp
                    feats_, _ = self.mshds.extract_packed(p.wav, offs_, [n_samp] * n_clips)
                    return feats_.to(torch.float32)
            fut = self._pool.submit(_mshds_job)
        if self.mshds is not None and not self.overlap:
            cols.append(mshds_cols)
        if "smile" in self.stages:
            cols.append(smile_cols if smile_cols is not None else smile.smile_features(p).to(torch.float32))
        if self.w2v2 is not None:
            offs = np.arange(n_clips, dtype=np.int64) * n_samp
            seq, frame_off = self.w2v2.extract_packed(p.wav, offs, [n_samp] * n_clips)
            frames = int(frame_off[1]) if n_clips else 0
            self.last_frames = frames
            if self.model is not None:
                logits = self.model(seq.view(n_clips, frames, self.w2v2.cfg.hidden_size))
                cols.append(logits)
            cols.append(torch.full((n_clips, 1), float(frames), dtype=torch.float32, device=self.device))
        if self.overlap:
            mshds_cols = fut.result()
            main.wait_stream(self._aux)
            mshds_cols.record_stream(main)
            cols.insert(0, mshds_cols)
        rows = cols[0] if len(cols) == 1 else torch.cat(cols, dim=1)
        if self.finite_cols is None:
            self.finite_cols = torch.isfinite(rows[0]).nonzero().flatten()
        return rows

    def describe(self, clips, seconds):
        parts = []
        if "mshds" in self.stages:
            parts.append("MSHDS Praat-style 25/25 features (speech rate, pitch, intensity, HNR, LTAS slope/tilt, CPPS, formants, spectral moments; fp64)")
        if "smile" in self.stages:
            parts.append("openSMILE-style 38/38 LLD (incl. SHS pitch + Viterbi, jitter / shimmer / logHNR) + 912 functionals")
        if "w2v2" in self.stages:
            parts.append("Wav2Vec2-base frame embeddings (5 s windows / 4 s hop, fp32, seeded random weights)")
        if "cnnlstm" in self.stages:
            parts.append("CNN-LSTM-attn forward (C=H=128) on the Wav2Vec2 sequences")
        return f"{' -> '.join(parts)} on {clips} x {seconds:g} s synthetic 16 kHz mono clips per GPU"


def rooflines(prof, stages, clips, seconds, steps, hbm_peak_gbs, mfma_f32_peak_tflops, f64_peak_tflops, wall_ms=None,
              frames_per_launch=None):
    out = []
    for name, rec in sorted(prof.items(), key=lambda kv: -kv[1]["ms"]):
        if rec["launches"] <= 0 or rec["ms"] <= 0:
            continue
        avg_ms = rec["ms"] / rec["launches"]
        base = {"kernel": name, "avg_launch_ms": round(avg_ms, 4), "launches": rec["launches"], "traffic": None,
                "share_of_step_wall": round(rec["ms"] / wall_ms, 4) if wall_ms else None}
        if name in LATENCY_FAMILIES and name != "lstm_recurrent":
            r = {**base, "bound": "latency", "what": LATENCY_FAMILIES[name]}
            if frames_per_launch and frames_per_launch.get(name):
                r["steps_per_launch"] = int(frames_per_launch[name])
                r["us_per_step"] = round(1e3 * avg_ms / frames_per_launch[name], 3)
            out.append(r)
            continue
        if name in ("mshds_pitch_ac_fft", "mshds_pitch_cc_fft"):
            per_launch = rec["bytes"] / rec["launches"]
            lds = per_launch / (avg_ms * 1e-3) / 1e9
            tf = rec["flops"] / (rec["ms"] * 1e-3) / 1e12
            out.append({**base, "bound": "fp64_vector", "achieved": round(tf, 3), "peak": f64_peak_tflops, "unit": "TFLOP/s",
                        "frac": round(tf / f64_peak_tflops, 4), "algorithmic_flops_per_launch": rec["flops"] / rec["launches"],
                        "lds_gbs": round(lds, 1), "lds_frac_of_peak": round(lds / LDS_PEAK_GBS, 4),
                        "algorithmic_lds_bytes_per_launch": per_launch,
                        "note": "FLOPs = 5 S log2 S per complex transform + ~30 per point of the spectrum step (real operations, an "
                                "FMA counts two); LDS bytes = the two exchanges of each transform (16 B x S written and read) + the "
                                "paired spectrum step; phase timing: profiles/r03/pitch_phase_r03.txt"})
            continue
        if rec["flops"] > 0:
            fp64 = name.startswith("mshds_")
            split3 = name in ("w2v2_gemm", "w2v2_posconv_gemm")
            peak = f64_peak_tflops if fp64 else (F16_MFMA_PEAK_TFLOPS if split3 else mfma_f32_peak_tflops)
            alg = rec["flops"] / (rec["ms"] * 1e-3) / 1e12
            ach = SPLIT_PRODUCTS * alg if split3 else alg
            r = {**base, "bound": "mfma", "achieved": round(ach, 3), "peak": peak, "unit": "TFLOP/s", "frac": round(ach / peak, 4),
                 "arithmetic": ("f64 (v_mfma_f64_16x16x4_f64 issues at the fp64 vector rate)" if fp64 else
                                ("fp32-accurate result from 3 fp16 MFMA products of two-way operand splits (power-of-two row "
                                 "scales), fp32 accumulation; rounds 2-3 needed 6 bf16 products for the same result"
                                 if split3 else "f32 MFMA")),
                 "algorithmic_flops_per_launch": rec["flops"] / rec["launches"]}
            if split3:
                r["fp32_equivalent_tflops"] = round(alg, 3)
                r["fp32_equivalent_over_fp32_mfma_peak"] = round(alg / mfma_f32_peak_tflops, 4)
                r["executed_products_per_multiply_add"] = SPLIT_PRODUCTS
            if name == "lstm_recurrent":
                r["note"] = "latency-bound persistent recurrence: the figure that matters is the time per step"
            out.append(r)
        elif name == "smile_lld":
            per_launch = SMILE_LLD_BYTES_PER_AUDIO_S * clips * seconds * steps / rec["launches"]
            ach = per_launch / (avg_ms * 1e-3) / 1e9
            out.append({**base, "bound": "hbm", "achieved": round(ach, 2), "peak": hbm_peak_gbs, "unit": "GB/s",
                        "frac": round(ach / hbm_peak_gbs, 5), "algorithmic_bytes_per_launch": per_launch,
                        "note": "SURVEY.md 8d assigns HBM (64 000 B read + 30 400 B of float64 LLD rows written per audio-second); the "
                                "kernel is float64 since round 3 (every decision of the chain coincides with the oracle) and is "
                                "bound by fp64 issue + LDS round trips at 2 waves / SIMD: profiles/r03/smile_phase.txt, DESIGN.md"})
        elif rec["bytes"] > 0:
            per_launch = rec["bytes"] / rec["launches"]
            ach = per_launch / (avg_ms * 1e-3) / 1e9
            out.append({**base, "bound": "hbm", "achieved": round(ach, 2), "peak": hbm_peak_gbs, "unit": "GB/s",
                        "frac": round(ach / hbm_peak_gbs, 5), "algorithmic_bytes_per_launch": per_launch})
    return out


def c2_level_roofline(prof_one, clips, seconds, wall_s, hbm_peak_gbs, f64_peak_tflops):
    audio_s = clips * seconds
    flops = sum(v["flops"] for k, v in prof_one.items() if k.startswith("mshds") and v["flops"] > 0)
    counted = sorted(k for k, v in prof_one.items() if k.startswith("mshds") and v["flops"] > 0)
    tf = flops / wall_s / 1e12
    hbm = 64000.0 * audio_s / wall_s / 1e9
    return {"kernel": "C2 (MSHDS + openSMILE-style) as a whole, one-stream pass", "wall_ms": round(1e3 * wall_s, 3),
            "bound": "fp64_vector", "achieved": round(tf, 3), "peak": f64_peak_tflops, "unit": "TFLOP/s",
            "frac": round(tf / f64_peak_tflops, 4), "algorithmic_fp64_flops": flops, "families_counted": counted,
            "families_not_counted": "Brent iterations, path finder, pulse walker, Burg / root finder, CPPS, intensity, "
                                    "openSMILE-style chain (latency- or issue-bound, no closed FLOP count)",
            "survey_8d_hbm_reading": {"bytes_per_audio_s": 64000, "achieved_GBs": round(hbm, 2), "peak_GBs": hbm_peak_gbs,
                                      "frac": round(hbm / hbm_peak_gbs, 6),
                                      "note": "the stage reads each sample a few dozen times from L2 / LDS and computes in fp64: "
                                              "the HBM roof SURVEY.md assigned is not what bounds it"}}
```

Before: 12640.

## Fuse pitch correlation and candidate kernels so rows stay in LDS

Adds a fused pitch path where each wave, after computing a frame's autocorrelation or cross-correlation FFT row, keeps that row in LDS and runs the candidate search in the same wave. The separate candidate kernel launch and the HBM round-trip of the per-frame correlation row are removed. The two-kernel path is still available through a flag. The candidate code now synchronises per wave instead of per block, and the LDS footprint becomes the larger of the two phases, which may lower occupancy and serialises the candidate work behind the FFT work within each wave.

```diff
diff --git a/robust_speech_analysis_framework_amd/csrc/mshds_pitch.hip b/robust_speech_analysis_framework_amd/csrc/mshds_pitch.hip
--- a/robust_speech_analysis_framework_amd/csrc/mshds_pitch.hip
+++ b/robust_speech_analysis_framework_amd/csrc/mshds_pitch.hip
@@ -18,6 +18,7 @@
     int nfft;
     double voicing_thr2;
     int debug_stop;
+    int two_kernel;
 };
 
 struct FrameOut {
@@ -332,6 +333,40 @@
     }
 }
 
+struct DeferArgs {
+    FrameHdr* hdr;
+    double* pc_a;
+    double* pc_b;
+    int grouped;
+};
+struct CandArgs {
+    FrameOut* out;
+    FrameOut* out2;
+    const double* cheb;
+    DeferArgs DA;
+};
+__device__ __forceinline__ void cand_write_stopped(FrameOut* o, int tid);
+template <bool ROW_IN_LDS>
+__device__ __forceinline__ void cand_frame(char* smem_raw, const int tid, const ClipInfo& c, const int clip, const int f, const double* __restrict__ gpeak,
+                                           const PitchParams& P, const double* __restrict__ rbuf, int rstride, double intensity_in,
+                                           int max_frames, FrameOut* __restrict__ out, FrameOut* __restrict__ out2,
+                                           const double* __restrict__ cheb, const DeferArgs& DA);
+struct CandRowSink { double* r; int lo, hi; };
+__device__ __forceinline__ CandRowSink cand_row_sink(char* smem_raw, const PitchParams& P, int L) {
+    int r_lo, r_hi;
+    pitch_r_range(P.brent_ixmax, L, P.min_lag, P.max_lag, P.refine_depth, &r_lo, &r_hi);
+    return CandRowSink{CandLds(r_lo, r_hi).r_store(smem_raw) - r_lo, r_lo, r_hi};
+}
+__device__ __forceinline__ void cand_row_put(const CandRowSink& S, int l, double v) {
+    if (l <= S.hi) S.r[l] = v;
+    if (-l >= S.lo) S.r[-l] = v;
+}
+__device__ __forceinline__ void cand_row_begin(const CandRowSink& S, int lane, int L) {
+    if (lane == 0) S.r[0] = 1.0;
+    for (int k = L + 1 + lane; k <= S.hi; k += 64) S.r[k] = 0.0;
+    for (int k = -(L + 1) - lane; k >= S.lo; k -= 64) S.r[k] = 0.0;
+}
+
 
 __device__ __forceinline__ wfft::cplx ld_tw(const double2_t* __restrict__ tw, int i) {
     const double2_t w = tw[i];
@@ -353,14 +388,13 @@
     return v + (row == 0 ? 0.0 : (row == 1 ? t0 : (row == 2 ? t0 + t1 : (t0 + t1) + t2)));
 }
 
-template <int R>
-__global__ __launch_bounds__(64, R == 32 ? 2 : (R == 16 ? 3 : 4)) void pitch_ac_wave_kernel(const float* __restrict__ wav, const ClipInfo* __restrict__ ci,
-                                                           const double* __restrict__ gpeak, const double* __restrict__ win,
-                                                           const double* __restrict__ wr, const PitchParams P,
-                                                           const double2_t* __restrict__ tw, double* __restrict__ rbuf,
-                                                           int rstride, int max_frames) {
+template <int R, bool FUSED>
+__device__ __forceinline__ void pitch_ac_wave_frames(char* smem_raw, const float* __restrict__ wav, const ClipInfo* __restrict__ ci,
+                                                     const double* __restrict__ gpeak, const double* __restrict__ win,
+                                                     const double* __restrict__ wr, const PitchParams& P,
+                                                     const double2_t* __restrict__ tw, double* __restrict__ rbuf,
+                                                     int rstride, int max_frames, const CandArgs& CA) {
     using namespace wfft;
-    extern __shared__ __attribute__((aligned(16))) char smem_raw[];
     double* lds = reinterpret_cast<double*>(smem_raw);
     const ClipInfo c = ci[blockIdx.y];
     const int f0 = blockIdx.x * WF_FRAMES;
@@ -376,12 +410,13 @@
     int pa = P.half_window - P.half_period, pb = P.half_window + P.half_period;
     pa = pa < 0 ? 0 : pa;
     pb = pb > nw ? nw : pb;
+    const CandRowSink SR = cand_row_sink(smem_raw, P, L);
 #pragma unroll 1
     for (int f = f0; f < f1; ++f) {
         int lane = lane_;
         asm volatile("" : "+v"(lane));
         cplx w_s = ld_tw(tw, 2 * lane), w_b = ld_tw(tw, (lane % L2) * (N / 64));
-        double* rb = rbuf + ((int64_t)blockIdx.y * max_frames + f) * rstride;
+        double* rb = FUSED ? nullptr : rbuf + ((int64_t)blockIdx.y * max_frames + f) * rstride;
         const double t = c.t1 + f * P.dt;
         const int left = (int)low_index(t, c.x1), right = left + 1;
         const int start = right - P.half_window;
@@ -445,7 +480,7 @@
         }
         const double local_peak = wave_max_dpp(pk);
         const double intensity = gp > 0.0 ? (local_peak > gp ? 1.0 : local_peak / gp) : 0.0;
-        if (P.debug_stop == 1) continue;
+        if (P.debug_stop == 1) { if (FUSED) cand_write_stopped(CA.out + c.frame_off + f, lane_); continue; }
         wave_fft<R>(v, lds, lane, w_s, w_b);
         {
             ac_spec_store<R>(v, mem, lane);
@@ -459,9 +494,10 @@
         w_s = ld_tw(tw, 2 * lane);
         w_b = ld_tw(tw, (lane % L2) * (N / 64));
         wave_fft<R>(v, lds, lane, w_s, w_b);
-        if (P.debug_stop == 2) continue;
+        if (P.debug_stop == 2) { if (FUSED) cand_write_stopped(CA.out + c.frame_off + f, lane_); continue; }
         const double r0 = readlane_f64(v[0].x, 0);
-        if (lane == 0) { rb[0] = 1.0; rb[L + 1] = intensity; }
+        if (FUSED) { wave_sync(); cand_row_begin(SR, lane, L); }
+        else if (lane == 0) { rb[0] = 1.0; rb[L + 1] = intensity; }
         double wa[8], wb[8];
 #pragma unroll
         for (int m = 0; m < 8; ++m) {
@@ -473,19 +509,48 @@
         for (int m = 0; m < 8; ++m) {
             const int l0 = 2 * (lane + 64 * m);
             if (128 * m > L) break;
-            if (l0 >= 1 && l0 <= L) rb[l0] = r0 > 0.0 ? v[m].x * fast_rcp(r0 * wa[m]) : 0.0;
-            if (l0 + 1 <= L) rb[l0 + 1] = r0 > 0.0 ? -v[m].y * fast_rcp(r0 * wb[m]) : 0.0;
+            if (l0 >= 1 && l0 <= L) {
+                const double q = r0 > 0.0 ? v[m].x * fast_rcp(r0 * wa[m]) : 0.0;
+                if (FUSED) cand_row_put(SR, l0, q); else rb[l0] = q;
+            }
+            if (l0 + 1 <= L) {
+                const double q = r0 > 0.0 ? -v[m].y * fast_rcp(r0 * wb[m]) : 0.0;
+                if (FUSED) cand_row_put(SR, l0 + 1, q); else rb[l0 + 1] = q;
+            }
+        }
+        if (FUSED) {
+            asm volatile("" : "+v"(lane));
+            cand_frame<true>(smem_raw, lane, c, blockIdx.y, f, gpeak, P, nullptr, 0, intensity, max_frames, CA.out, CA.out2, CA.cheb, CA.DA);
+            wave_sync();
         }
     }
 }
 
 template <int R>
-__global__ __launch_bounds__(64, R == 32 ? 2 : 3) void pitch_cc_wave_kernel(const float* __restrict__ wav, const ClipInfo* __restrict__ ci,
-                                                           const double* __restrict__ gpeak, const PitchParams P,
+__global__ __launch_bounds__(64, R == 32 ? 2 : (R == 16 ? 3 : 4)) void pitch_ac_wave_kernel(const float* __restrict__ wav, const ClipInfo* __restrict__ ci,
+                                                           const double* __restrict__ gpeak, const double* __restrict__ win,
+                                                           const double* __restrict__ wr, const PitchParams P,
                                                            const double2_t* __restrict__ tw, double* __restrict__ rbuf,
                                                            int rstride, int max_frames) {
+    extern __shared__ __attribute__((aligned(16))) char smem_raw[];
+    pitch_ac_wave_frames<R, false>(smem_raw, wav, ci, gpeak, win, wr, P, tw, rbuf, rstride, max_frames, CandArgs{});
+}
+
+template <int R>
+__global__ __launch_bounds__(64, R == 32 ? 2 : 3) void pitch_ac_cand_kernel(const float* __restrict__ wav, const ClipInfo* __restrict__ ci,
+                                                           const double* __restrict__ gpeak, const double* __restrict__ win,
+                                                           const double* __restrict__ wr, const PitchParams P,
+                                                           const double2_t* __restrict__ tw, int max_frames, const CandArgs CA) {
+    extern __shared__ __attribute__((aligned(16))) char smem_raw[];
+    pitch_ac_wave_frames<R, true>(smem_raw, wav, ci, gpeak, win, wr, P, tw, nullptr, 0, max_frames, CA);
+}
+
+template <int R, bool FUSED>
+__device__ __forceinline__ void pitch_cc_wave_frames(char* smem_raw, const float* __restrict__ wav, const ClipInfo* __restrict__ ci,
+                                                     const double* __restrict__ gpeak, const PitchParams& P,
+                                                     const double2_t* __restrict__ tw, double* __restrict__ rbuf,
+                                                     int rstride, int max_frames, const CandArgs& CA) {
     using namespace wfft;
-    extern __shared__ __attribute__((aligned(16))) char smem_raw[];
     const int nw = P.nsamp_window, L = P.max_lag;
     const CcWaveLds lay(Plan<R>::LDS_DOUBLES, L);
     double* lds = lay.fft(smem_raw);
@@ -504,11 +569,12 @@
     int pa = P.half_window - P.half_period, pb = P.half_window + P.half_period;
     pa = pa < 0 ? 0 : pa;
     pb = pb > nw ? nw : pb;
+    const CandRowSink SR = cand_row_sink(smem_raw, P, L);
 #pragma unroll 1
     for (int f = f0; f < f1; ++f) {
         int lane = lane_;
         asm volatile("" : "+v"(lane));
-        double* rb = rbuf + ((int64_t)blockIdx.y * max_frames + f) * rstride;
+        double* rb = FUSED ? nullptr : rbuf + ((int64_t)blockIdx.y * max_frames + f) * rstride;
         const double t = c.t1 + f * P.dt;
         const int left = (int)low_index(t, c.x1), right = left + 1;
         const double start_time = t - 0.5 * (1.0 / P.min_pitch + P.dt_window);
@@ -586,7 +652,7 @@
                 carry += readlane_f64(sc, 63);
             }
         }
-        if (P.debug_stop == 1) continue;
+        if (P.debug_stop == 1) { if (FUSED) { cand_write_stopped(CA.out + c.frame_off + f, lane_); wave_sync(); } continue; }
         const cplx w_s1 = ld_tw(tw, lane);
         wave_fft<R>(v, lds, lane, w_s1, ld_tw(tw, (lane % L2) * R));
         cplx y[H];
@@ -597,8 +663,8 @@
         cc_spec_load<R>(y, mem, lane, y_half);
         wave_sync();
         wave_fft<H>(y, lds, lane, ld_tw(tw, 2 * lane), ld_tw(tw, (lane % L2H) * R));
-        if (P.debug_stop == 2) continue;
-        if (lane == 0) { rb[0] = 1.0; rb[L + 1] = intensity; }
+        if (P.debug_stop == 2) { if (FUSED) { cand_write_stopped(CA.out + c.frame_off + f, lane_); wave_sync(); } continue; }
+        if (!FUSED && lane == 0) { rb[0] = 1.0; rb[L + 1] = intensity; }
         const double inv_n = 1.0 / (double)S;
         constexpr int MO = H < 8 ? H : 8;
         double ya[MO], yb[MO];
@@ -608,30 +674,48 @@
             ya[m] = s_sy[l0 < L ? l0 : L];
             yb[m] = s_sy[l0 + 1 < L ? l0 + 1 : L];
         }
+        if (FUSED) { wave_sync(); cand_row_begin(SR, lane, L); }
 #pragma unroll
         for (int m = 0; m < MO; ++m) {
             const int l0 = 2 * (lane + 64 * m);
             if (128 * m > L) break;
             if (l0 >= 1 && l0 <= L) {
                 const double den = sumx2 * ya[m];
-                rb[l0] = (l0 <= loc_max_lag && den > 0.0) ? (y[m].x * inv_n) * fast_rsqrt(den) : 0.0;
+                const double q = (l0 <= loc_max_lag && den > 0.0) ? (y[m].x * inv_n) * fast_rsqrt(den) : 0.0;
+                if (FUSED) cand_row_put(SR, l0, q); else rb[l0] = q;
             }
             if (l0 + 1 <= L) {
                 const double den = sumx2 * yb[m];
-                rb[l0 + 1] = (l0 + 1 <= loc_max_lag && den > 0.0) ? (-y[m].y * inv_n) * fast_rsqrt(den) : 0.0;
-            }
+                const double q = (l0 + 1 <= loc_max_lag && den > 0.0) ? (-y[m].y * inv_n) * fast_rsqrt(den) : 0.0;
+                if (FUSED) cand_row_put(SR, l0 + 1, q); else rb[l0 + 1] = q;
+            }
+        }
+        if (FUSED) {
+            asm volatile("" : "+v"(lane));
+            cand_frame<true>(smem_raw, lane, c, blockIdx.y, f, gpeak, P, nullptr, 0, intensity, max_frames, CA.out, CA.out2, CA.cheb, CA.DA);
         }
         wave_sync();
     }
 }
 
+template <int R>
+__global__ __launch_bounds__(64, R == 32 ? 2 : 3) void pitch_cc_wave_kernel(const float* __restrict__ wav, const ClipInfo* __restrict__ ci,
+                                                           const double* __restrict__ gpeak, const PitchParams P,
+                                                           const double2_t* __restrict__ tw, double* __restrict__ rbuf,
+                                                           int rstride, int max_frames) {
+    extern __shared__ __attribute__((aligned(16))) char smem_raw[];
+    pitch_cc_wave_frames<R, false>(smem_raw, wav, ci, gpeak, P, tw, rbuf, rstride, max_frames, CandArgs{});
+}
+
+template <int R>
+__global__ __launch_bounds__(64, R == 32 ? 2 : 3) void pitch_cc_cand_kernel(const float* __restrict__ wav, const ClipInfo* __restrict__ ci,
+                                                           const double* __restrict__ gpeak, const PitchParams P,
+                                                           const double2_t* __restrict__ tw, int max_frames, const CandArgs CA) {
+    extern __shared__ __attribute__((aligned(16))) char smem_raw[];
+    pitch_cc_wave_frames<R, true>(smem_raw, wav, ci, gpeak, P, tw, nullptr, 0, max_frames, CA);
+}
+
 constexpr int CT = 64;
-struct DeferArgs {
-    FrameHdr* hdr;
-    double* pc_a;
-    double* pc_b;
-    int grouped;
-};
 struct CandCtx {
     const PitchParams& P;
     const DeferArgs& DA;
@@ -938,6 +1022,8 @@
     }
 }
 
+__device__ __forceinline__ void cand_sync() { wfft::wave_sync(); }
+
 __device__ __forceinline__ bool cand_hand_over_or_brent(const CandCtx& X, int nc, const int* place_lag, double* cf, double* cs,
                                                         double* pc_out) {
     const DeferArgs& DA = X.DA;
@@ -945,7 +1031,7 @@
     const double* s_P = X.s_part;
     if (DA.hdr) {
         for (int i = 2 * NCH + tid; i < nc * 2 * NCH; i += CT) pc_out[i] = s_P[i];
-        __syncthreads();
+        cand_sync();
         return true;
     }
     if (tid < 64) {
@@ -956,7 +1042,7 @@
         if (ym > 1.0) ym = 1.0 / ym;
         if (live) { cf[k] = 1.0 / DXS / (xm - RC); cs[k] = ym; }
     }
-    __syncthreads();
+    cand_sync();
     return false;
 }
 
@@ -970,7 +1056,7 @@
     if (nref <= 4) { if (span >= 6 * 64) refine_candidates<64, true>(A, tid, CT); else refine_candidates<64, false>(A, tid, CT); }
     else if (nref <= 8) { if (span >= 6 * 32) refine_candidates<32, true>(A, tid, CT); else refine_candidates<32, false>(A, tid, CT); }
     else { if (span >= 6 * 16) refine_candidates<16, true>(A, tid, CT); else refine_candidates<16, false>(A, tid, CT); }
-    __syncthreads();
+    cand_sync();
 }
 
 __device__ __forceinline__ bool cand_refine_list(const CandCtx& X, int nc, const int* place_lag, double* cf, double* cs,
@@ -985,7 +1071,7 @@
             cand_coef_16x16x4(X, nc, place_lag, C);
             if (C.n_clip_cols > 0) cand_coef_clipped_cells(X, nc, place_lag);
         }
-        __syncthreads();
+        cand_sync();
         if (X.P.debug_stop == 6) return true;
         return cand_hand_over_or_brent(X, nc, place_lag, cf, cs, pc_out);
     }
@@ -1018,16 +1104,17 @@
     }
 }
 
-__global__ __launch_bounds__(64) void pitch_cand_kernel(const ClipInfo* __restrict__ ci, const double* __restrict__ gpeak,
-                                                        const PitchParams P, const double* __restrict__ rbuf, int rstride,
-                                                        int max_frames, FrameOut* __restrict__ out,
-                                                        FrameOut* __restrict__ out2, const double* __restrict__ cheb,
-                                                        const DeferArgs DA) {
-    extern __shared__ __attribute__((aligned(16))) char smem_raw[];
-    const ClipInfo c = ci[blockIdx.y];
-    const int f = blockIdx.x;
-    if (f >= c.n_frames) return;
-    const int tid = threadIdx.x, lane = tid & 63;
+__device__ __forceinline__ void cand_write_stopped(FrameOut* o, int tid) {
+    if (tid == 0) { o->intensity = 0.0; o->ncand = 1.0; }
+    if (tid < MAXC) { o->freq[tid] = 0.0; o->strength[tid] = 0.0; }
+}
+
+template <bool ROW_IN_LDS>
+__device__ __forceinline__ void cand_frame(char* smem_raw, const int tid, const ClipInfo& c, const int clip, const int f, const double* __restrict__ gpeak,
+                                           const PitchParams& P, const double* __restrict__ rbuf, int rstride, double intensity_in,
+                                           int max_frames, FrameOut* __restrict__ out, FrameOut* __restrict__ out2,
+                                           const double* __restrict__ cheb, const DeferArgs& DA) {
+    const int lane = tid & 63;
     const int L = P.is_cc ? P.max_lag : P.brent_ixmax;
     const int RC = P.brent_ixmax;
     const int RN = 2 * P.brent_ixmax + 1;
@@ -1057,35 +1144,37 @@
     FrameOut* o = out + c.frame_off + f;
 #define RSAF_PITCH_DBG_STOP(k)                                                                       \
     if (P.debug_stop == (k)) {                                                                       \
-        if (tid == 0) { o->intensity = 0.0; o->ncand = 1.0; }                                        \
-        if (tid < MAXC) { o->freq[tid] = 0.0; o->strength[tid] = 0.0; }                              \
+        cand_write_stopped(o, tid);                                                                  \
         return;                                                                                      \
     }
-    RSAF_PITCH_DBG_STOP(1)
-    RSAF_PITCH_DBG_STOP(2)
-    const double* rb = rbuf + ((int64_t)blockIdx.y * max_frames + f) * rstride;
-    const double intensity = rb[L + 1];
-    const double gp = gpeak[blockIdx.y];
-    cand_load_row(X, rb, r_lo, r_hi);
+    double intensity = intensity_in;
+    if (!ROW_IN_LDS) {
+        RSAF_PITCH_DBG_STOP(1)
+        RSAF_PITCH_DBG_STOP(2)
+        const double* rb = rbuf + ((int64_t)clip * max_frames + f) * rstride;
+        intensity = rb[L + 1];
+        cand_load_row(X, rb, r_lo, r_hi);
+    }
+    const double gp = gpeak[clip];
     if (tid == 0) s_cnt[CandLds::CNT_NMAX] = 0;
-    __syncthreads();
+    cand_sync();
     const bool dual = out2 != nullptr && P.voicing_thr2 >= 0.0;
     const double thr_low = dual && P.voicing_thr2 < P.voicing_thr ? P.voicing_thr2 : P.voicing_thr;
     cand_collect_maxima(X, thr_low);
-    __syncthreads();
+    cand_sync();
     RSAF_PITCH_DBG_STOP(3)
     const int nmax = s_cnt[CandLds::CNT_NMAX];
     cand_first_estimates(X, nmax);
-    __syncthreads();
+    cand_sync();
     RSAF_PITCH_DBG_STOP(4)
     const CandMaxima M{lane < nmax ? s_mloc[lane] : 0.0, lane + 64 < nmax ? s_mloc[lane + 64] : 0.0,
                        lane < nmax ? r[RC + s_maxlag[lane]] : -1.0, lane + 64 < nmax ? r[RC + s_maxlag[lane + 64]] : -1.0};
     cand_build_list(X, M, P.voicing_thr, s_cf, s_cs, s_cloc, s_place, &s_cnt[CandLds::CNT_NCAND]);
     if (dual) cand_build_list(X, M, P.voicing_thr2, s_cf2, s_cs2, s_cloc2, s_place2, &s_cnt[CandLds::CNT_NCAND2]);
-    __syncthreads();
+    cand_sync();
     const int ncand = s_cnt[CandLds::CNT_NCAND];
     RSAF_PITCH_DBG_STOP(5)
-    const int64_t wframe = (int64_t)blockIdx.y * max_frames + f;
+    const int64_t wframe = (int64_t)clip * max_frames + f;
     FrameHdr* hdr = DA.hdr ? DA.hdr + wframe : nullptr;
     int flags = 0;
     if (!dual) {
@@ -1100,7 +1189,7 @@
         const bool def_a = cand_refine_list(X, nc_a, pl_a, cf_a, cs_a, DA.pc_a ? DA.pc_a + wframe * PC_DOUBLES : nullptr);
         if (def_a) flags |= HDR_A_DEFER;
         if (tid == 0) s_cnt[CandLds::CNT_MISSING] = 0;
-        __syncthreads();
+        cand_sync();
         int hit = 0;
         {
             const int pa_reg = tid < MAXC ? pl_a[tid] : 0;
@@ -1110,12 +1199,12 @@
                 if (hit) { if (!def_a) { cf_b[tid] = cf_a[hit]; cs_b[tid] = cs_a[hit]; } } else atomicAdd(&s_cnt[CandLds::CNT_MISSING], 1);
             }
         }
-        __syncthreads();
+        cand_sync();
         if (s_cnt[CandLds::CNT_MISSING] > 0) {
             if (tid >= 1 && tid < nc_b) {
                 for (int m = 0; m < nmax; ++m) if (s_maxlag[m] == pl_b[tid]) { cf_b[tid] = s_mfreq[m]; cs_b[tid] = s_mstr[m]; }
             }
-            __syncthreads();
+            cand_sync();
             if (cand_refine_list(X, nc_b, pl_b, cf_b, cs_b, DA.pc_b ? DA.pc_b + wframe * PC_DOUBLES : nullptr)) flags |= HDR_B_DEFER;
         } else if (def_a) {
             flags |= HDR_B_COPY;
@@ -1126,6 +1215,18 @@
     cand_write_frame_out(o, tid, intensity, gp, ncand, s_cf, s_cs);
 }
 #undef RSAF_PITCH_DBG_STOP
+
+__global__ __launch_bounds__(64) void pitch_cand_kernel(const ClipInfo* __restrict__ ci, const double* __restrict__ gpeak,
+                                                        const PitchParams P, const double* __restrict__ rbuf, int rstride,
+                                                        int max_frames, FrameOut* __restrict__ out,
+                                                        FrameOut* __restrict__ out2, const double* __restrict__ cheb,
+                                                        const DeferArgs DA) {
+    extern __shared__ __attribute__((aligned(16))) char smem_raw[];
+    const ClipInfo c = ci[blockIdx.y];
+    const int f = blockIdx.x;
+    if (f >= c.n_frames) return;
+    cand_frame<false>(smem_raw, threadIdx.x, c, blockIdx.y, f, gpeak, P, rbuf, rstride, 0.0, max_frames, out, out2, cheb, DA);
+}
 
 __global__ __launch_bounds__(256) void pitch_cell_coef_kernel(const ClipInfo* __restrict__ ci, int n_clips, int max_frames,
                                                               const int* __restrict__ hdr, const double* __restrict__ rbuf,
@@ -1550,8 +1651,50 @@
     PS_DT_WINDOW,
     PS_TABLE_MODE,
 };
+constexpr int PS_TWO_KERNEL = 16, PS_FUSE_ALL = 32;
 
 static int pitch_row_lags(const double* h) { return (int)h[PS_IS_CC] ? (int)h[PS_MAX_LAG] : (int)h[PS_BRENT_IXMAX]; }
+
+struct PitchShape {
+    int nfft, ncc;
+    int wave_r;
+    bool unclipped;
+    bool fused;
+    size_t lds_fused;
+};
+static PitchShape pitch_shape(const double* h) {
+    PitchShape sh;
+    const int nw = (int)h[PS_NSAMP_WINDOW], max_lag = (int)h[PS_MAX_LAG], ixmax = (int)h[PS_BRENT_IXMAX], min_lag = (int)h[PS_MIN_LAG];
+    const int depth = (int)h[PS_REFINE_DEPTH], mode = (int)h[PS_TABLE_MODE];
+    const bool is_cc = (int)h[PS_IS_CC] != 0;
+    sh.nfft = 1;
+    while ((double)sh.nfft < (double)nw * 1.5 && sh.nfft < (1 << 30)) sh.nfft *= 2;
+    if (sh.nfft < 16) sh.nfft = 16;
+    sh.ncc = 64;
+    while (sh.ncc < nw + max_lag + 1 && sh.ncc < (1 << 30)) sh.ncc *= 2;
+    int log2m = 0, log2n = 0;
+    while ((2 << log2m) < sh.nfft) ++log2m;
+    while ((1 << log2n) < sh.ncc) ++log2n;
+    sh.wave_r = 0;
+    if (!is_cc) sh.wave_r = log2m <= 9 ? 8 : (log2m <= 11 ? 1 << (log2m - 6) : 0);
+    else if (log2n <= 11) sh.wave_r = log2n <= 10 ? 16 : 32;
+    const int cell_lag_lo = min_lag > 2 ? min_lag : 2, cell_lag_hi = std::min(max_lag - 1, ixmax - 1);
+    sh.unclipped = ixmax + cell_lag_lo - 1 >= depth && cell_lag_hi + 2 + depth <= ixmax;
+    sh.fused = false;
+    sh.lds_fused = 0;
+    const int tmode = mode & (PS_TWO_KERNEL - 1);
+    if (sh.wave_r && !(mode & PS_TWO_KERNEL) && (!is_cc || (mode & PS_FUSE_ALL)) && (tmode == 0 || tmode == 1) &&
+        (sh.unclipped || tmode == 1)) {
+        const int Lr = pitch_row_lags(h);
+        int r_lo, r_hi;
+        pitch_r_range(ixmax, Lr, min_lag, max_lag, depth, &r_lo, &r_hi);
+        const int plan = sh.wave_r == 8 ? wfft::Plan<8>::LDS_DOUBLES : sh.wave_r == 16 ? wfft::Plan<16>::LDS_DOUBLES : wfft::Plan<32>::LDS_DOUBLES;
+        sh.lds_fused = FusedLds(plan, is_cc, Lr, r_lo, r_hi).bytes();
+        sh.fused = sh.lds_fused <= 48 * 1024;
+    }
+    return sh;
+}
+
 
 struct PitchCall {
     const float* wav;
@@ -1577,6 +1720,9 @@
     double silence_thr, octave_jump, vuv;
     bool dual;
     int seg_len, Lr, rstride;
+    bool fused;
+    int ws_rstride;
+    size_t lds_fused;
     int ncc, log2m, log2n;
     int wave_r;
     size_t lds_corr, lds_cand, lds_cell;
@@ -1611,7 +1757,8 @@
     P.min_lag = (int)h[PS_MIN_LAG]; P.max_lag = (int)h[PS_MAX_LAG]; P.brent_ixmax = (int)h[PS_BRENT_IXMAX];
     P.max_cand = (int)h[PS_MAX_CAND]; P.refine_depth = (int)h[PS_REFINE_DEPTH]; P.is_cc = (int)h[PS_IS_CC];
     P.dt_window = h[PS_DT_WINDOW];
-    const int table_mode = (int)h[PS_TABLE_MODE];
+    const int table_mode = (int)h[PS_TABLE_MODE] & (PS_TWO_KERNEL - 1);
+    P.two_kernel = ((int)h[PS_TABLE_MODE] & PS_TWO_KERNEL) ? 1 : 0;
     P.cheb_clipped = table_mode == 1 ? 1 : 0;
     P.voicing_thr2 = dual ? voicing_thr2 : -1.0;
     { const char* e = getenv("RSAF_PITCH_STOP"); P.debug_stop = e ? atoi(e) : 0; }
@@ -1621,15 +1768,13 @@
     RSAF_CHECK_ARG(P.nsamp_window >= 4 && P.brent_ixmax >= 2 && P.max_lag >= 2, "window too short");
     RSAF_CHECK_ARG(P.is_cc || (c.window && c.window_r), "AC needs the window tables");
     RSAF_CHECK_ARG((P.is_cc ? P.max_lag : P.brent_ixmax) <= 1023, "more than 1023 lags (pitch floor below ~16 Hz) is not supported");
-    P.nfft = 1;
-    while ((double)P.nfft < (double)P.nsamp_window * 1.5) P.nfft *= 2;
-    if (P.nfft < 16) P.nfft = 16;
+    const PitchShape sh = pitch_shape(h);
+    P.nfft = sh.nfft;
     RSAF_CHECK_ARG(P.is_cc || P.nsamp_window + P.brent_ixmax <= P.nfft, "brent_ixmax must not exceed half the analysis window");
     const int seg_len = pl.seg_len = P.is_cc ? P.nsamp_window + P.max_lag + 1 : P.nsamp_window;
     const int Lr = pl.Lr = pitch_row_lags(h);
     pl.rstride = Lr + 2;
-    int ncc = 64;
-    while (ncc < seg_len) ncc *= 2;
+    int ncc = sh.ncc;
     RSAF_CHECK_ARG(!P.is_cc || ncc <= 4096, "cross-correlation window + lag range longer than 4 095 samples is not supported");
     RSAF_CHECK_ARG(P.is_cc || P.nfft <= 4096, "autocorrelation window longer than 2 730 samples is not supported");
     pl.lds_corr = P.is_cc ? CcLds(ncc, Lr).bytes() : 0;
@@ -1639,7 +1784,14 @@
     pitch_r_range(P.brent_ixmax, Lr, P.min_lag, P.max_lag, pl.grouped ? 30 : P.refine_depth, &r_lo_h, &r_hi_h);
     pl.lds_cand = CandLds(r_lo_h, r_hi_h).bytes();
     RSAF_CHECK_ARG(pl.lds_corr <= 150 * 1024 && pl.lds_cand <= 150 * 1024, "analysis window too long for LDS");
-    const int64_t row_bytes_per_clip = (int64_t)max_frames * PitchWs::bytes_per_frame(pl.rstride);
+    pl.cheb = table_mode == 2 ? nullptr : c.sinc_cheb;
+    P.cheb_all_full = sh.unclipped ? 1 : 0;
+    if (pl.cheb == nullptr) P.cheb_clipped = 0;
+    if (!sh.unclipped && !P.cheb_clipped) pl.cheb = nullptr;
+    pl.fused = sh.fused && pl.cheb != nullptr && !pl.grouped;
+    pl.lds_fused = sh.lds_fused;
+    pl.ws_rstride = pl.fused ? 0 : pl.rstride;
+    const int64_t row_bytes_per_clip = (int64_t)max_frames * PitchWs::bytes_per_frame(pl.ws_rstride);
     RSAF_CHECK_ARG(max_frames == 0 || (c.workspace && c.workspace_bytes >= row_bytes_per_clip),
                    "workspace too small (rsaf_mshds_pitch_workspace_bytes)");
     int group = max_frames == 0 ? n_clips : (int)std::min<int64_t>(n_clips, c.workspace_bytes / std::max<int64_t>(row_bytes_per_clip, 1));
@@ -1650,20 +1802,13 @@
     while ((2 << pl.log2m) < P.nfft) ++pl.log2m;
     pl.log2n = 0;
     while ((1 << pl.log2n) < ncc) ++pl.log2n;
-    int wave_r = 0;
-    if (!P.is_cc) wave_r = pl.log2m <= 9 ? 8 : 1 << (pl.log2m - 6);
-    else if (pl.log2n <= 11) wave_r = pl.log2n <= 10 ? 16 : 32;
+    const int wave_r = sh.wave_r;
     if (wave_r && !P.is_cc) P.nfft = 128 * wave_r;
     if (wave_r && P.is_cc) ncc = 64 * wave_r;
     pl.wave_r = wave_r;
     pl.ncc = ncc;
-    pl.cheb = table_mode == 2 ? nullptr : c.sinc_cheb;
     const int cell_lag_lo = P.min_lag > 2 ? P.min_lag : 2;
     const int cell_lag_hi = std::min(P.max_lag - 1, P.brent_ixmax - 1);
-    const bool unclipped = P.brent_ixmax + cell_lag_lo - 1 >= P.refine_depth && cell_lag_hi + 2 + P.refine_depth <= P.brent_ixmax;
-    P.cheb_all_full = unclipped ? 1 : 0;
-    if (pl.cheb == nullptr) P.cheb_clipped = 0;
-    if (!unclipped && !P.cheb_clipped) pl.cheb = nullptr;
     pl.cell_b_lo = P.brent_ixmax + cell_lag_lo - 1;
     pl.cell_n_b = cell_lag_hi - cell_lag_lo + 2;
     pl.cell_ntap_pad = (Lr + 1 + 3) & ~3;
@@ -1712,7 +1857,7 @@
 
 static PitchGroup pitch_group(const PitchCall& c, const PitchPlan& pl, int c0) {
     const int nc = std::min(pl.group, c.n_clips - c0);
-    return PitchGroup{c.ci + c0, c.gpeak + c0, nc, PitchWs(c.workspace, (int64_t)nc * c.max_frames, pl.rstride)};
+    return PitchGroup{c.ci + c0, c.gpeak + c0, nc, PitchWs(c.workspace, (int64_t)nc * c.max_frames, pl.ws_rstride)};
 }
 
 template <int R>
@@ -1761,6 +1906,40 @@
     return RSAF_OK;
 }
 
+template <int R>
+static void launch_ac_cand(const PitchCall& c, const PitchPlan& pl, const PitchGroup& g, dim3 grid, const double2_t* tw, const CandArgs& CA) {
+    hipLaunchKernelGGL(pitch_ac_cand_kernel<R>, grid, dim3(64), pl.lds_fused, c.stream, c.wav, g.ci, g.gpeak, c.window, c.window_r,
+                       pl.P, tw, c.max_frames, CA);
+}
+
+template <int R>
+static void launch_cc_cand(const PitchCall& c, const PitchPlan& pl, const PitchGroup& g, dim3 grid, const double2_t* tw2, const CandArgs& CA) {
+    hipLaunchKernelGGL(pitch_cc_cand_kernel<R>, grid, dim3(64), pl.lds_fused, c.stream, c.wav, g.ci, g.gpeak, pl.P, tw2, c.max_frames, CA);
+}
+
+static int launch_fused(const PitchCall& c, const PitchPlan& pl, const PitchGroup& g, const double2_t* tw, const double2_t* tw2,
+                        FrameOut* out, FrameOut* out2) {
+    const double rows = (double)c.max_frames * (double)g.nc;
+    const CandArgs CA{out, out2, pl.cheb,
+                      DeferArgs{pl.defer ? g.ws.hdr : nullptr, pl.defer ? g.ws.pc_a : nullptr, pl.defer ? g.ws.pc_b : nullptr, 0}};
+    ProfScope prof(pl.P.is_cc ? "mshds_pitch_cc_cand" : "mshds_pitch_ac_cand", c.stream,
+                   rows * (pl.corr_flops + 2048.0 * 2.0 * ceil(2.0 * pl.P.refine_depth / 4.0)), rows * pl.corr_lds);
+    const dim3 wave_grid((c.max_frames + WF_FRAMES - 1) / WF_FRAMES, g.nc);
+    if (pl.P.is_cc)
+        switch (pl.wave_r) {
+            case 16: launch_cc_cand<16>(c, pl, g, wave_grid, tw2, CA); break;
+            case 32: launch_cc_cand<32>(c, pl, g, wave_grid, tw2, CA); break;
+        }
+    else
+        switch (pl.wave_r) {
+            case 8: launch_ac_cand<8>(c, pl, g, wave_grid, tw, CA); break;
+            case 16: launch_ac_cand<16>(c, pl, g, wave_grid, tw, CA); break;
+            case 32: launch_ac_cand<32>(c, pl, g, wave_grid, tw, CA); break;
+        }
+    RSAF_CHECK_HIP(hipGetLastError());
+    return RSAF_OK;
+}
+
 static int launch_refinement(const PitchCall& c, const PitchPlan& pl, const PitchGroup& g, FrameOut* out, FrameOut* out2) {
     const double rows = (double)c.max_frames * (double)g.nc;
     if (pl.grouped) {
@@ -1809,8 +1988,12 @@
     FrameOut* out2 = pl.dual ? o2.frame_out : nullptr;
     for (int c0 = 0; c.max_frames > 0 && c0 < c.n_clips; c0 += pl.group) {
         const PitchGroup g = pitch_group(c, pl, c0);
-        if ((rc = launch_correlation(c, pl, g, tw, tw2)) != RSAF_OK) return rc;
-        if ((rc = launch_candidates(c, pl, g, o1.frame_out, out2)) != RSAF_OK) return rc;
+        if (pl.fused) {
+            if ((rc = launch_fused(c, pl, g, tw, tw2, o1.frame_out, out2)) != RSAF_OK) return rc;
+        } else {
+            if ((rc = launch_correlation(c, pl, g, tw, tw2)) != RSAF_OK) return rc;
+            if ((rc = launch_candidates(c, pl, g, o1.frame_out, out2)) != RSAF_OK) return rc;
+        }
         if (pl.defer && pl.P.debug_stop == 0 && (rc = launch_refinement(c, pl, g, o1.frame_out, out2)) != RSAF_OK) return rc;
     }
     if ((rc = launch_paths(c, pl, o1, pl.P.voicing_thr)) != RSAF_OK) return rc;
@@ -1823,7 +2006,8 @@
 
 int64_t rsaf_mshds_pitch_workspace_bytes_per_clip(int max_frames, const double* params_host ) {
     if (!params_host || max_frames < 0) return -1;
-    return (int64_t)max_frames * PitchWs::bytes_per_frame(pitch_row_lags(params_host) + 2);
+    const int rstride = pitch_shape(params_host).fused ? 0 : pitch_row_lags(params_host) + 2;
+    return (int64_t)max_frames * PitchWs::bytes_per_frame(rstride);
 }
 
 int rsaf_mshds_pitch(const float* wav, const void* clip_info, int n_clips, int max_frames, const double* gpeak,
diff --git a/robust_speech_analysis_framework_amd/csrc/mshds_pitch_layout.h b/robust_speech_analysis_framework_amd/csrc/mshds_pitch_layout.h
--- a/robust_speech_analysis_framework_amd/csrc/mshds_pitch_layout.h
+++ b/robust_speech_analysis_framework_amd/csrc/mshds_pitch_layout.h
@@ -98,6 +98,25 @@
     PL_HD size_t bytes() const { return (size_t)(fft_doubles + sy_doubles) * sizeof(double); }
 };
 
+struct FusedLds {
+    enum Phase { CORR = 0, CAND = 1 };
+    int fft_doubles, sy_doubles;
+    int r_lo, r_hi;
+    PL_HD FusedLds(int plan_doubles, bool is_cc, int L, int r_lo_, int r_hi_)
+        : fft_doubles(plan_doubles), sy_doubles(is_cc ? CcWaveLds(plan_doubles, L).sy_doubles : 0), r_lo(r_lo_), r_hi(r_hi_) {}
+    PL_HD CandLds cand() const { return CandLds(r_lo, r_hi); }
+    PL_HD size_t corr_bytes() const { return (size_t)(fft_doubles + sy_doubles) * sizeof(double); }
+    PL_HD size_t bytes() const { return corr_bytes() > cand().bytes() ? corr_bytes() : cand().bytes(); }
+    struct Span { const char* name; size_t begin, end; Phase phase; };
+    static constexpr int N_SPANS = 4;
+    PL_HD void spans(Span* s) const {
+        s[0] = Span{"fft", 0, (size_t)fft_doubles * sizeof(double), CORR};
+        s[1] = Span{"sy", s[0].end, corr_bytes(), CORR};
+        s[2] = Span{"r_store", 0, (size_t)cand().r_doubles * sizeof(double), CAND};
+        s[3] = Span{"lists", s[2].end, cand().bytes(), CAND};
+    }
+};
+
 struct CellLds {
     int tab_doubles;
     PL_HD explicit CellLds(int ntap_pad) : tab_doubles(ntap_pad * NCH) {}
diff --git a/robust_speech_analysis_framework_amd/mshds.py b/robust_speech_analysis_framework_amd/mshds.py
--- a/robust_speech_analysis_framework_amd/mshds.py
+++ b/robust_speech_analysis_framework_amd/mshds.py
@@ -125,6 +125,7 @@
 
 
 CHEB_CLIP_MAX_DEPTH = 128
+PITCH_TWO_KERNEL, PITCH_FUSE_ALL = 16, 32
 
 
 def sinc_cheb_tables(depth: int, with_clipped: bool):
@@ -257,7 +258,7 @@
     def pitch(self, wav, sample_offs, lengths, gpeak, *, time_step, floor, ceiling, max_candidates=15,
               silence_threshold=0.03, voicing_threshold=0.45, octave_cost=0.01, octave_jump_cost=0.35,
               voiced_unvoiced_cost=0.14, periods=3.0, is_cc=False, refine_depth=70, voicing_threshold2=None,
-              stream=None, dom=None):
+              stream=None, dom=None, two_kernel=None, fuse_all=False, keep_workspace=False):
         import torch
         lib = _lib.load()
         g = _PitchGeom(time_step, floor, ceiling, periods, is_cc)
@@ -276,10 +277,12 @@
                                   lambda: (sinc_cell_tables(g.max_lag, g.brent_ixmax, g.min_lag, int(refine_depth)),))
             if cell is not None:
                 table_mode, cheb = 2, cell
+        if two_kernel is None:
+            two_kernel = self.pitch_two_kernel
         params = (C.c_double * 18)(g.dt, g.floor, g.ceiling, voicing_threshold, octave_cost, silence_threshold,
                                    octave_jump_cost, voiced_unvoiced_cost, g.nsamp_window, g.nsamp_period, g.min_lag,
                                    g.max_lag, g.brent_ixmax, max_candidates, refine_depth, 1 if is_cc else 0,
-                                   g.dt_window, table_mode)
+                                   g.dt_window, table_mode + (PITCH_TWO_KERNEL if two_kernel else PITCH_FUSE_ALL if fuse_all else 0))
         second = None
         if voicing_threshold2 is not None:
             second = {"geom": g, "ci": ci, "ci_dev": ci_d, "total_frames": total, "max_frames": mx, **self._pitch_outputs(tf, n)}
@@ -291,7 +294,7 @@
         chp = _lib.ptr(cheb)
         per_clip = int(lib.rsaf_mshds_pitch_workspace_bytes_per_clip(mx, params)) if n else 0
         ws_bytes = max(per_clip * max(1, min(n, int(self.pitch_ws_cap_bytes // max(per_clip, 1)))), 8)
-        ws = torch.empty(ws_bytes // 8, dtype=torch.float64, device=dev)
+        ws = (torch.zeros if keep_workspace else torch.empty)(ws_bytes // 8, dtype=torch.float64, device=dev)
         def ptrs(o):
             return [_lib.ptr(o[k]) for k in first]
         if n and g.half_window >= 2:
@@ -310,9 +313,12 @@
                 o["stats"][:, 0] = 0
         if second is not None:
             second["stats"] = second["stats"][:n]
-        return {"geom": g, "ci": ci, "ci_dev": ci_d, "sel_freq": first["sel_freq"], "sel_strength": first["sel_strength"],
-                "stats": first["stats"][:n], "frame_out": first["frame_out"], "total_frames": total, "max_frames": mx,
-                "second": second}
+        res = {"geom": g, "ci": ci, "ci_dev": ci_d, "sel_freq": first["sel_freq"], "sel_strength": first["sel_strength"],
+               "stats": first["stats"][:n], "frame_out": first["frame_out"], "total_frames": total, "max_frames": mx,
+               "second": second}
+        if keep_workspace:
+            res["workspace"], res["workspace_per_clip"] = ws, per_clip
+        return res
 
     def intensity(self, wav, sample_offs, lengths, minimum_pitch, time_step, subtract_mean=True, stream=None, dom=None):
         import torch
@@ -524,6 +530,7 @@
         self._last_ltas = {"pitch": p, "pulses": pulses, "n_pulses": npul, "max_pulses": max_pulses}
         return out[:n]
 
+    pitch_two_kernel = False
     pitch_ws_cap_bytes = 16.0e9
     CPP_CHUNK = 48
 
diff --git a/robust_speech_analysis_framework_amd/pipeline.py b/robust_speech_analysis_framework_amd/pipeline.py
--- a/robust_speech_analysis_framework_amd/pipeline.py
+++ b/robust_speech_analysis_framework_amd/pipeline.py
@@ -13,6 +13,8 @@
     "smile_viterbi": "Viterbi over 7 states, one wave per clip",
     "lstm_recurrent": "persistent bi-LSTM recurrence",
 }
+PITCH_FUSED_FAMILIES = ("mshds_pitch_ac_cand", "mshds_pitch_cc_cand")
+PITCH_WAVE_FAMILIES = ("mshds_pitch_ac_fft", "mshds_pitch_cc_fft") + PITCH_FUSED_FAMILIES
 F16_MFMA_PEAK_TFLOPS = 2500.0
 SPLIT_PRODUCTS = 3
 
@@ -163,7 +165,8 @@
                 r["us_per_step"] = round(1e3 * avg_ms / frames_per_launch[name], 3)
             out.append(r)
             continue
-        if name in ("mshds_pitch_ac_fft", "mshds_pitch_cc_fft"):
+        if name in PITCH_WAVE_FAMILIES:
+            fused = name in PITCH_FUSED_FAMILIES
             per_launch = rec["bytes"] / rec["launches"]
             lds = per_launch / (avg_ms * 1e-3) / 1e9
             tf = rec["flops"] / (rec["ms"] * 1e-3) / 1e12
@@ -173,7 +176,9 @@
                         "algorithmic_lds_bytes_per_launch": per_launch,
                         "note": "FLOPs = 5 S log2 S per complex transform + ~30 per point of the spectrum step (real operations, an "
                                 "FMA counts two); LDS bytes = the two exchanges of each transform (16 B x S written and read) + the "
-                                "paired spectrum step; phase timing: profiles/r03/pitch_phase_r03.txt"})
+                                "paired spectrum step; phase timing: profiles/r03/pitch_phase_r03.txt"
+                                + ("; fused frame kernel: the candidate phase runs in the same wave on the row in LDS (no row in HBM), "
+                                   "its Chebyshev coefficient build (fp64 matrix pipe) is added to the FLOPs; profiles/r27" if fused else "")})
             continue
         if rec["flops"] > 0:
             fp64 = name.startswith("mshds_")
```

Measured after the change: 12750, median of 6. About the same (+0.8%).
